# NVlabs/neuralrgbd

Hardware: AMD Instinct MI355X
Metric: depth frames/sec @256x192x64cand, 5-view window; warp-kernel HBM GB/s vs peak (higher is better)
Workload: dtype f32; 1 GPU; plane-sweep grid 256x192x64cand (image 1024x768); config_id=B, depth_candidates=64, views=5, streams_per_gpu=1, streams_total=1, parallelism=replicas x1 (independent video streams)

## Files before the change

### include/nrgbd.h

```cpp
#ifndef NRGBD_H
#define NRGBD_H

#ifdef __cplusplus
extern "C" {
#endif

#define NRGBD_OK             0
#define NRGBD_E_NULL        -1
#define NRGBD_E_SHAPE       -2
#define NRGBD_E_ALIGN       -3
#define NRGBD_E_ARG         -4

#define NRGBD_DIST_L2        0
#define NRGBD_DIST_L1        1

#define NRGBD_MAX_D        256
#define NRGBD_MAX_V         16

#define NRGBD_INTERFACE_VERSION "0.10"
const char* nrgbd_version(void);
const char* nrgbd_strerror(int code);

int nrgbd_homography_terms(const float* K, const float* R, long r_view_stride, long r_row_stride,
                           const float* t, long t_view_stride, long t_elem_stride, float* KR, float* Kt,
// ... 61 lines not shown
int nrgbd_dpv_resample(const float* dpv, const float* T, const float* rays,
                       const float* d_candi, float tan_hh, float tan_hv,
                       float z_half, float z_radius, float pad_value,
                       int do_clamp, float clamp_lo, float clamp_hi,
                       float* out, int D, int h, int w, void* stream);

int nrgbd_dpv_resample_to(const float* dpv, const float* T, const float* rays,
                          const float* d_candi_out, float tan_hh, float tan_hv,
                          float z_half, float z_radius, float pad_value,
                          int do_clamp, float clamp_lo, float clamp_hi,
                          float* out, int D_src, int D_out, int h, int w, void* stream);

int nrgbd_dpv_keyframe_maps(const float* dpv, const float* T, const float* rays,
                            const float* d_candi_out, const float* d_candi_src,
                            float tan_hh, float tan_hv, float z_half, float z_radius, float pad_value,
                            int do_clamp, float clamp_lo, float clamp_hi,
                            float* dmap_kf, float* conf_kf, float* dmap_ref, float* conf_ref,
                            int D_src, int D_out, int h, int w, void* stream);

int nrgbd_logsoftmax_d(const float* a, const float* b, float scale, float* out,
                       int D, long n, void* stream);

int nrgbd_depth_regress(const float* logp, const float* d_candi,
                        float* depth, float* conf, int D, long n, void* stream);

int nrgbd_export_depth_u16(const float* logp, const float* d_candi, float depth_scale, float conf_scale,
                           float* depth, float* conf, unsigned short* depth_u16, unsigned short* conf_u16,
                           int D, long n, void* stream);

int nrgbd_depth_regress_rows(const float* logp, const float* d_candi,
                             float* depth, float* conf, int D, long n, void* stream);
int nrgbd_export_depth_u16_rows(const float* logp, const float* d_candi, float depth_scale, float conf_scale,
                                float* depth, float* conf, unsigned short* depth_u16, unsigned short* conf_u16,
                                int D, long n, void* stream);

int nrgbd_warp_depth_fwd(const float* src, const float* dmap, const float* K, const float* R, const float* t,
                         const float* rays, float* out, int N, int C, int H, int W, void* stream);
int nrgbd_warp_depth_bwd_workgroups(int H, int W);
int nrgbd_warp_depth_bwd(const float* src, const float* dmap, const float* K, const float* R, const float* t,
                         const float* rays, const float* g_out, float* partial, float* g_R, float* g_t,
                         int N, int C, int H, int W, void* stream);

#define NRGBD_LBA_STATE      32
#define NRGBD_LBA_MAX_LEVELS  8
int nrgbd_lba_pyramid(const float* const* planes, int nplanes, int H, int W, const int* ks, int nlevels, float* out,
                      void* stream);
int nrgbd_lba_workgroups(int H, int W);
int nrgbd_lba_grad(const float* ref, const float* src, const float* dmap, const float* conf, const float* K, const float* rays,
                   const float* state, float* partial, int N, int H, int W, void* stream);
int nrgbd_lba_update(const float* partial, int nwg, const float* init, float* state, float* loss_log, int log_stride,
                     int log_slot, int N, int H, int W, int joint, int step, double lr, int opt_R, int opt_t, void* stream);

int nrgbd_conv3d_workgroups(int D, int H, int W);
int nrgbd_conv3d_pack_weights(const float* w, float* w_packed, int Cin, void* stream);
int nrgbd_conv3d_3x3x3_f32(const float* x, const float* x_ss, int x_relu,
                           const float* res, const float* res_ss, int res_relu,
                           float* materialized, const float* w_packed, float* y, float* stats,
                           int D, int H, int W, int Cin, int Cout, void* stream);
int nrgbd_conv3d_3x3x3_cout1_f32(const float* x, const float* x_ss, int x_relu,
                                 const float* res, const float* res_ss, int res_relu,
                                 const float* w_tap_major, float* y,
                                 int D, int H, int W, int Cin, void* stream);
int nrgbd_conv3d_cout1_bwd_workgroups(int D, int H, int W, int dgrad);
int nrgbd_conv3d_cout1_dgrad_f32(const float* gy, const float* w_tap_major, float* gx, int D, int H, int W, void* stream);
int nrgbd_conv3d_cout1_wgrad_workspace(int D, int H, int W, size_t* bytes);
int nrgbd_conv3d_cout1_wgrad_f32(const float* x, const float* gy, float* dw, void* workspace, size_t workspace_bytes, int D, int H, int W,
                                 void* stream);
int nrgbd_conv3d_wgrad_workgroups(void);
int nrgbd_conv3d_wgrad_ranges(void);
int nrgbd_conv3d_wgrad_f32(const float* x, const float* gy, float* partial, float* dw,
                           int D, int H, int W, int Cin, void* stream);
int nrgbd_bn3d_finalize(const float* stats, int num_workgroups, long count,
                        const float* gamma, const float* beta, float eps, float momentum,
                        float* running_mean, float* running_var, float* scale_shift, unsigned int* collapse_count, long long* batches_tracked, void* stream);

int nrgbd_bn2d_partial_floats(int C);
int nrgbd_bn2d_train_act(const float* x, const float* gamma, const float* beta, float eps, int act,
                         const float* residual, float* y, float* partial, float* mean_var,
                         int N, int C, long HW, void* stream);
int nrgbd_avgpool8(const float* x, float* y, int NC, int H, int W, void* stream);
int nrgbd_avgpool_cl(const float* x, float* y, int N, int H, int W, int C, int k, void* stream);
int nrgbd_conv2d_few_f32(const float* x, int ldx, const float* w_packed, const float* bias, int out_lrelu, float* y, int ldy,
                         int ycoff, int N, int H, int W, int Cin, int Cout, void* stream);
int nrgbd_scatter_channels(const float* src, long stride_c, long stride_y, long stride_x, int C, int H, int W, float* dst,
                           int ldy, int coff, int n_rep, long rep_stride, void* stream);
int nrgbd_bias_act_nchw(float* x, const float* bias, float slope, int N, int C, long HW, void* stream);

int nrgbd_conv_wino_tiles(int N, int H, int W, int dilation);
int nrgbd_conv_wino_rnet_f32(const float* x, const float* w_wino, const float* bias, int out_lrelu, float* y,
                             int N, int H, int W, int Cin, int Cout, void* stream);
int nrgbd_conv_wino_rnet_ex_f32(const float* x, const float* w_wino, const float* bias, int out_lrelu, float* y,
                                int N, int H, int W, int Cin, int Cout, int ldy, int ycoff, int cout_valid, void* stream);
int nrgbd_conv_wino_rnet_deconv_f32(const float* x, const float* w_masked, const float* bias, int out_lrelu, float* y,
                                    int N, int H, int W, int Cin, int Cout, int ldy, int ycoff, int cout_valid, void* stream);
int nrgbd_conv_wino_rnet_deconv_pack(const float* w_wino, float* w_masked, int Cin, void* stream);
int nrgbd_conv_wino_pack(const float* w, float* w_wino, int Cin, int Cout, int kd, int transposed, void* stream);
int nrgbd_bn_finalize_cm(const float* stats, int rows, int C, long count, const float* gamma, const float* beta, float eps,
                         float momentum, float* running_mean, float* running_var, float* scale_shift, unsigned int* collapse_count,
                         long long* batches_tracked, void* stream);
int nrgbd_conv_wino_f32(const float* x, const float* x_ss, int x_relu, const float* res, const float* res_ss,
                        int res_relu, float* materialized, const float* w_wino, float* y, float* stats,
                        int N, int H, int W, int Cin, int Cout, int kd, int dilation, void* stream);

int nrgbd_conv_wino_dw_pack(const float* w, float* w_wino, int Cin, int Cout, int transposed, void* stream);
int nrgbd_conv_wino_dw_f32(const float* x, const float* x_ss, int x_relu, const float* res, const float* res_ss,
                           int res_relu, float* materialized, const float* w_wino, float* y, float* stats,
                           int N, int H, int W, int Cin, int Cout, void* stream);
int nrgbd_conv_wino_dw_workgroups(int N, int H, int W, int Cout);
int nrgbd_conv_wino_dw4_pack(const float* w, float* w_wino, int Cin, int Cout, int transposed, void* stream);
int nrgbd_conv_wino_dw4_workspace(int N, int H, int W, int Cout, size_t* bytes);
int nrgbd_conv_wino_dw4_f32(const float* x, const float* x_ss, int x_relu, float x_unit, const float* w_wino, float* y, float* stats,
                            void* workspace, size_t workspace_bytes, int N, int H, int W, int Cin, int Cout, void* stream);
int nrgbd_conv_wino_dw_unit_f32(const float* x, const float* x_ss, float x_unit, const float* w_wino, float* y, float* stats,
                                int N, int H, int W, int Cin, int Cout, void* stream);

int nrgbd_conv2d_rnet_f32(const float* x, const float* w_packed, const float* bias, int out_lrelu, float* y,
                          int ldy, int ycoff, int cout_valid, int mode, int pa, int pb,
                          int N, int H, int W, int Cin, int Cout, void* stream);
int nrgbd_rnet_pack(const float* dpv_log, const float* feat, int feat_planar, float* out, int D, int Cf, long P,
                    void* stream);

int nrgbd_conv2d_taps_f32(const float* x, const float* x_ss, int x_relu, const float* w_packed, float* y, float* stats,
                          int N, int H, int W, int Cin, int Cout, int taps, int in_stride, void* stream);
int nrgbd_space_to_depth2(const float* x, int nchw, float* y, int N, int C, int H, int W, int Cp, void* stream);
int nrgbd_conv2d_wgrad_workgroups(int N, int H, int W, int Cin, int Cout);
int nrgbd_conv2d_wgrad_f32(const float* x, const float* gy, float* partial, float* dw, int N, int H, int W, int Cin, int Cout,
                           int dilation, void* stream);
int nrgbd_conv2d_workgroups(int N, int H, int W);
int nrgbd_conv_pack_weights(const float* w, float* w_packed, int Cin, int Cout, int taps, void* stream);
int nrgbd_conv2d_3x3_f32(const float* x, const float* x_ss, int x_relu,
                         const float* res, const float* res_ss, int res_relu,
                         float* materialized, const float* w_packed, const float* bias, int out_lrelu,
                         float* y, float* stats, int N, int H, int W, int Cin, int Cout, int dilation,
                         void* stream);
int nrgbd_bn_finalize(const float* stats, int num_workgroups, int C, long count,
                      const float* gamma, const float* beta, float eps, float momentum,
                      float* running_mean, float* running_var, float* scale_shift, unsigned int* collapse_count, long long* batches_tracked, void* stream);
int nrgbd_bn_small_stats(int nseg, const float* const* x, const long* rows, int C, const float* const* gamma, const float* const* beta,
                     const float* eps, const float* momentum, float* const* running_mean, float* const* running_var,
                     long long* const* batches_tracked, float* const* scale_shift, void* stream);
int nrgbd_spp_concat(const float* quarter, int Cq, const float* deep, int Cd,
                     const float* bz0, const float* bss0, int bh0, int bw0, const float* bz1, const float* bss1, int bh1, int bw1,
                     const float* bz2, const float* bss2, int bh2, int bw2, const float* bz3, const float* bss3, int bh3, int bw3,
                     int Cb, float* out, int N, int h, int w, void* stream);
int nrgbd_logsoftmax_rows(const float* x, float* y, long rows, int C, void* stream);
int nrgbd_logsoftmax_d_bwd(const float* logp, const float* g, float scale, float* gz, int D, long n, void* stream);
int nrgbd_logsoftmax_rows_bwd(const float* y, const float* g, float* gx, long rows, int C, void* stream);
int nrgbd_nll_workgroups(long n);
int nrgbd_nll_fwd(const float* logp, const long long* target, long ignore_index, int D, long n, int channels_last,
                  float* partial, float* out, void* stream);
int nrgbd_nll_bwd(const long long* target, long ignore_index, const float* g_out, const float* stat, float* g_logp, int D,
                  long n, int channels_last, void* stream);
int nrgbd_adam_step(float* const* params, const float* const* grads, float* const* exp_avg, float* const* exp_avg_sq,
                    float* const* steps, const long* numel, int ntensors, double lr, double beta1, double beta2, double eps,
                    double weight_decay, int maximize, void* stream);
long nrgbd_grad_norm_workspace(const long* numel, int ntensors);
int nrgbd_grad_norm(const float* const* grads, const long* numel, int ntensors, double max_norm, void* workspace,
                    size_t workspace_bytes, float* clip, float* nonfinite_steps, void* stream);
int nrgbd_scale_tensors(float* const* tensors, const long* numel, int ntensors, const float* clip, void* stream);
int nrgbd_adam_step_clipped(float* const* params, const float* const* grads, float* const* exp_avg, float* const* exp_avg_sq,
                            float* const* steps, const long* numel, int ntensors, double lr, double beta1, double beta2, double eps,
                            double weight_decay, int maximize, const float* clip, int skip_nonfinite, void* stream);
int nrgbd_bias_lrelu_cl_workgroups(long rows, int C);
int nrgbd_bias_lrelu_cl_fwd(const float* x, const float* bias, float slope, float* y, long rows, int C, void* stream);
int nrgbd_bias_lrelu_cl_bwd(const float* y, const float* gy, float slope, float* gx, float* g_bias, float* partial,
                            long rows, int C, void* stream);
int nrgbd_upsample_bilinear_ac(const float* x, float* y, int N, int bh, int bw, int H, int W, int C, int backward,
                               void* stream);
#define NRGBD_GATHER_MAX_V   6
typedef struct { int idx[NRGBD_GATHER_MAX_V + 1]; } nrgbd_window_slots;
int nrgbd_frame_ingest_u8(const unsigned char* src, int Hin, int Win, long pitch, int layout, float mean0, float mean1, float mean2,
                          float std0, float std1, float std2, float* dst, int Hout, int Wout, void* stream);
int nrgbd_window_gather(const float* ring, int R, long slot_stride, nrgbd_window_slots slots, int V, float* src, float* ref,
                        int H, int W, void* stream);
#define NRGBD_DEPTH_MAX_THRESHOLDS 512
int nrgbd_depth_ingest_u16(const unsigned short* depth, int Hin, int Win, long pitch, const int* rows_full, const int* cols_full,
                           const int* rows_q, const int* cols_q, const int* mask_rows_q, const int* mask_cols_q, float depth_scale,
                           const int* thr_q, int n_q, const int* thr_full, int n_full, long long* labels_q, long long* labels_full,
                           float* dmap_raw, float* dmap_imgsize, int H, int W, int h, int w, void* stream);
int nrgbd_nhwc_stats_workgroups(long P);
int nrgbd_nhwc_stats(const float* x, long P, int C, float* stats, void* stream);
int nrgbd_nhwc_act(const float* x, const float* x_ss, int x_relu, const float* res, const float* res_ss,
                   int res_relu, float* y, long P, int C, int ldy, void* stream);
int nrgbd_nhwc_act_lean(const float* x, const float* x_ss, int x_relu, const float* res, const float* res_ss,
                        int res_relu, float* y, long P, int C, int ldy, int wg_per_cu, void* stream);
#define NRGBD_DEPTH_EVAL_MAX_SETS 8
int nrgbd_depth_eval_workgroups(long n);
long nrgbd_depth_eval_workspace(long n, int J);
int nrgbd_depth_eval(const float* depth, const float* logconf, const float* gt, long n, float gt_min, float gt_max,
                     const float* log_thr, int J, void* workspace, long workspace_bytes, double* frame_sums,
                     long long* frame_counts, long long* frame_header, double* total_sums, long long* total_counts,
                     long long* total_header, float* err_map, void* stream);
#define NRGBD_DGF_TILE_Y 16
#define NRGBD_DGF_TILE_X 64
int nrgbd_dgf_refine_f32(const float* depth_lr, int n, int h, int w, const float* img, int H, int W,
                         const float* w1, const float* b1, const float* w2, const float* b2, float eps,
                         float* out, void* stream);
#define NRGBD_TSDF_EXTRACT_VOXELS 1024
#define NRGBD_TSDF_SCAN_PASS 1024
#define NRGBD_TSDF_RAYCAST_MAX_STEPS 65536
#define NRGBD_TSDF_RAYCAST_TILE 16
#define NRGBD_TSDF_RAYCAST_MAX_SIDE 16384
int nrgbd_tsdf_integrate_f32(float* tsdf, float* weight, int X, int Y, int Z, float ox, float oy, float oz, float voxel_size,
                             const float* depth, const float* gate, float gate_thr, const float* wmap, int H, int W,
                             const float* pose, float fx, float fy, float cx, float cy, float trunc, float d_near, float d_far,
                             float w_max, const int* box, void* stream);
long nrgbd_tsdf_extract_workspace(int X, int Y, int Z);
// ... 79 lines not shown
```

### neuralrgbd_amd/_lib.py

```python
import ctypes
import os

_HERE = os.path.dirname(os.path.abspath(__file__))
LIB_PATH = os.path.join(_HERE, "csrc", "libnrgbd_hip.so")

_c = ctypes
_P = _c.c_void_p
_F = _c.c_float
_I = _c.c_int
_L = _c.c_long
_D = _c.c_double
_Z = _c.c_size_t

GATHER_MAX_V = 6
DEPTH_MAX_THRESHOLDS = 512
DEPTH_EVAL_MAX_SETS = 8
DGF_TILE = (16, 64)
TSDF_EXTRACT_VOXELS = 1024
TSDF_SCAN_PASS = 1024
TSDF_RAYCAST_MAX_STEPS = 65536
TSDF_RAYCAST_TILE = 16
TSDF_RAYCAST_MAX_SIDE = 16384
ICP_MAX_WG = 256
ICP_RECORD_BYTES = 240
ICP_STATE_BYTES = 152
ICP_FEW, ICP_NONFINITE, ICP_DEGENERATE, ICP_LARGE = 1, 2, 3, 4
ICP_MAX_THETA2 = 0.25
CONSISTENCY_MAX_SRC = 16


class WindowSlots(ctypes.Structure):
    _fields_ = [("idx", _I * (GATHER_MAX_V + 1))]


SIGNATURES = {
    "nrgbd_version": (_c.c_char_p, []),
    "nrgbd_strerror": (_c.c_char_p, [_I]),
    "nrgbd_homography_terms": (_I, [_P, _P, _L, _L, _P, _L, _L, _P, _P, _I, _P]),
    "nrgbd_pose_inverse": (_I, [_P, _L, _P, _P, _I, _P]),
    "nrgbd_pack_nhwc": (_I, [_P, _P, _P, _I, _I, _I, _I, _I, _I, _I, _P, _P]),
    "nrgbd_costvol_fwd": (_I, [_P, _P, _P, _P, _P, _P, _F, _F, _F, _I, _I, _P, _P,
                               _I, _I, _I, _I, _I, _I, _P]),
    "nrgbd_costvol_fwd_gen": (_I, [_P, _P, _P, _P, _P, _P, _F, _F, _F, _I, _I, _P, _P,
                                   _I, _I, _I, _I, _I, _I, _I, _P]),
    "nrgbd_costvol_bwd_workspace": (_I, [_I, _I, _I, _I, _I, _P]),
    "nrgbd_costvol_bwd": (_I, [_P, _P, _P, _P, _P, _P, _F, _F, _F, _I, _I, _P, _P, _P,
                               _I, _I, _I, _I, _I, _I, _P, _Z, _P]),
    "nrgbd_costvol_bwd_det_workspace": (_I, [_I, _I, _I, _I, _I, _P]),
    "nrgbd_costvol_bwd_det": (_I, [_P, _P, _P, _P, _P, _P, _F, _F, _F, _I, _I, _P, _P, _P,
                                   _I, _I, _I, _I, _I, _I, _P, _Z, _P]),
    "nrgbd_bn_cl_workgroups": (_I, [_L, _I]),
    "nrgbd_bn_cl_fwd": (_I, [_P, _P, _P, _P, _F, _F, _P, _P, _I, _P, _P, _P, _L, _I, _P]),
    "nrgbd_bn_cl_bwd": (_I, [_P, _P, _P, _I, _P, _P, _P, _P, _P, _L, _I, _P]),
    "nrgbd_warp_volume": (_I, [_P, _L, _L, _L, _L, _P, _L, _L, _L, _P, _P, _P, _P, _F, _F, _I,
                               _P, _P, _P, _I, _I, _I, _I, _I, _I, _P]),
    "nrgbd_warp_volume_cl": (_I, [_P, _L, _L, _L, _L, _P, _L, _L, _L, _P, _P, _P, _P, _F, _F, _I,
                                  _P, _P, _P, _I, _I, _I, _I, _I, _I, _P]),
    "nrgbd_dpv_resample": (_I, [_P, _P, _P, _P, _F, _F, _F, _F, _F, _I, _F, _F, _P, _I, _I, _I, _P]),
    "nrgbd_dpv_resample_to": (_I, [_P, _P, _P, _P, _F, _F, _F, _F, _F, _I, _F, _F, _P, _I, _I, _I, _I, _P]),
    "nrgbd_dpv_keyframe_maps": (_I, [_P, _P, _P, _P, _P, _F, _F, _F, _F, _F, _I, _F, _F, _P, _P, _P, _P, _I, _I, _I, _I, _P]),
    "nrgbd_logsoftmax_d": (_I, [_P, _P, _F, _P, _I, _L, _P]),
    "nrgbd_depth_regress": (_I, [_P, _P, _P, _P, _I, _L, _P]),
    "nrgbd_export_depth_u16": (_I, [_P, _P, _F, _F, _P, _P, _P, _P, _I, _L, _P]),
    "nrgbd_depth_regress_rows": (_I, [_P, _P, _P, _P, _I, _L, _P]),
    "nrgbd_export_depth_u16_rows": (_I, [_P, _P, _F, _F, _P, _P, _P, _P, _I, _L, _P]),
    "nrgbd_warp_depth_fwd": (_I, [_P, _P, _P, _P, _P, _P, _P, _I, _I, _I, _I, _P]),
    "nrgbd_warp_depth_bwd_workgroups": (_I, [_I, _I]),
    "nrgbd_warp_depth_bwd": (_I, [_P, _P, _P, _P, _P, _P, _P, _P, _P, _P, _I, _I, _I, _I, _P]),
    "nrgbd_lba_pyramid": (_I, [_P, _I, _I, _I, _P, _I, _P, _P]),
    "nrgbd_lba_workgroups": (_I, [_I, _I]),
    "nrgbd_lba_grad": (_I, [_P, _P, _P, _P, _P, _P, _P, _P, _I, _I, _I, _P]),
    "nrgbd_lba_update": (_I, [_P, _I, _P, _P, _P, _I, _I, _I, _I, _I, _I, _I, _D, _I, _I, _P]),
    "nrgbd_conv3d_workgroups": (_I, [_I, _I, _I]),
    "nrgbd_conv3d_pack_weights": (_I, [_P, _P, _I, _P]),
    "nrgbd_conv3d_3x3x3_f32": (_I, [_P, _P, _I, _P, _P, _I, _P, _P, _P, _P, _I, _I, _I, _I, _I, _P]),
    "nrgbd_conv3d_3x3x3_cout1_f32": (_I, [_P, _P, _I, _P, _P, _I, _P, _P, _I, _I, _I, _I, _P]),
    "nrgbd_conv3d_cout1_bwd_workgroups": (_I, [_I, _I, _I, _I]),
    "nrgbd_conv3d_cout1_dgrad_f32": (_I, [_P, _P, _P, _I, _I, _I, _P]),
    "nrgbd_conv3d_cout1_wgrad_workspace": (_I, [_I, _I, _I, _P]),
    "nrgbd_conv3d_cout1_wgrad_f32": (_I, [_P, _P, _P, _P, _Z, _I, _I, _I, _P]),
    "nrgbd_conv_wino_tiles": (_I, [_I, _I, _I, _I]),
    "nrgbd_conv_wino_rnet_f32": (_I, [_P, _P, _P, _I, _P, _I, _I, _I, _I, _I, _P]),
    "nrgbd_conv_wino_rnet_ex_f32": (_I, [_P, _P, _P, _I, _P, _I, _I, _I, _I, _I, _I, _I, _I, _P]),
    "nrgbd_conv_wino_rnet_deconv_f32": (_I, [_P, _P, _P, _I, _P, _I, _I, _I, _I, _I, _I, _I, _I, _P]),
    "nrgbd_conv_wino_rnet_deconv_pack": (_I, [_P, _P, _I, _P]),
    "nrgbd_conv_wino_pack": (_I, [_P, _P, _I, _I, _I, _I, _P]),
    "nrgbd_bn_finalize_cm": (_I, [_P, _I, _I, _L, _P, _P, _F, _F, _P, _P, _P, _P, _P, _P]),
    "nrgbd_conv_wino_f32": (_I, [_P, _P, _I, _P, _P, _I, _P, _P, _P, _P, _I, _I, _I, _I, _I, _I, _I, _P]),
    "nrgbd_conv_wino_dw_pack": (_I, [_P, _P, _I, _I, _I, _P]),
    "nrgbd_conv_wino_dw_f32": (_I, [_P, _P, _I, _P, _P, _I, _P, _P, _P, _P, _I, _I, _I, _I, _I, _P]),
    "nrgbd_conv_wino_dw_workgroups": (_I, [_I, _I, _I, _I]),
    "nrgbd_conv_wino_dw_unit_f32": (_I, [_P, _P, _F, _P, _P, _P, _I, _I, _I, _I, _I, _P]),
    "nrgbd_conv_wino_dw4_pack": (_I, [_P, _P, _I, _I, _I, _P]),
    "nrgbd_conv_wino_dw4_workspace": (_I, [_I, _I, _I, _I, _P]),
    "nrgbd_conv_wino_dw4_f32": (_I, [_P, _P, _I, _F, _P, _P, _P, _P, _c.c_size_t, _I, _I, _I, _I, _I, _P]),
    "nrgbd_conv3d_wgrad_workgroups": (_I, []),
    "nrgbd_conv3d_wgrad_ranges": (_I, []),
    "nrgbd_conv3d_wgrad_f32": (_I, [_P, _P, _P, _P, _I, _I, _I, _I, _P]),
    "nrgbd_bn3d_finalize": (_I, [_P, _I, _L, _P, _P, _F, _F, _P, _P, _P, _P, _P, _P]),
    "nrgbd_bn2d_partial_floats": (_I, [_I]),
    "nrgbd_bn2d_train_act": (_I, [_P, _P, _P, _F, _I, _P, _P, _P, _P, _I, _I, _L, _P]),
    "nrgbd_avgpool8": (_I, [_P, _P, _I, _I, _I, _P]),
    "nrgbd_conv2d_few_f32": (_I, [_P, _I, _P, _P, _I, _P, _I, _I, _I, _I, _I, _I, _I, _P]),
    "nrgbd_avgpool_cl": (_I, [_P, _P, _I, _I, _I, _I, _I, _P]),
    "nrgbd_scatter_channels": (_I, [_P, _L, _L, _L, _I, _I, _I, _P, _I, _I, _I, _L, _P]),
    "nrgbd_bias_act_nchw": (_I, [_P, _P, _F, _I, _I, _L, _P]),
    "nrgbd_conv2d_workgroups": (_I, [_I, _I, _I]),
    "nrgbd_conv2d_wgrad_workgroups": (_I, [_I, _I, _I, _I, _I]),
    "nrgbd_conv2d_wgrad_f32": (_I, [_P, _P, _P, _P, _I, _I, _I, _I, _I, _I, _P]),
    "nrgbd_conv2d_taps_f32": (_I, [_P, _P, _I, _P, _P, _P, _I, _I, _I, _I, _I, _I, _I, _P]),
    "nrgbd_space_to_depth2": (_I, [_P, _I, _P, _I, _I, _I, _I, _I, _P]),
    "nrgbd_conv_pack_weights": (_I, [_P, _P, _I, _I, _I, _P]),
    "nrgbd_conv2d_3x3_f32": (_I, [_P, _P, _I, _P, _P, _I, _P, _P, _P, _I, _P, _P, _I, _I, _I, _I, _I, _I, _P]),
    "nrgbd_conv2d_rnet_f32": (_I, [_P, _P, _P, _I, _P, _I, _I, _I, _I, _I, _I, _I, _I, _I, _I, _I, _P]),
    "nrgbd_rnet_pack": (_I, [_P, _P, _I, _P, _I, _I, _L, _P]),
    "nrgbd_bn_finalize": (_I, [_P, _I, _I, _L, _P, _P, _F, _F, _P, _P, _P, _P, _P, _P]),
    "nrgbd_logsoftmax_rows": (_I, [_P, _P, _L, _I, _P]),
    "nrgbd_logsoftmax_d_bwd": (_I, [_P, _P, _F, _P, _I, _L, _P]),
    "nrgbd_logsoftmax_rows_bwd": (_I, [_P, _P, _P, _L, _I, _P]),
    "nrgbd_nll_workgroups": (_I, [_L]),
    "nrgbd_nll_fwd": (_I, [_P, _P, _L, _I, _L, _I, _P, _P, _P]),
    "nrgbd_nll_bwd": (_I, [_P, _L, _P, _P, _P, _I, _L, _I, _P]),
    "nrgbd_adam_step": (_I, [_P, _P, _P, _P, _P, _P, _I, _D, _D, _D, _D, _D, _I, _P]),
    "nrgbd_grad_norm_workspace": (_L, [_P, _I]),
    "nrgbd_grad_norm": (_I, [_P, _P, _I, _D, _P, _Z, _P, _P, _P]),
    "nrgbd_scale_tensors": (_I, [_P, _P, _I, _P, _P]),
    "nrgbd_adam_step_clipped": (_I, [_P, _P, _P, _P, _P, _P, _I, _D, _D, _D, _D, _D, _I, _P, _I, _P]),
    "nrgbd_bias_lrelu_cl_workgroups": (_I, [_L, _I]),
    "nrgbd_bias_lrelu_cl_fwd": (_I, [_P, _P, _F, _P, _L, _I, _P]),
    "nrgbd_bias_lrelu_cl_bwd": (_I, [_P, _P, _F, _P, _P, _P, _L, _I, _P]),
    "nrgbd_upsample_bilinear_ac": (_I, [_P, _P, _I, _I, _I, _I, _I, _I, _I, _P]),
    "nrgbd_bn_small_stats": (_I, [_I, _P, _P, _I, _P, _P, _P, _P, _P, _P, _P, _P, _P]),
    "nrgbd_spp_concat": (_I, [_P, _I, _P, _I, _P, _P, _I, _I, _P, _P, _I, _I, _P, _P, _I, _I, _P, _P, _I, _I, _I, _P, _I, _I, _I, _P]),
    "nrgbd_frame_ingest_u8": (_I, [_P, _I, _I, _L, _I, _F, _F, _F, _F, _F, _F, _P, _I, _I, _P]),
    "nrgbd_window_gather": (_I, [_P, _I, _L, WindowSlots, _I, _P, _P, _I, _I, _P]),
    "nrgbd_depth_ingest_u16": (_I, [_P, _I, _I, _L, _P, _P, _P, _P, _P, _P, _F, _P, _I, _P, _I, _P, _P, _P, _P, _I, _I, _I, _I, _P]),
    "nrgbd_depth_eval_workgroups": (_I, [_L]),
    "nrgbd_depth_eval_workspace": (_L, [_L, _I]),
    "nrgbd_depth_eval": (_I, [_P, _P, _P, _L, _F, _F, _P, _I, _P, _L, _P, _P, _P, _P, _P, _P, _P, _P]),
    "nrgbd_dgf_refine_f32": (_I, [_P, _I, _I, _I, _P, _I, _I, _P, _P, _P, _P, _F, _P, _P]),
    "nrgbd_tsdf_integrate_f32": (_I, [_P, _P, _I, _I, _I, _F, _F, _F, _F, _P, _P, _F, _P, _I, _I, _P, _F, _F, _F, _F, _F, _F, _F, _F, _P, _P]),
    "nrgbd_tsdf_extract_workspace": (_L, [_I, _I, _I]),
    "nrgbd_tsdf_extract_points": (_I, [_P, _P, _I, _I, _I, _F, _F, _F, _F, _F, _P, _L, _P, _L, _P, _P]),
    "nrgbd_tsdf_raycast_f32": (_I, [_P, _P, _I, _I, _I, _F, _F, _F, _F, _P, _P, _F, _F, _F, _F, _I, _I, _F, _F, _F, _F, _P, _P, _P]),
    "nrgbd_tsdf_mesh_workspace": (_L, [_I, _I, _I]),
    "nrgbd_tsdf_extract_mesh": (_I, [_P, _P, _I, _I, _I, _F, _F, _F, _F, _F, _P, _L, _P, _L, _P, _L, _P, _P]),
    "nrgbd_tsdf_integrate_color_f32": (_I, [_P, _P, _P, _I, _I, _I, _F, _F, _F, _F, _P, _P, _F, _P, _I, _I, _P, _F, _F, _F, _F, _F, _F, _F, _F,
                                            _P, _P, _I, _I, _F, _F, _F, _F, _P, _P]),
    "nrgbd_tsdf_extract_points_color": (_I, [_P, _P, _P, _I, _I, _I, _F, _F, _F, _F, _F, _P, _L, _P, _P, _L, _P, _P]),
    "nrgbd_tsdf_extract_mesh_color": (_I, [_P, _P, _P, _I, _I, _I, _F, _F, _F, _F, _F, _P, _L, _P, _P, _L, _P, _L, _P, _P]),
    "nrgbd_tsdf_raycast_color_f32": (_I, [_P, _P, _P, _I, _I, _I, _F, _F, _F, _F, _P, _P, _F, _F, _F, _F, _I, _I, _F, _F, _F, _F, _P, _P, _P, _P]),
    "nrgbd_tsdf_reintegrate_f32": (_I, [_P, _P, _I, _I, _I, _F, _F, _F, _F, _P, _P, _P, _P, _P, _I, _I, _F, _F, _F, _F, _F, _F, _F, _F, _F, _F,
                                        _P, _P]),
    "nrgbd_tsdf_reintegrate_color_f32": (_I, [_P, _P, _P, _I, _I, _I, _F, _F, _F, _F, _P, _P, _P, _P, _P, _I, _I, _F, _F, _F, _F, _F, _F, _F, _F,
                                              _F, _F, _P, _P, _I, _I, _F, _F, _F, _F, _P, _P]),
    "nrgbd_icp_workgroups": (_I, [_I, _I]),
    "nrgbd_icp_workspace": (_L, [_I, _I]),
    "nrgbd_icp_terms_f32": (_I, [_P, _P, _F, _I, _I, _F, _F, _F, _F, _F, _F, _I, _P, _P, _I, _I, _F, _F, _F, _F, _P, _F, _F, _P, _L, _P,
                                 _P]),
    "nrgbd_icp_terms_photo_f32": (_I, [_P, _P, _F, _I, _I, _F, _F, _F, _F, _F, _F, _I, _P, _P, _I, _I, _F, _F, _F, _F, _P, _F, _F, _P, _L,
                                       _P, _P, _P, _P, _P, _F, _F, _P, _P]),
    "nrgbd_icp_update": (_I, [_P, _P, _I, _P, _I, _c.c_longlong, _D, _P, _P]),
    "nrgbd_depth_consistency_f32": (_I, [_P, _P, _F, _I, _I, _F, _F, _F, _F, _F, _F, _P, _P, _L, _P, _P, _I, _F, _I, _P, _P, _P]),
    "nrgbd_tsdf_shift_f32": (_I, [_P, _P, _I, _I, _I, _I, _I, _I, _I, _I, _P]),
    "nrgbd_tsdf_blocks_gather_f32": (_I, [_P, _I, _I, _I, _I, _P, _I, _P, _P, _P]),
    "nrgbd_tsdf_blocks_scatter_f32": (_I, [_P, _I, _I, _I, _I, _P, _I, _P, _P]),
    "nrgbd_nhwc_stats_workgroups": (_I, [_L]),
    "nrgbd_nhwc_stats": (_I, [_P, _L, _I, _P, _P]),
    "nrgbd_nhwc_act": (_I, [_P, _P, _I, _P, _P, _I, _P, _L, _I, _I, _P]),
    "nrgbd_nhwc_act_lean": (_I, [_P, _P, _I, _P, _P, _I, _P, _L, _I, _I, _I, _P]),
}

_lib = None


class NrgbdError(RuntimeError):
    pass


def load():
    global _lib
    if _lib is not None:
        return _lib
    if not os.path.isfile(LIB_PATH):
        raise NrgbdError(
            "libnrgbd_hip.so not found at %s — build it with `python -m neuralrgbd_amd.build` "
            "(hipcc --offload-arch=gfx950). There is no CPU / eager fallback for this path." % LIB_PATH)
    lib = ctypes.CDLL(LIB_PATH)
    for name, (res, args) in SIGNATURES.items():
        try:
            fn = getattr(lib, name)
        except AttributeError:
            raise NrgbdError("libnrgbd_hip.so does not export %s (stale build?)" % name)
# ... 11 lines not shown
```

### neuralrgbd_amd/csrc/conv2d.hip

```cpp
#include <cstdint>
#include <cstdlib>

#include "conv_tile.hpp"

namespace nrgbd {

constexpr int kT2 = 16;

struct Conv2dArgs {
    const float* x;
    const float* x_ss;
    const float* res;
    const float* res_ss;
    float* mat;
    const float* wp;
    const float* bias;
    float* y;
    float* stats;
    int x_relu, res_relu, out_lrelu;
    int N, H, W, Cin;
    int xcd;
    int ldy;
    int ycoff;
    int cout_valid;
    int up;
    int pa, pb;
    float* planar;
    int xs;
};

template <int COUT, int DIL, bool RES, int NTAP = 9, int EPI = 0>
__global__ __launch_bounds__(256, COUT <= 32 ? 3 : 2) void conv2d_mfma_kernel(const Conv2dArgs a) {
    constexpr int HS = kT2 + 2 * DIL, HALO = HS * HS;
    constexpr int NPF = (HALO * (kCB / 4) + 255) / 256;
    constexpr int NF = COUT / 32;
    constexpr int G4 = kCB / 8;
    constexpr int NSTEP = NTAP * G4;
    static_assert(NTAP == 9 || ((NTAP == 4 || NTAP == 1) && DIL == 1), "2x2 taps: transposed-conv phases / stride-2 convs on a "
                                                                         "space-to-depth input; 1 tap: 1x1 convolutions");
    constexpr bool PF_SPREAD = 2 + (RES ? 2 : 1) * NPF <= NSTEP;
    static_assert(PF_SPREAD || NSTEP >= 2, "prefetch does not fit the step loop");
    extern __shared__ __attribute__((aligned(16))) float lds[];

    const int tid = threadIdx.x, lane = tid & 63, wv = tid >> 6;
    const int tiles_x = (a.W + kT2 - 1) / kT2, tiles_y = (a.H + kT2 - 1) / kT2;
    int t = xcd_tile(blockIdx.x, gridDim.x, a.xcd);
    const int tile_id = t;
    const int tx = t % tiles_x; t /= tiles_x;
    const int ty = t % tiles_y; const int n = t / tiles_y;
    const int x0 = tx * kT2, y0 = ty * kT2;
    const int Cin = a.Cin, ncblk = Cin / kCB;

    const int i = lane & 31, khalf = lane >> 5;
    int dy, px;
    row_to_yx(i, dy, px);
    const int wy = wv * 4;
    int pa = a.pa, pb = a.pb;
    const float* wpk = a.wp;
    if constexpr (NTAP == 4) {
        if (a.up == 2) { pa = blockIdx.y >> 1; pb = blockIdx.y & 1; wpk += (size_t)blockIdx.y * 4 * a.Cin * COUT; }
    }
    const int hv0 = (wy + dy) * HS + px + (NTAP == 4 ? pa * HS + pb : NTAP == 1 ? HS + 1 : 0);

    f32x16 acc[2][NF];
#pragma unroll
    for (int m = 0; m < 2; ++m)
#pragma unroll
        for (int f = 0; f < NF; ++f)
#pragma unroll
            for (int e = 0; e < 16; ++e) acc[m][f][e] = 0.f;

    const int c4 = tid & 3;
    unsigned pf_off[NPF];
    unsigned pf_ok = 0;
    unsigned pf_own = 0;
    f32x4 pre[NPF], prer[RES ? NPF : 1];
#pragma unroll
    for (int u = 0; u < NPF; ++u) {
        const int hv = (tid >> 2) + 64 * u;
        const int hy = hv / HS, hx = hv - hy * HS;
        const int gy = y0 + hy - DIL, gx = x0 + hx - DIL;
        const bool ok = hv < HALO && gy >= 0 && gy < a.H && gx >= 0 && gx < a.W;
        const int xs = (NTAP == 1 && a.xs > 1) ? a.xs : 1;
        pf_off[u] = ok ? (unsigned)((((size_t)n * (a.H * xs) + (size_t)gy * xs) * (a.W * xs) + (size_t)gx * xs) * Cin + c4 * 4) : (unsigned)(c4 * 4);
        if (ok) pf_ok |= 1u << u;
        if (ok && hy >= DIL && hy < DIL + kT2 && hx >= DIL && hx < DIL + kT2) pf_own |= 1u << u;
    }
#pragma unroll
    for (int u = 0; u < NPF; ++u) {
        pre[u] = *reinterpret_cast<const f32x4*>(a.x + pf_off[u]);
        if constexpr (RES) prer[u] = *reinterpret_cast<const f32x4*>(a.res + pf_off[u]);
    }

    const int wstep = ncblk * (G4 * NF * 64);
    for (int cblk = 0; cblk < ncblk; ++cblk) {
        {
            const int c = cblk * kCB + c4 * 4;
            float ss[8] = {1.f, 0.f, 1.f, 0.f, 1.f, 0.f, 1.f, 0.f}, rs[8] = {1.f, 0.f, 1.f, 0.f, 1.f, 0.f, 1.f, 0.f};
            if (a.x_ss) {
#pragma unroll
                for (int e = 0; e < 8; ++e) ss[e] = a.x_ss[2 * c + e];
            }
            if (RES && a.res_ss) {
#pragma unroll
                for (int e = 0; e < 8; ++e) rs[e] = a.res_ss[2 * c + e];
            }
#pragma unroll
            for (int u = 0; u < NPF; ++u) {
                const int hv = (tid >> 2) + 64 * u;
                if (hv >= HALO) continue;
                f32x4 v = {0.f, 0.f, 0.f, 0.f};
                if ((pf_ok >> u) & 1u) {
                    v = pre[u];
                    if (a.x_ss) {
                        v.x = __builtin_fmaf(v.x, ss[0], ss[1]); v.y = __builtin_fmaf(v.y, ss[2], ss[3]);
                        v.z = __builtin_fmaf(v.z, ss[4], ss[5]); v.w = __builtin_fmaf(v.w, ss[6], ss[7]);
                    }
                    if (a.x_relu) { v.x = fmaxf(v.x, 0.f); v.y = fmaxf(v.y, 0.f); v.z = fmaxf(v.z, 0.f); v.w = fmaxf(v.w, 0.f); }
                    if constexpr (RES) {
                        f32x4 r = prer[u];
                        if (a.res_ss) {
                            r.x = __builtin_fmaf(r.x, rs[0], rs[1]); r.y = __builtin_fmaf(r.y, rs[2], rs[3]);
                            r.z = __builtin_fmaf(r.z, rs[4], rs[5]); r.w = __builtin_fmaf(r.w, rs[6], rs[7]);
                        }
                        if (a.res_relu) { r.x = fmaxf(r.x, 0.f); r.y = fmaxf(r.y, 0.f); r.z = fmaxf(r.z, 0.f); r.w = fmaxf(r.w, 0.f); }
                        v = v + r;
                    }
                    if (a.mat && ((pf_own >> u) & 1u))
                        *reinterpret_cast<f32x4*>(a.mat + pf_off[u] + cblk * kCB) = v;
                }
                *reinterpret_cast<f32x4*>(lds + lds_slot(hv, c4)) = v;
            }
        }
        __syncthreads();

        const f32x4* wb = reinterpret_cast<const f32x4*>(wpk) + (size_t)cblk * (G4 * NF * 64) + lane;
        constexpr int BD = NTAP == 1 ? 1 : (COUT <= 64 ? 3 : 1), NB = BD + 1;
        f32x4 Bn[NB][NF], An[2][2];
#pragma unroll
        for (int b = 0; b < BD; ++b) {
            const f32x4* w0 = wb + (size_t)(b / G4) * wstep + (b % G4) * (NF * 64);
#pragma unroll
            for (int f = 0; f < NF; ++f) Bn[b][f] = w0[f * 64];
        }
        An[0][0] = *reinterpret_cast<const f32x4*>(lds + lds_slot(hv0, khalf * 2));
        An[0][1] = *reinterpret_cast<const f32x4*>(lds + lds_slot(hv0 + 2 * HS, khalf * 2));
        const unsigned nb = (cblk + 1) * kCB, live = cblk + 1 < ncblk ? ~0u : 0u;
#pragma unroll
        for (int s = 0; s < NSTEP; ++s) {
            const int cur = s & 1, nxt = cur ^ 1;
            if (s + 1 < NSTEP) {
                const int tap = (s + 1) / G4, g = (s + 1) % G4;
                const int voff = NTAP == 9 ? ((tap / 3) * HS + (tap % 3)) * DIL : NTAP == 4 ? (tap >> 1) * HS + (tap & 1) : 0;
                int h0 = hv0;
                asm volatile("" : "+v"(h0));
                An[nxt][0] = *reinterpret_cast<const f32x4*>(lds + lds_slot(h0 + voff, khalf * 2 + g));
                An[nxt][1] = *reinterpret_cast<const f32x4*>(lds + lds_slot(h0 + 2 * HS + voff, khalf * 2 + g));
            }
            if (s + BD < NSTEP) {
                const int tap = (s + BD) / G4, g = (s + BD) % G4;
                const f32x4* wn = wb + (size_t)tap * wstep + g * (NF * 64);
#pragma unroll
                for (int f = 0; f < NF; ++f) Bn[(s + BD) % NB][f] = wn[f * 64];
            }
            if constexpr (PF_SPREAD) {
                if constexpr (!RES) {
                    if (s >= 2 && s < 2 + NPF && live) pre[s - 2] = *reinterpret_cast<const f32x4*>(a.x + pf_off[s - 2] + nb);
                } else {
                    if (s >= 2 && s < 2 + NPF) pre[s - 2] = *reinterpret_cast<const f32x4*>(a.x + ((pf_off[s - 2] + nb) & live));
                }
                if constexpr (RES) {
                    if (s >= 2 + NPF && s < 2 + 2 * NPF)
                        prer[s - 2 - NPF] = *reinterpret_cast<const f32x4*>(a.res + ((pf_off[s - 2 - NPF] + nb) & live));
                }
            } else {
                if (s == 0) {
#pragma unroll
                    for (int u = 0; u < NPF; ++u) pre[u] = *reinterpret_cast<const f32x4*>(a.x + ((pf_off[u] + nb) & live));
                }
                if constexpr (RES) {
                    if (s == 1) {
#pragma unroll
                        for (int u = 0; u < NPF; ++u) prer[u] = *reinterpret_cast<const f32x4*>(a.res + ((pf_off[u] + nb) & live));
                    }
                }
            }
#pragma unroll
            for (int e = 0; e < 4; ++e)
#pragma unroll
                for (int m = 0; m < 2; ++m)
#pragma unroll
                    for (int f = 0; f < NF; ++f)
                        acc[m][f] = __builtin_amdgcn_mfma_f32_32x32x2f32(An[cur][m][e], Bn[s % NB][f][e], acc[m][f], 0, 0, 0);
        }
        __syncthreads();
    }

    float s1[NF], s2[NF], bs[NF];
#pragma unroll
    for (int f = 0; f < NF; ++f) { s1[f] = 0.f; s2[f] = 0.f; bs[f] = a.bias ? a.bias[f * 32 + i] : 0.f; }
    if constexpr (EPI == 1) {
        const size_t plane = (size_t)a.H * a.W;
#pragma unroll
        for (int m = 0; m < 2; ++m) {
#pragma unroll
            for (int q = 0; q < 4; ++q) {
                float z[4][NF];
#pragma unroll
                for (int e = 0; e < 4; ++e) {
                    float mx = -INFINITY;
#pragma unroll
                    for (int f = 0; f < NF; ++f) { z[e][f] = acc[m][f][4 * q + e] + bs[f]; mx = fmaxf(mx, z[e][f]); }
#pragma unroll
                    for (int o = 1; o < 32; o <<= 1) mx = fmaxf(mx, __shfl_xor(mx, o, 64));
                    float sm = 0.f;
#pragma unroll
                    for (int f = 0; f < NF; ++f) { z[e][f] = z[e][f] - mx; sm += expf(z[e][f]); }
#pragma unroll
                    for (int o = 1; o < 32; o <<= 1) sm += __shfl_xor(sm, o, 64);
                    const float ls = logf(sm);
#pragma unroll
                    for (int f = 0; f < NF; ++f) z[e][f] = z[e][f] - ls;
                }
                const int row = 8 * q + 4 * khalf;
                int ry, rx;
                row_to_yx(row, ry, rx);
                const int gy = y0 + wy + 2 * m + ry, gx = x0 + rx;
                if (gy < a.H) {
#pragma unroll
                    for (int f = 0; f < NF; ++f) {
                        float* o = a.planar + ((size_t)n * COUT + f * 32 + i) * plane + (size_t)gy * a.W + gx;
                        if (gx + 3 < a.W && (a.W & 3) == 0) {
                            *reinterpret_cast<f32x4*>(o) = f32x4{z[0][f], z[1][f], z[2][f], z[3][f]};
                        } else {
#pragma unroll
                            for (int e = 0; e < 4; ++e)
                                if (gx + e < a.W) o[e] = z[e][f];
                        }
                    }
                }
            }
        }
        return;
    }
#pragma unroll
    for (int m = 0; m < 2; ++m) {
#pragma unroll
        for (int r = 0; r < 16; ++r) {
            const int row = (r & 3) + 8 * (r >> 2) + 4 * khalf;
            int ry, rx;
            row_to_yx(row, ry, rx);
            const int gy = y0 + wy + 2 * m + ry, gx = x0 + rx;
            if (gy < a.H && gx < a.W) {
                const size_t pix = a.up ? ((size_t)n * (2 * a.H) + 2 * gy + pa) * (2 * a.W) + 2 * gx + pb
                                        : ((size_t)n * a.H + gy) * a.W + gx;
#pragma unroll
                for (int f = 0; f < NF; ++f) {
                    float z = acc[m][f][r] + bs[f];
                    if (a.out_lrelu) z = z > 0.f ? z : 0.01f * z;
                    if (f * 32 + i < a.cout_valid) a.y[pix * a.ldy + a.ycoff + f * 32 + i] = z;
                    s1[f] += z;
                    s2[f] = __builtin_fmaf(z, z, s2[f]);
                }
            }
        }
    }
    if (a.stats) {
        float* red = lds;
#pragma unroll
        for (int f = 0; f < NF; ++f) {
            s1[f] += __shfl_xor(s1[f], 32, 64);
            s2[f] += __shfl_xor(s2[f], 32, 64);
        }
        if (khalf == 0) {
#pragma unroll
            for (int f = 0; f < NF; ++f) {
                red[wv * (2 * COUT) + f * 32 + i] = s1[f];
                red[wv * (2 * COUT) + COUT + f * 32 + i] = s2[f];
            }
        }
// ... 98 lines not shown
void nhwc_act_lean_kernel(const float* __restrict__ x, const float* __restrict__ x_ss, int x_relu, const float* __restrict__ res,
                          const float* __restrict__ res_ss, int res_relu, float* __restrict__ y, int P, int C, int ldy) {
    extern __shared__ __attribute__((aligned(16))) float lean_tab[];
    const int tid = threadIdx.x, cq = C >> 2, ppw = 256 / cq;
    const bool xa = x_ss != nullptr, ra = RES && res_ss != nullptr;
    for (int j = tid; j < 2 * C; j += 256) {
        if (xa) lean_tab[(j & 1) * C + (j >> 1)] = x_ss[j];
        if (ra) lean_tab[2 * C + (j & 1) * C + (j >> 1)] = res_ss[j];
    }
    __syncthreads();
    const int lp = tid / cq, c = (tid - lp * cq) * 4;
    const unsigned lx = (unsigned)tid * 16u;
    const unsigned ly = ((unsigned)lp * (unsigned)ldy + (unsigned)c) * 4u;
    const float* tx = lean_tab + c;
    const int pstep = (int)gridDim.x * ppw;
    int pb = (int)blockIdx.x * ppw;
    u32x4 v[kLeanWords], r[RES ? kLeanWords : 1];
    auto request = [&](int u, int q) {
        v[u] = __builtin_amdgcn_raw_buffer_load_b128(lean_window(x, q, P, C, C, ppw), lx, 0, kLeanNt);
        if constexpr (RES) r[u] = __builtin_amdgcn_raw_buffer_load_b128(lean_window(res, q, P, C, C, ppw), lx, 0, kLeanNt);
    };
    auto finish = [&](int u, int q) {
        f32x4 a = __builtin_bit_cast(f32x4, v[u]);
        lean_apply(a, tx, C, xa, x_relu);
        if constexpr (RES) {
            f32x4 b = __builtin_bit_cast(f32x4, r[u]);
            lean_apply(b, tx + 2 * C, C, ra, res_relu);
            a = a + b;
        }
        __builtin_amdgcn_raw_buffer_store_b128(__builtin_bit_cast(u32x4, a), lean_window(y, q, P, ldy, C, ppw), ly, 0, kLeanNt);
    };
    static_assert(kLeanWords == 2, "the loop below names its two slots");
    request(0, pb);
    for (; pb < P; pb += 2 * pstep) {
        request(1, pb + pstep);
        finish(0, pb);
        request(0, pb + 2 * pstep);
        finish(1, pb + pstep);
    }
}

__global__ __launch_bounds__(256) void bn_finalize_kernel(const float* __restrict__ stats, int nwg, int C, double count,
                                                          const float* __restrict__ gamma, const float* __restrict__ beta,
                                                          float eps, float momentum, float* __restrict__ running_mean,
                                                          float* __restrict__ running_var, float* __restrict__ ss, unsigned int* __restrict__ collapse_count, long long* __restrict__ batches_tracked) {
    __shared__ double sh[2][256];
    const int c = blockIdx.x, tid = threadIdx.x;
    double s1 = 0.0, s2 = 0.0;
    for (int g = tid; g < nwg; g += 256) {
        s1 += (double)stats[(size_t)g * 2 * C + c];
        s2 += (double)stats[(size_t)g * 2 * C + C + c];
    }
    sh[0][tid] = s1; sh[1][tid] = s2;
    __syncthreads();
    for (int o = 128; o > 0; o >>= 1) {
        if (tid < o) { sh[0][tid] += sh[0][tid + o]; sh[1][tid] += sh[1][tid + o]; }
        __syncthreads();
    }
    if (tid == 0) bn_finalize_channel(sh[0][0], sh[1][0], count, gamma[c], beta[c], eps, momentum, running_mean, running_var, ss, c, collapse_count);
    if (tid == 0 && c == 0 && batches_tracked) *batches_tracked += 1;
}

template <int COUT, int DIL>
static void launch_conv2d(const Conv2dArgs& a, int nwg, hipStream_t st) {
    constexpr int HS = kT2 + 2 * DIL;
    const size_t lds = (size_t)HS * HS * kSV * sizeof(float);
    if (a.res) hipLaunchKernelGGL((conv2d_mfma_kernel<COUT, DIL, true>), dim3(nwg), dim3(256), lds, st, a);
    else       hipLaunchKernelGGL((conv2d_mfma_kernel<COUT, DIL, false>), dim3(nwg), dim3(256), lds, st, a);
}

template <int COUT, int NTAP, int EPI>
static void launch_conv2d_ex(const Conv2dArgs& a, int nwg, hipStream_t st, int ny = 1) {
    constexpr int HS = kT2 + 2;
    const size_t lds = (size_t)HS * HS * kSV * sizeof(float);
    hipLaunchKernelGGL((conv2d_mfma_kernel<COUT, 1, false, NTAP, EPI>), dim3(nwg, ny), dim3(256), lds, st, a);
}

template <int COUT, int NTAP>
static void launch_conv2d_taps(const Conv2dArgs& a, int nwg, hipStream_t st) {
    constexpr int HS = kT2 + 2;
    const size_t lds = (size_t)HS * HS * kSV * sizeof(float);
    hipLaunchKernelGGL((conv2d_mfma_kernel<COUT, 1, false, NTAP, 0>), dim3(nwg), dim3(256), lds, st, a);
}

__global__ __launch_bounds__(256) void space_to_depth2_kernel(const float* __restrict__ x, int nchw, float* __restrict__ y,
                                                              int N, int C, int H, int W, int Cp) {
    const int Ho = H >> 1, Wo = W >> 1;
    const long total = (long)N * Ho * Wo * Cp;
    const long idx = (long)blockIdx.x * 256 + threadIdx.x;
    if (idx >= total) return;
    const int cp = (int)(idx % Cp);
    long t = idx / Cp;
    const int xo = (int)(t % Wo); t /= Wo;
    const int yo = (int)(t % Ho);
    const int n = (int)(t / Ho);
    float v = 0.f;
    if (cp < 4 * C) {
        const int ph = cp / C, c = cp - ph * C;
        const int yi = 2 * yo + (ph >> 1), xi = 2 * xo + (ph & 1);
        v = nchw ? x[(((size_t)n * C + c) * H + yi) * W + xi] : x[(((size_t)n * H + yi) * W + xi) * C + c];
    }
    y[idx] = v;
}

__global__ __launch_bounds__(256) void space_to_depth2_cl4_kernel(const float* __restrict__ x, float* __restrict__ y, int N, int C, int H,
                                                                  int W, int Cp) {
    const int Ho = H >> 1, Wo = W >> 1, q4 = Cp >> 2;
    const long total = (long)N * Ho * Wo * q4;
    const long idx = (long)blockIdx.x * 256 + threadIdx.x;
    if (idx >= total) return;
    const int cp = (int)(idx % q4) * 4;
    long t = idx / q4;
    const int xo = (int)(t % Wo); t /= Wo;
    const int yo = (int)(t % Ho);
    const int n = (int)(t / Ho);
    float4 v = make_float4(0.f, 0.f, 0.f, 0.f);
    if (cp < 4 * C) {
        const int ph = cp / C, c = cp - ph * C;
        v = *reinterpret_cast<const float4*>(x + (((size_t)n * H + 2 * yo + (ph >> 1)) * W + 2 * xo + (ph & 1)) * C + c);
    }
    *reinterpret_cast<float4*>(y + idx * 4) = v;
}

__global__ __launch_bounds__(256) void space_to_depth2_rgb_kernel(const float* __restrict__ x, float* __restrict__ y, int N, int H, int W) {
    const int Ho = H >> 1, Wo = W >> 1;
    const long total = (long)N * Ho * Wo;
    const long idx = (long)blockIdx.x * 256 + threadIdx.x;
    if (idx >= total) return;
    const int xo = (int)(idx % Wo);
    long t = idx / Wo;
    const int yo = (int)(t % Ho);
    const int n = (int)(t / Ho);
    float2 v[3][2];
#pragma unroll
    for (int c = 0; c < 3; ++c)
#pragma unroll
        for (int py = 0; py < 2; ++py)
            v[c][py] = *reinterpret_cast<const float2*>(x + (((size_t)n * 3 + c) * H + 2 * yo + py) * W + 2 * xo);
    float o[16];
#pragma unroll
    for (int py = 0; py < 2; ++py)
#pragma unroll
        for (int c = 0; c < 3; ++c) { o[(py * 2 + 0) * 3 + c] = v[c][py].x; o[(py * 2 + 1) * 3 + c] = v[c][py].y; }
    o[12] = o[13] = o[14] = o[15] = 0.f;
    float4* dst = reinterpret_cast<float4*>(y + idx * 16);
#pragma unroll
    for (int q = 0; q < 4; ++q) dst[q] = make_float4(o[4 * q], o[4 * q + 1], o[4 * q + 2], o[4 * q + 3]);
}

}

extern "C" int nrgbd_space_to_depth2(const float* x, int nchw, float* y, int N, int C, int H, int W, int Cp, void* stream) {
    using namespace nrgbd;
    if (!x || !y) return NRGBD_E_NULL;
    if (N <= 0 || C <= 0 || H <= 0 || W <= 0 || (H & 1) || (W & 1) || Cp < 4 * C) return NRGBD_E_SHAPE;
    const long total = (long)N * (H / 2) * (W / 2) * Cp;
    const bool aligned = (((uintptr_t)x | (uintptr_t)y) & 15) == 0;
    if (!nchw && (C & 3) == 0 && (Cp & 3) == 0 && aligned)
        hipLaunchKernelGGL(space_to_depth2_cl4_kernel, dim3((unsigned)((total / 4 + 255) / 256)), dim3(256), 0, (hipStream_t)stream, x, y, N, C,
                           H, W, Cp);
    else if (nchw && C == 3 && Cp == 16 && aligned)
        hipLaunchKernelGGL(space_to_depth2_rgb_kernel, dim3((unsigned)((total / 16 + 255) / 256)), dim3(256), 0, (hipStream_t)stream, x, y, N,
                           H, W);
    else
        hipLaunchKernelGGL(space_to_depth2_kernel, dim3((unsigned)((total + 255) / 256)), dim3(256), 0, (hipStream_t)stream, x, nchw,
                           y, N, C, H, W, Cp);
    NRGBD_CHECK_LAUNCH();
    return NRGBD_OK;
}

extern "C" int nrgbd_conv2d_taps_f32(const float* x, const float* x_ss, int x_relu, const float* w_packed, float* y,
                                     float* stats, int N, int H, int W, int Cin, int Cout, int taps, int in_stride, void* stream) {
    using namespace nrgbd;
    if (!x || !w_packed || !y) return NRGBD_E_NULL;
    if (N <= 0 || H <= 0 || W <= 0 || Cin <= 0 || Cin % kCB) return NRGBD_E_SHAPE;
    if (taps != 1 && taps != 4) return NRGBD_E_ARG;
    if (in_stride < 1 || in_stride > 8 || (in_stride != 1 && taps != 1)) return NRGBD_E_ARG;
    if ((long)N * H * W * Cin * in_stride * in_stride >= (1L << 32)) return NRGBD_E_SHAPE;
    Conv2dArgs a{x, x_ss, nullptr, nullptr, nullptr, w_packed, nullptr, y, stats, x_relu, 0, 0, N, H, W, Cin,
                 0, Cout, 0, Cout, 0, 0, 0, nullptr, in_stride};
    const int nwg = ceil_div(W, kT2) * ceil_div(H, kT2) * N;
    hipStream_t st = (hipStream_t)stream;
    if (taps == 1) {
        if (Cout == 32) launch_conv2d_taps<32, 1>(a, nwg, st);
        else if (Cout == 64) launch_conv2d_taps<64, 1>(a, nwg, st);
        else if (Cout == 128) launch_conv2d_taps<128, 1>(a, nwg, st);
        else return NRGBD_E_SHAPE;
    } else {
        if (Cout == 32) launch_conv2d_taps<32, 4>(a, nwg, st);
        else if (Cout == 64) launch_conv2d_taps<64, 4>(a, nwg, st);
        else return NRGBD_E_SHAPE;
    }
    NRGBD_CHECK_LAUNCH();
    return NRGBD_OK;
}

extern "C" int nrgbd_conv2d_workgroups(int N, int H, int W) {
    using namespace nrgbd;
    if (N <= 0 || H <= 0 || W <= 0) return NRGBD_E_SHAPE;
    return ceil_div(W, kT2) * ceil_div(H, kT2) * N;
}

extern "C" int nrgbd_conv_pack_weights(const float* w, float* wp, int Cin, int Cout, int taps, void* stream) {
    using namespace nrgbd;
    if (!w || !wp) return NRGBD_E_NULL;
    if (Cin <= 0 || Cin % kCB || Cout <= 0 || Cout % 32 || (taps != 9 && taps != 27 && taps != 4 && taps != 1)) return NRGBD_E_SHAPE;
    const long total = (long)taps * Cin * Cout;
    hipLaunchKernelGGL(conv_pack_weights_kernel, dim3((unsigned)((total + 255) / 256)), dim3(256), 0, (hipStream_t)stream,
                       w, wp, Cin, Cout, taps);
    NRGBD_CHECK_LAUNCH();
    return NRGBD_OK;
}

extern "C" int nrgbd_conv2d_3x3_f32(const float* x, const float* x_ss, int x_relu, const float* res, const float* res_ss,
                                    int res_relu, float* materialized, const float* w_packed, const float* bias,
                                    int out_lrelu, float* y, float* stats, int N, int H, int W, int Cin, int Cout,
                                    int dilation, void* stream) {
    using namespace nrgbd;
    if (!x || !w_packed || !y) return NRGBD_E_NULL;
    if (N <= 0 || H <= 0 || W <= 0 || Cin <= 0 || Cin % kCB) return NRGBD_E_SHAPE;
    if ((long)N * H * W * Cin >= (1L << 32)) return NRGBD_E_SHAPE;
    Conv2dArgs a{x, x_ss, res, res_ss, materialized, w_packed, bias, y, stats, x_relu, res_relu, out_lrelu, N, H, W, Cin,
                 dev_env_int("NRGBD_XCD"), Cout, 0, Cout, 0, 0, 0, nullptr};
    const int nwg = ceil_div(W, kT2) * ceil_div(H, kT2) * N;
    hipStream_t st = (hipStream_t)stream;
    if (dilation == 1 && Cout == 32) launch_conv2d<32, 1>(a, nwg, st);
    else if (dilation == 1 && Cout == 64) launch_conv2d<64, 1>(a, nwg, st);
    else if (dilation == 1 && Cout == 96) launch_conv2d<96, 1>(a, nwg, st);
    else if (dilation == 1 && Cout == 128) launch_conv2d<128, 1>(a, nwg, st);
    else if (dilation == 2 && Cout == 128) launch_conv2d<128, 2>(a, nwg, st);
    else return NRGBD_E_SHAPE;
    NRGBD_CHECK_LAUNCH();
    return NRGBD_OK;
}

extern "C" int nrgbd_conv2d_rnet_f32(const float* x, const float* w_packed, const float* bias, int out_lrelu, float* y,
                                     int ldy, int ycoff, int cout_valid, int mode, int pa, int pb, int N, int H, int W,
                                     int Cin, int Cout, void* stream) {
    using namespace nrgbd;
    if (!x || !w_packed || !y) return NRGBD_E_NULL;
    if (N <= 0 || H <= 0 || W <= 0 || Cin <= 0 || Cin % kCB) return NRGBD_E_SHAPE;
    if ((long)N * H * W * Cin >= (1L << 32)) return NRGBD_E_SHAPE;
    if (mode < 0 || mode > 3 || (pa & ~1) || (pb & ~1)) return NRGBD_E_ARG;
    if (mode != 2 && (cout_valid <= 0 || cout_valid > Cout || ycoff < 0 || ldy < ycoff + cout_valid)) return NRGBD_E_SHAPE;
    Conv2dArgs a{x, nullptr, nullptr, nullptr, nullptr, w_packed, bias, y, nullptr, 0, 0, out_lrelu, N, H, W, Cin,
                 0, ldy, ycoff, cout_valid, mode == 1 ? 1 : (mode == 3 ? 2 : 0), pa, pb, mode == 2 ? y : nullptr};
    const int nwg = ceil_div(W, kT2) * ceil_div(H, kT2) * N;
    hipStream_t st = (hipStream_t)stream;
    if (mode == 0) {
        if (Cout == 64) launch_conv2d_ex<64, 9, 0>(a, nwg, st);
        else if (Cout == 96) launch_conv2d_ex<96, 9, 0>(a, nwg, st);
        else if (Cout == 128) launch_conv2d_ex<128, 9, 0>(a, nwg, st);
        else return NRGBD_E_SHAPE;
    } else if (mode == 1) {
        if (Cout == 64) launch_conv2d_ex<64, 4, 0>(a, nwg, st);
        else return NRGBD_E_SHAPE;
    } else if (mode == 3) {
        if (Cout == 64) launch_conv2d_ex<64, 4, 0>(a, nwg, st, 4);
        else return NRGBD_E_SHAPE;
    } else {
        if (Cout == 64) launch_conv2d_ex<64, 9, 1>(a, nwg, st);
        else if (Cout == 128) launch_conv2d_ex<128, 9, 1>(a, nwg, st);
        else return NRGBD_E_SHAPE;
    }
    NRGBD_CHECK_LAUNCH();
    return NRGBD_OK;
}

namespace nrgbd {
__global__ __launch_bounds__(256) void rnet_pack_kernel(const float* __restrict__ dpv_log, const float* __restrict__ feat,
                                                        int feat_planar, float* __restrict__ out, int D, int Cf, long P) {
    __shared__ float tile[64][65];
    const long p0 = (long)blockIdx.x * 64;
    const int tid = threadIdx.x, lane = tid & 63, wv = tid >> 6;
    const int C = D + Cf;
// ... 97 lines not shown
```

### neuralrgbd_amd/csrc/conv_few.hip

```cpp
#include "common.hpp"

namespace nrgbd {

typedef float f32x4 __attribute__((ext_vector_type(4)));

constexpr int kFewT = 16, kFewHS = kFewT + 2, kFewHalo = kFewHS * kFewHS;
constexpr int kFewPitch = 20;
constexpr int kFewNPF = (kFewHalo * 4 + 255) / 256;

struct ConvFewArgs {
    const float* x;
    const float* wp;
    const float* bias;
    float* y;
    int N, H, W, Cin, ldx, ldy, ycoff, lrelu;
};

template <int CO>
__global__ __launch_bounds__(256, 6) void conv_few_kernel(const ConvFewArgs a) {
    __shared__ __attribute__((aligned(16))) float tile[1][kFewHalo * kFewPitch];
    const int tid = threadIdx.x, px = tid & 15, py = tid >> 4;
    const int tiles_x = (a.W + kFewT - 1) / kFewT, tiles_y = (a.H + kFewT - 1) / kFewT;
    int t = blockIdx.x;
    const int tx = t % tiles_x; t /= tiles_x;
    const int ty = t % tiles_y; const int n = t / tiles_y;
    const int x0 = tx * kFewT, y0 = ty * kFewT;
    const int nblk = a.Cin >> 4;

    const int c4 = tid & 3;
    unsigned off[kFewNPF];
    unsigned ok = 0;
#pragma unroll
    for (int u = 0; u < kFewNPF; ++u) {
        const int hv = (tid >> 2) + 64 * u;
        const int hy = hv / kFewHS, hx = hv - hy * kFewHS;
        const int gy = y0 + hy - 1, gx = x0 + hx - 1;
        const bool in = hv < kFewHalo && gy >= 0 && gy < a.H && gx >= 0 && gx < a.W;
        off[u] = in ? (unsigned)((((size_t)n * a.H + gy) * a.W + gx) * a.ldx + c4 * 4) : (unsigned)(c4 * 4);
        if (in) ok |= 1u << u;
    }
    f32x4 pre[kFewNPF];
#pragma unroll
    for (int u = 0; u < kFewNPF; ++u) pre[u] = *reinterpret_cast<const f32x4*>(a.x + off[u]);
    auto publish = [&](int buf) {
#pragma unroll
        for (int u = 0; u < kFewNPF; ++u) {
            const int hv = (tid >> 2) + 64 * u;
            if (hv < kFewHalo)
                *reinterpret_cast<f32x4*>(&tile[buf][hv * kFewPitch + c4 * 4]) = ((ok >> u) & 1u) ? pre[u] : f32x4{0.f, 0.f, 0.f, 0.f};
        }
    };
    publish(0);
    __syncthreads();

    float acc[CO];
#pragma unroll
    for (int co = 0; co < CO; ++co) acc[co] = a.bias ? a.bias[co] : 0.f;

    for (int c = 0; c < nblk; ++c) {
        constexpr int buf = 0;
        if (c + 1 < nblk) {
#pragma unroll
            for (int u = 0; u < kFewNPF; ++u) pre[u] = *reinterpret_cast<const f32x4*>(a.x + off[u] + (c + 1) * 16);
        }
        const float* w = a.wp + (size_t)c * (9 * CO * 16);
#pragma unroll 1
        for (int ky = 0; ky < 3; ++ky) {
            const float* trow = &tile[buf][((py + ky) * kFewHS + px) * kFewPitch];
#pragma unroll
            for (int kx = 0; kx < 3; ++kx) {
                const float* tp = trow + kx * kFewPitch;
                f32x4 v[4];
#pragma unroll
                for (int q = 0; q < 4; ++q) v[q] = *reinterpret_cast<const f32x4*>(tp + 4 * q);
#pragma unroll
                for (int co = 0; co < CO; ++co) {
                    const float* wr = w + ((ky * 3 + kx) * CO + co) * 16;
#pragma unroll
                    for (int q = 0; q < 4; ++q) {
                        acc[co] = __builtin_fmaf(v[q].x, wr[4 * q + 0], acc[co]);
                        acc[co] = __builtin_fmaf(v[q].y, wr[4 * q + 1], acc[co]);
                        acc[co] = __builtin_fmaf(v[q].z, wr[4 * q + 2], acc[co]);
                        acc[co] = __builtin_fmaf(v[q].w, wr[4 * q + 3], acc[co]);
                    }
                }
            }
        }
        __syncthreads();
        if (c + 1 < nblk) publish(0);
        __syncthreads();
    }
    const int gy = y0 + py, gx = x0 + px;
    if (gy < a.H && gx < a.W) {
        float* o = a.y + (((size_t)n * a.H + gy) * a.W + gx) * a.ldy + a.ycoff;
#pragma unroll
        for (int co = 0; co < CO; ++co) {
            float z = acc[co];
            if (a.lrelu) z = z > 0.f ? z : 0.01f * z;
            o[co] = z;
        }
    }
}

}

extern "C" int nrgbd_conv2d_few_f32(const float* x, int ldx, const float* w_packed, const float* bias, int out_lrelu, float* y, int ldy,
                                    int ycoff, int N, int H, int W, int Cin, int Cout, void* stream) {
    using namespace nrgbd;
    if (!x || !w_packed || !y) return NRGBD_E_NULL;
    if (N <= 0 || H <= 0 || W <= 0 || Cin <= 0 || (Cin & 15) || ldx < Cin || (ldx & 3) || Cout < 1 || Cout > 4 || ycoff < 0 ||
        ldy < ycoff + Cout)
        return NRGBD_E_SHAPE;
    if (reinterpret_cast<uintptr_t>(x) & 15) return NRGBD_E_ALIGN;
    if ((long)N * H * W * ldx >= (1L << 32)) return NRGBD_E_SHAPE;
    ConvFewArgs a{x, w_packed, bias, y, N, H, W, Cin, ldx, ldy, ycoff, out_lrelu};
    const int nwg = ceil_div(W, kFewT) * ceil_div(H, kFewT) * N;
    hipStream_t st = (hipStream_t)stream;
    switch (Cout) {
        case 1: hipLaunchKernelGGL(conv_few_kernel<1>, dim3(nwg), dim3(256), 0, st, a); break;
        case 2: hipLaunchKernelGGL(conv_few_kernel<2>, dim3(nwg), dim3(256), 0, st, a); break;
        case 3: hipLaunchKernelGGL(conv_few_kernel<3>, dim3(nwg), dim3(256), 0, st, a); break;
        default: hipLaunchKernelGGL(conv_few_kernel<4>, dim3(nwg), dim3(256), 0, st, a); break;
    }
    NRGBD_CHECK_LAUNCH();
    return NRGBD_OK;
}
```

### neuralrgbd_amd/csrc/wino_pc.hip

```cpp
#include "wino_pc.hpp"

namespace nrgbd {

namespace {

struct PcLane {
    int kq, jj;
    int msel, cwv;
    int a0, a1;
    unsigned ldy, lane_yoff;
};
template <bool HALF> using PcAcc = f32x4[16][HALF ? 1 : 2];

template <int DIL, int EPI, bool HALF>
__device__ __forceinline__ PcLane pc_lane(const WinoPcArgs& a, int lane, int wv) {
    PcLane c;
    c.kq = lane >> 4; c.jj = lane & 15;
    c.msel = HALF ? (wv >> 1) : 0;
    c.cwv = HALF ? (wv & 1) : wv;
    c.a0 = pc_slot(0, 16 * c.msel + c.jj, c.kq); c.a1 = pc_slot(0, 16 + c.jj, c.kq);
    c.ldy = (EPI == 1 && a.ldy) ? (unsigned)a.ldy : (unsigned)a.Cout;
    c.lane_yoff = (unsigned)c.jj + (unsigned)((DIL * 2 * (c.kq >> 1)) * a.W + 8 * (c.kq & 1) * DIL) * c.ldy;
    return c;
}

template <bool HALF>
__device__ __forceinline__ void pc_prime_weights(f32x4 (&Bn)[kPcNB], const f32x4* wt) {
    constexpr int BD = HALF ? 6 : kPcBD;
#pragma unroll
    for (int b = 0; b < BD; ++b) Bn[b] = wt[b * 256];
}
template <bool HALF>
__device__ __forceinline__ void pc_prime_a(f32x4 (&An)[4][2], const float* Vb, const PcLane& c) {
#pragma unroll
    for (int i = 0; i < 2; ++i) {
        An[i][0] = *reinterpret_cast<const f32x4*>(Vb + c.a0 + (HALF ? 2 * i : i) * kPcTiles * kCB);
        An[i][1] = *reinterpret_cast<const f32x4*>(Vb + (HALF ? c.a0 + (2 * i + 1) * kPcTiles * kCB : c.a1 + i * kPcTiles * kCB));
    }
}

template <bool HALF, bool FIRST>
__device__ __forceinline__ void pc_mfma_stage(PcAcc<HALF>& acc, f32x4 (&An)[4][2], f32x4 (&Bn)[kPcNB], const float* Vc, const float* Vn,
                                              const f32x4* wcur, const f32x4* wnx, const PcLane& c) {
    const int a0 = c.a0, a1 = c.a1;
    const f32x4 zero4 = {0.f, 0.f, 0.f, 0.f};
    if constexpr (HALF) {
#pragma unroll
        for (int xp = 0; xp < 8; ++xp) {
            const int cur = xp & 3, nxt = (xp + 2) & 3;
            const float* Vs = xp + 2 < 8 ? Vc : Vn;
            const int pn = (xp + 2) & 7;
            An[nxt][0] = *reinterpret_cast<const f32x4*>(Vs + a0 + (2 * pn) * (kPcTiles * kCB));
            An[nxt][1] = *reinterpret_cast<const f32x4*>(Vs + a0 + (2 * pn + 1) * (kPcTiles * kCB));
#pragma unroll
            for (int e = 0; e < 4; ++e) {
                acc[2 * xp][0] = __builtin_amdgcn_mfma_f32_16x16x4f32(An[cur][0][e], Bn[(2 * xp) % kPcNB][e],
                                                                      FIRST && e == 0 ? zero4 : acc[2 * xp][0], 0, 0, 0);
                acc[2 * xp + 1][0] = __builtin_amdgcn_mfma_f32_16x16x4f32(An[cur][1][e], Bn[(2 * xp + 1) % kPcNB][e],
                                                                          FIRST && e == 0 ? zero4 : acc[2 * xp + 1][0], 0, 0, 0);
                if (e == 1) Bn[(2 * xp + 6) % kPcNB] = 2 * xp + 6 < 16 ? wcur[(2 * xp + 6) * 256] : wnx[(2 * xp + 6 - 16) * 256];
                if (e == 3) Bn[(2 * xp + 7) % kPcNB] = 2 * xp + 7 < 16 ? wcur[(2 * xp + 7) * 256] : wnx[(2 * xp + 7 - 16) * 256];
                __builtin_amdgcn_sched_barrier(0);
            }
        }
    } else {
#pragma unroll
        for (int xi = 0; xi < 16; ++xi) {
            const int cur = xi & 3, nxt = (xi + 2) & 3;
            if (xi + 2 < 16) {
                An[nxt][0] = *reinterpret_cast<const f32x4*>(Vc + a0 + (xi + 2) * (kPcTiles * kCB));
                An[nxt][1] = *reinterpret_cast<const f32x4*>(Vc + a1 + (xi + 2) * (kPcTiles * kCB));
            } else {
                An[nxt][0] = *reinterpret_cast<const f32x4*>(Vn + a0 + (xi + 2 - 16) * (kPcTiles * kCB));
                An[nxt][1] = *reinterpret_cast<const f32x4*>(Vn + a1 + (xi + 2 - 16) * (kPcTiles * kCB));
            }
#pragma unroll
            for (int e = 0; e < 4; ++e) {
                acc[xi][0] = __builtin_amdgcn_mfma_f32_16x16x4f32(An[cur][0][e], Bn[xi % kPcNB][e], FIRST && e == 0 ? zero4 : acc[xi][0], 0, 0, 0);
                acc[xi][1] = __builtin_amdgcn_mfma_f32_16x16x4f32(An[cur][1][e], Bn[xi % kPcNB][e], FIRST && e == 0 ? zero4 : acc[xi][1], 0, 0, 0);
                if (e == kPcWPos) Bn[(xi + kPcBD) % kPcNB] = xi + kPcBD < 16 ? wcur[(xi + kPcBD) * 256] : wnx[(xi + kPcBD - 16) * 256];
                __builtin_amdgcn_sched_barrier(0);
            }
        }
    }
}

template <int DIL, int EPI, bool HALF>
__device__ __forceinline__ void pc_epilogue_interior(const PcAcc<HALF>& acc, const WinoPcArgs& a, const PcLane& c, float* ybase, bool cok,
                                                     float bval, float& s1, float& s2) {
    const unsigned ldy = c.ldy, lane_yoff = c.lane_yoff;
    float neg1 = -1.f;
    asm volatile("" : "+v"(neg1));
    const f32x2 n1 = {neg1, neg1};
    const f32x2 bias2 = {bval, bval};
    f32x2 S1 = {0.f, 0.f}, S2 = {0.f, 0.f};
#pragma unroll
    for (int mi = 0; mi < (HALF ? 1 : 2); ++mi) {
        const int m = HALF ? c.msel : mi;
#pragma unroll
        for (int rp = 0; rp < 2; ++rp) {
            f32x2 tr[2][4];
#pragma unroll
            for (int xx = 0; xx < 4; ++xx) {
                const f32x2 m0 = rp ? acc[0 + xx][mi].hi : acc[0 + xx][mi].lo, m1 = rp ? acc[4 + xx][mi].hi : acc[4 + xx][mi].lo;
                const f32x2 m2 = rp ? acc[8 + xx][mi].hi : acc[8 + xx][mi].lo, m3 = rp ? acc[12 + xx][mi].hi : acc[12 + xx][mi].lo;
                tr[0][xx] = (m0 + m1) + m2;
                tr[1][xx] = __builtin_elementwise_fma(m3, n1, __builtin_elementwise_fma(m2, n1, m1));
            }
#pragma unroll
            for (int aa = 0; aa < 2; ++aa) {
                f32x2 o0 = (tr[aa][0] + tr[aa][1]) + tr[aa][2];
                f32x2 o1 = __builtin_elementwise_fma(tr[aa][3], n1, __builtin_elementwise_fma(tr[aa][2], n1, tr[aa][1]));
                if constexpr (EPI == 1) {
                    o0 = o0 + bias2; o1 = o1 + bias2;
                    if (a.out_lrelu) {
                        const f32x2 sl = {0.01f, 0.01f};
                        o0 = __builtin_elementwise_max(o0, o0 * sl); o1 = __builtin_elementwise_max(o1, o1 * sl);
                    }
                }
                float* oa = ybase + ((size_t)(DIL * (4 * m + aa)) * a.W + (size_t)(2 * (2 * rp) * DIL)) * ldy;
                float* ob = ybase + ((size_t)(DIL * (4 * m + aa)) * a.W + (size_t)(2 * (2 * rp + 1) * DIL)) * ldy;
                if (cok) {
                    oa[lane_yoff] = o0.x; oa[lane_yoff + DIL * ldy] = o1.x;
                    ob[lane_yoff] = o0.y; ob[lane_yoff + DIL * ldy] = o1.y;
                }
                S1 = (S1 + o0) + o1;
                S2 = __builtin_elementwise_fma(o1, o1, __builtin_elementwise_fma(o0, o0, S2));
            }
        }
    }
    s1 = S1.x + S1.y; s2 = S2.x + S2.y;
}

template <int DIL, int EPI, bool HALF>
__device__ __forceinline__ void pc_epilogue_edge(const PcAcc<HALF>& acc, const WinoPcArgs& a, const PcTile& tl, const PcLane& c, float* ybase,
                                                 bool cok, float bval, float& s1, float& s2) {
    const unsigned ldy = c.ldy, lane_yoff = c.lane_yoff;
#pragma unroll
    for (int mi = 0; mi < (HALF ? 1 : 2); ++mi) {
        const int m = HALF ? c.msel : mi;
#pragma unroll
        for (int r = 0; r < 4; ++r) {
            float tr[2][4];
#pragma unroll
            for (int xx = 0; xx < 4; ++xx) {
                const float m0 = acc[0 + xx][mi][r], m1 = acc[4 + xx][mi][r], m2 = acc[8 + xx][mi][r], m3 = acc[12 + xx][mi][r];
                tr[0][xx] = (m0 + m1) + m2;
                tr[1][xx] = (m1 - m2) - m3;
            }
#pragma unroll
            for (int aa = 0; aa < 2; ++aa) {
                float o0 = (tr[aa][0] + tr[aa][1]) + tr[aa][2];
                float o1 = (tr[aa][1] - tr[aa][2]) - tr[aa][3];
                if constexpr (EPI == 1) {
                    o0 += bval; o1 += bval;
                    if (a.out_lrelu) { o0 = fmaxf(o0, 0.01f * o0); o1 = fmaxf(o1, 0.01f * o1); }
                }
                float* o = ybase + ((size_t)(DIL * (4 * m + aa)) * a.W + (size_t)(2 * r * DIL)) * ldy;
                const int tile = 16 * m + 4 * c.kq + r;
                const int gy = tl.y0 + tl.py + DIL * (2 * (tile >> 3) + aa), gx = tl.x0 + tl.px + DIL * (2 * (tile & 7));
                if (gy < a.H && cok) {
                    if (gx < a.W) { o[lane_yoff] = o0; s1 += o0; s2 = __builtin_fmaf(o0, o0, s2); }
// ... 364 lines not shown
        const f32x4 R0 = *reinterpret_cast<const f32x4*>(rawT + p.rdR0 + co);
        const f32x4 R1 = *reinterpret_cast<const f32x4*>(rawT + p.rdR1 + co);
        const f32x4 R2 = *reinterpret_cast<const f32x4*>(rawT + p.rdR2 + co);
        ya[cc] = pk_fma_s(R1, m1, R0);
        yb[cc] = pk_fma_s(R2, p.sg, R1);
    }
    float* V = Vq + p.vslot;
    constexpr int kXi = kPcTiles * kCB;
    *reinterpret_cast<f32x4*>(V + 0 * kXi) = pk_fma_s(ya[2], m1, ya[0]);
    *reinterpret_cast<f32x4*>(V + 1 * kXi) = pk_add(ya[1], ya[2]);
    *reinterpret_cast<f32x4*>(V + 2 * kXi) = pk_fma_s(ya[1], m1, ya[2]);
    *reinterpret_cast<f32x4*>(V + 3 * kXi) = pk_fma_s(ya[3], m1, ya[1]);
    *reinterpret_cast<f32x4*>(V + 4 * kXi) = pk_fma_s(yb[2], m1, yb[0]);
    *reinterpret_cast<f32x4*>(V + 5 * kXi) = pk_add(yb[1], yb[2]);
    *reinterpret_cast<f32x4*>(V + 6 * kXi) = pk_fma_s(yb[1], m1, yb[2]);
    *reinterpret_cast<f32x4*>(V + 7 * kXi) = pk_fma_s(yb[3], m1, yb[1]);
}

template <int KD, bool RES, int EPI, bool MAT>
__device__ __forceinline__ void pc_stage(const WinoPcArgs& a, const PcProd& P, int NS, int s, PcRegs<RES>& r) {
    const int cb = s / KD, kd = s - cb * KD;
    const int z = KD == 3 ? P.tl.n + kd - 1 : P.tl.n;
    const bool zin = KD != 3 || (z >= 0 && z < a.N);
    float* raw = P.rawb + (P.gi & 1) * kPcShStrip;
    const float* rawT = P.rawb + ((P.gi & 1) ^ 1) * kPcShStrip;
    if (!zin) {
#pragma unroll
        for (int u = 0; u < kPcNPF; ++u) *reinterpret_cast<f32x4*>(raw + P.p.wr_off[u]) = f32x4{0.f, 0.f, 0.f, 0.f};
    } else {
        asm volatile("" : "+v"(r.ss[0]), "+v"(r.ss[1]));
        if constexpr (RES) asm volatile("" : "+v"(r.rs[0]), "+v"(r.rs[1]));
        if (P.interior) pc_activate_publish<KD, RES, EPI, MAT, true>(a, P, r, raw, cb, kd, z);
        else pc_activate_publish<KD, RES, EPI, MAT, false>(a, P, r, raw, cb, kd, z);
    }
    const bool nx = s + 2 >= NS;
    pc_issue<KD, RES, EPI>(a, P, nx && P.has_next, nx ? s + 2 - NS : s + 2, r);
    if (P.gi > 0) pc_transform(P.p, rawT, P.Vb + P.qbuf * kPcV);
}
__device__ __forceinline__ void pc_stage_end(PcProd& P) {
    if (P.gi > 0) P.qbuf = P.qbuf == kPcNBuf - 1 ? 0 : P.qbuf + 1;
    ++P.gi;
}

}

template <int KD, int DIL, bool RES, bool ODD = false, int EPI = 0, bool MAT = false, bool HALF = false>
__global__ __launch_bounds__(512) void conv_wino_pc_kernel(const WinoPcArgs a) {
    extern __shared__ __attribute__((aligned(16))) float lds[];
    float* Vb = lds;
    float* rawb = lds + kPcNBuf * kPcV;
    float* ssl = rawb + kPcStrips;

    const int tid = threadIdx.x, lane = tid & 63;
    const int wave = __builtin_amdgcn_readfirstlane(tid >> 6);
    const int wv = wave & 3;
    const int NS = (a.Cin / kCB) * KD;

    int first, step, end;
    pc_tile_share(a.ntiles, first, step, end);
    if (first >= end) return;
    const int count = (end - first + step - 1) / step;
    if constexpr (EPI == 0) {
        pc_load_ss_table<true>(ssl, a.Cin, a.x_ss, RES ? a.res_ss : nullptr, 1.f);
        __syncthreads();
    }

    if constexpr (EPI == 2) {
        if (wave >= 4) { pc_dc_consumer(a, Vb, NS, first, step, count, lane, wv); return; }
    }
    if (wave >= 4) {
        const PcLane c = pc_lane<DIL, EPI, HALF>(a, lane, wv);
        PcAcc<HALF> acc;
        const f32x4* wbase = reinterpret_cast<const f32x4*>(a.wp) + c.cwv * 64 + lane;
        const size_t wgroup = (size_t)NS * 16 * 256;
        PcTile tl = pc_decode<KD, DIL>(first, a);
        const f32x4* wt = wbase + (size_t)tl.cg * wgroup;
        f32x4 Bn[kPcNB], An[4][2];
        pc_prime_weights<HALF>(Bn, wt);
        __syncthreads();
        __syncthreads();
        __syncthreads();
        pc_prime_a<HALF>(An, Vb, c);
        int buf = 0;
        for (int it = 0; it < count; ++it) {
            const int tnext = first + (it + 1 < count ? it + 1 : it) * step;
            const PcTile tn = pc_decode<KD, DIL>(tnext, a);
            const f32x4* wt_next = wbase + (size_t)tn.cg * wgroup;
            for (int s = 0; s < NS; ++s) {
                const float* Vc = Vb + buf * kPcV;
                const int nbuf = buf == kPcNBuf - 1 ? 0 : buf + 1;
                const float* Vn = Vb + nbuf * kPcV;
                const f32x4* wcur = wt + (size_t)s * (16 * 256);
                const f32x4* wnx = s + 1 < NS ? wcur + 16 * 256 : wt_next;
                if (s == 0) pc_mfma_stage<HALF, true>(acc, An, Bn, Vc, Vn, wcur, wnx, c);
                else pc_mfma_stage<HALF, false>(acc, An, Bn, Vc, Vn, wcur, wnx, c);
                __syncthreads();
                buf = nbuf;
            }
            pc_epilogue<DIL, EPI, HALF>(acc, a, tl, c);
            tl = tn;
            wt = wt_next;
        }
    } else {
        PcProd P;
        P.p = pc_items(wv, lane);
        P.Vb = Vb; P.rawb = rawb; P.ssl = ssl;
        P.plane = (unsigned)((size_t)a.H * a.W * a.Cin);
        P.tl = pc_decode<KD, DIL>(first, a); P.tn = P.tl;
        pc_book<KD, DIL>(a, P.p, P.tl, P.cur);
        PcRegs<RES> set0, set1;
        pc_issue<KD, RES, EPI>(a, P, false, 0, set0);
        pc_issue<KD, RES, EPI>(a, P, false, 1, set1);
        P.qbuf = 0; P.gi = 0;
        for (int it = 0; it < count; ++it) {
            P.has_next = it + 1 < count;
            P.interior = P.tl.y0 + P.tl.py - DIL >= 0 && P.tl.y0 + P.tl.py + DIL * kPcTH < a.H && P.tl.x0 + P.tl.px - DIL >= 0 && P.tl.x0 + P.tl.px + DIL * kPcTW < a.W;
            if constexpr (!ODD) {
                for (int s = 0; s < NS; s += 2) {
                    if (s + 2 == NS && P.has_next) { P.tn = pc_decode<KD, DIL>(first + (it + 1) * step, a); pc_book<KD, DIL>(a, P.p, P.tn, P.nxt); }
                    pc_stage<KD, RES, EPI, MAT>(a, P, NS, s, set0);
                    __syncthreads();
                    pc_stage_end(P);
                    pc_stage<KD, RES, EPI, MAT>(a, P, NS, s + 1, set1);
                    __syncthreads();
                    pc_stage_end(P);
                }
            } else {
                for (int s = 0; s < NS; ++s) {
                    if (s + 2 == NS && P.has_next) { P.tn = pc_decode<KD, DIL>(first + (it + 1) * step, a); pc_book<KD, DIL>(a, P.p, P.tn, P.nxt); }
                    if (((unsigned)it * (unsigned)NS + (unsigned)s) & 1u) { pc_stage<KD, RES, EPI, MAT>(a, P, NS, s, set1); __syncthreads(); }
                    else { pc_stage<KD, RES, EPI, MAT>(a, P, NS, s, set0); __syncthreads(); }
                    pc_stage_end(P);
                }
            }
            P.tl = P.tn;
            P.cur = P.nxt;
        }
        pc_transform(P.p, rawb + ((P.gi & 1) ^ 1) * kPcShStrip, Vb + P.qbuf * kPcV);
        __syncthreads();
        __syncthreads();
        __syncthreads();
    }
}

__global__ __launch_bounds__(1024) void bn_finalize_cm_kernel(const float* __restrict__ stats, int rows, int C, double count,
                                                              const float* __restrict__ gamma, const float* __restrict__ beta,
                                                              float eps, float momentum, float* __restrict__ running_mean,
                                                              float* __restrict__ running_var, float* __restrict__ ss, unsigned int* __restrict__ collapse_count, long long* __restrict__ batches_tracked) {
    __shared__ double sh[2][1024];
    const int c = blockIdx.x, tid = threadIdx.x;
    const float* p1 = stats + (size_t)c * rows;
    const float* p2 = stats + (size_t)(C + c) * rows;
    double s1 = 0.0, s2 = 0.0;
    int g = tid;
    for (; g + 7 * 1024 < rows; g += 8 * 1024) {
        float u[8], v[8];
#pragma unroll
        for (int k = 0; k < 8; ++k) { u[k] = p1[g + k * 1024]; v[k] = p2[g + k * 1024]; }
#pragma unroll
        for (int k = 0; k < 8; ++k) { s1 += (double)u[k]; s2 += (double)v[k]; }
    }
    for (; g < rows; g += 1024) { s1 += (double)p1[g]; s2 += (double)p2[g]; }
    sh[0][tid] = s1; sh[1][tid] = s2;
    __syncthreads();
    for (int o = 512; o > 0; o >>= 1) {
        if (tid < o) { sh[0][tid] += sh[0][tid + o]; sh[1][tid] += sh[1][tid + o]; }
        __syncthreads();
    }
    if (tid == 0) bn_finalize_channel(sh[0][0], sh[1][0], count, gamma[c], beta[c], eps, momentum, running_mean, running_var, ss, c, collapse_count);
    if (tid == 0 && c == 0 && batches_tracked) *batches_tracked += 1;
}

__global__ __launch_bounds__(256) void conv_wino_pack_kernel(const float* __restrict__ w, float* __restrict__ wp, int Cin, int Cout, int KD,
                                                             int transposed) {
    const long total = (long)Cout * Cin * KD * 16;
    if (transposed == 2) {
        transposed = blockIdx.y;
        if (transposed) { const int c = Cin; Cin = Cout; Cout = c; wp += total; }
// ... 52 lines not shown
    const hipError_t e = set_max_dynamic_lds(reinterpret_cast<const void*>(&conv_wino_pc_kernel<KD, DIL, RES, ODD, EPI, MAT, HALF>), L.lds_attr);
    if (e != hipSuccess) return e;
    hipLaunchKernelGGL((conv_wino_pc_kernel<KD, DIL, RES, ODD, EPI, MAT, HALF>), dim3(L.nwg), dim3(512), L.lds, L.stream, a);
    return hipSuccess;
}

template <int KD, int DIL, bool HALF>
static hipError_t pc_launch_forms(const void* res, const void* mat, const PcLaunch& L, const WinoPcArgs& a) {
    if (res && mat) return pc_launch<KD, DIL, true, false, 0, true, HALF>(L, a);
    if (res) return pc_launch<KD, DIL, true, false, 0, false, HALF>(L, a);
    if (mat) return pc_launch<KD, DIL, false, false, 0, true, HALF>(L, a);
    return pc_launch<KD, DIL, false, false, 0, false, HALF>(L, a);
}

}

extern "C" int nrgbd_conv_wino_pack(const float* w, float* w_wino, int Cin, int Cout, int kd, int transposed, void* stream) {
    using namespace nrgbd;
    if (!w || !w_wino) return NRGBD_E_NULL;
    if (Cin <= 0 || Cin % kCB || Cout <= 0 || Cout % 64 || (kd != 1 && kd != 3)) return NRGBD_E_SHAPE;
    if (transposed < 0 || transposed > 2) return NRGBD_E_ARG;
    if (transposed == 2 && Cin % 64) return NRGBD_E_SHAPE;
    const long total = (long)Cout * Cin * kd * 16;
    hipLaunchKernelGGL(conv_wino_pack_kernel, dim3((unsigned)((total + 255) / 256), transposed == 2 ? 2 : 1), dim3(256), 0, (hipStream_t)stream,
                       w, w_wino, Cin, Cout, kd, transposed);
    NRGBD_CHECK_LAUNCH();
    return NRGBD_OK;
}

extern "C" int nrgbd_bn_finalize_cm(const float* stats, int rows, int C, long count, const float* gamma, const float* beta,
                                    float eps, float momentum, float* running_mean, float* running_var, float* scale_shift, unsigned int* collapse_count, long long* batches_tracked,
                                    void* stream) {
    using namespace nrgbd;
    if (!stats || !gamma || !beta || !scale_shift) return NRGBD_E_NULL;
    if (rows <= 0 || count <= 0 || C <= 0) return NRGBD_E_SHAPE;
    if ((running_mean == nullptr) != (running_var == nullptr)) return NRGBD_E_NULL;
    hipLaunchKernelGGL(bn_finalize_cm_kernel, dim3(C), dim3(1024), 0, (hipStream_t)stream, stats, rows, C, (double)count, gamma,
                       beta, eps, momentum, running_mean, running_var, scale_shift, collapse_count, batches_tracked);
    NRGBD_CHECK_LAUNCH();
    return NRGBD_OK;
}

extern "C" int nrgbd_conv_wino_tiles(int N, int H, int W, int dilation) {
    using namespace nrgbd;
    if (N <= 0 || H <= 0 || W <= 0 || (dilation != 1 && dilation != 2)) return NRGBD_E_SHAPE;
    return N * ceil_div(H, kPcTH * dilation) * ceil_div(W, kPcTW * dilation) * dilation * dilation;
}

extern "C" int nrgbd_conv_wino_f32(const float* x, const float* x_ss, int x_relu, const float* res, const float* res_ss,
                                   int res_relu, float* materialized, const float* w_wino, float* y, float* stats, int N,
                                   int H, int W, int Cin, int Cout, int kd, int dilation, void* stream) {
    using namespace nrgbd;
    if (!x || !w_wino || !y) return NRGBD_E_NULL;
    const bool half = Cout == 32;
    if (N <= 0 || H <= 0 || W <= 0 || Cin <= 0 || Cin % kCB || Cin > 2048 || Cout <= 0 || (Cout % 64 && !half)) return NRGBD_E_SHAPE;
    if ((kd != 1 && kd != 3) || (dilation != 1 && dilation != 2) || (kd == 3 && dilation != 1)) return NRGBD_E_ARG;
    if (half && (kd != 1 || dilation != 1)) return NRGBD_E_SHAPE;
    if ((Cin / kCB) * kd < 2) return NRGBD_E_SHAPE;
    if ((long)(kd == 3 ? 1 : N) * H * W * Cin >= (1L << 30)) return NRGBD_E_SHAPE;
    const int rows = nrgbd_conv_wino_tiles(N, H, W, dilation);
    const long nt = (long)rows * (half ? 1 : Cout / 64);
    if (nt >= (1L << 30)) return NRGBD_E_SHAPE;
    WinoPcArgs a{x, x_ss, res, res_ss, materialized, w_wino, y, stats, x_relu, res_relu, N, H, W, Cin, Cout, (int)nt, half ? 2 * rows : rows,
                 nullptr, 0, 0, 0, 0};
    int nwg = 0;
    const int rc = pc_workgroups(nt, &nwg);
    if (rc != NRGBD_OK) return rc;
    const size_t lds = (size_t)(kPcNBuf * kPcV + kPcStrips + 4 * Cin) * sizeof(float);
    const int lds_attr = (int)((size_t)(kPcNBuf * kPcV + kPcStrips + 4 * 2048) * sizeof(float));
    const bool odd = (((Cin / kCB) * kd) & 1) != 0;
    if (odd && (kd != 3 || res || materialized)) return NRGBD_E_SHAPE;
    const PcLaunch L{nwg, lds, lds_attr, (hipStream_t)stream};
    hipError_t e;
    if (half) e = pc_launch_forms<1, 1, true>(res, materialized, L, a);
    else if (kd == 3 && odd) e = pc_launch<3, 1, false, true>(L, a);
    else if (kd == 3) e = pc_launch_forms<3, 1, false>(res, materialized, L, a);
    else if (dilation == 1) e = pc_launch_forms<1, 1, false>(res, materialized, L, a);
    else e = pc_launch_forms<1, 2, false>(res, materialized, L, a);
    if (e != hipSuccess) return (int)e;
    NRGBD_CHECK_LAUNCH();
    return NRGBD_OK;
}

extern "C" int nrgbd_conv_wino_rnet_ex_f32(const float* x, const float* w_wino, const float* bias, int out_lrelu, float* y, int N,
                                           int H, int W, int Cin, int Cout, int ldy, int ycoff, int cout_valid, void* stream) {
    using namespace nrgbd;
    if (!x || !w_wino || !y) return NRGBD_E_NULL;
    const bool half = Cout == 32;
    if (N <= 0 || H <= 0 || W <= 0 || Cin < 32 || Cin % kCB || Cout <= 0 || (Cout % 64 && !half)) return NRGBD_E_SHAPE;
    if ((long)N * H * W * Cin >= (1L << 30)) return NRGBD_E_SHAPE;
    if (cout_valid < 0 || cout_valid > Cout || ycoff < 0 || (ldy != 0 && ldy < ycoff + (cout_valid ? cout_valid : Cout))) return NRGBD_E_ARG;
    if ((long)N * H * W * (ldy ? ldy : Cout) >= (1L << 32)) return NRGBD_E_SHAPE;
    const int rows = nrgbd_conv_wino_tiles(N, H, W, 1);
    const long nt = (long)rows * (half ? 1 : Cout / 64);
    if (nt >= (1L << 30)) return NRGBD_E_SHAPE;
    WinoPcArgs a{x, nullptr, nullptr, nullptr, nullptr, w_wino, y, nullptr, 0, 0, N, H, W, Cin, Cout, (int)nt, half ? 2 * rows : rows,
                 bias, out_lrelu, ldy, ycoff, cout_valid};
    int nwg = 0;
    const int rc = pc_workgroups(nt, &nwg);
    if (rc != NRGBD_OK) return rc;
    const size_t lds = (size_t)(kPcNBuf * kPcV + kPcStrips) * sizeof(float);
    const PcLaunch L{nwg, lds, (int)lds, (hipStream_t)stream};
    const bool odd = ((Cin / kCB) & 1) != 0;
    hipError_t e;
    if (odd && half) e = pc_launch<1, 1, false, true, 1, false, true>(L, a);
    else if (odd) e = pc_launch<1, 1, false, true, 1, false, false>(L, a);
    else if (half) e = pc_launch<1, 1, false, false, 1, false, true>(L, a);
    else e = pc_launch<1, 1, false, false, 1, false, false>(L, a);
    if (e != hipSuccess) return (int)e;
    NRGBD_CHECK_LAUNCH();
    return NRGBD_OK;
}

extern "C" int nrgbd_conv_wino_rnet_deconv_pack(const float* w_wino, float* w_masked, int Cin, void* stream) {
    using namespace nrgbd;
    if (!w_wino || !w_masked) return NRGBD_E_NULL;
    if (Cin <= 0 || Cin % kCB) return NRGBD_E_SHAPE;
    if ((reinterpret_cast<uintptr_t>(w_wino) | reinterpret_cast<uintptr_t>(w_masked)) & 15) return NRGBD_E_ALIGN;
    const int NS = Cin / kCB;
    const long total = 4L * NS * kPcDcPts * 256;
    hipLaunchKernelGGL(conv_wino_deconv_pack_kernel, dim3((unsigned)((total + 255) / 256)), dim3(256), 0, (hipStream_t)stream,
                       reinterpret_cast<const f32x4*>(w_wino), reinterpret_cast<f32x4*>(w_masked), NS);
    NRGBD_CHECK_LAUNCH();
    return NRGBD_OK;
}

extern "C" int nrgbd_conv_wino_rnet_deconv_f32(const float* x, const float* w_masked, const float* bias, int out_lrelu, float* y, int N,
                                               int H, int W, int Cin, int Cout, int ldy, int ycoff, int cout_valid, void* stream) {
    using namespace nrgbd;
    if (!x || !w_masked || !y) return NRGBD_E_NULL;
    if (N <= 0 || H <= 0 || W <= 0 || Cin < 32 || Cin % kCB || ((Cin / kCB) & 1) || Cout != 64) return NRGBD_E_SHAPE;
    if ((long)N * H * W * Cin >= (1L << 30)) return NRGBD_E_SHAPE;
    if (ldy == 0) ldy = Cout;
    if (cout_valid == 0) cout_valid = Cout;
    if (cout_valid < 0 || cout_valid > Cout || ycoff < 0 || ldy < ycoff + cout_valid) return NRGBD_E_ARG;
    if (4L * N * H * W * ldy >= (1L << 31)) return NRGBD_E_SHAPE;
    if ((reinterpret_cast<uintptr_t>(x) | reinterpret_cast<uintptr_t>(w_masked)) & 15) return NRGBD_E_ALIGN;
    if ((reinterpret_cast<uintptr_t>(y) | reinterpret_cast<uintptr_t>(bias)) & 3) return NRGBD_E_ALIGN;
    const int rows = nrgbd_conv_wino_tiles(N, H, W, 1);
    const long nt = (long)rows * 4;
    if (nt >= (1L << 30)) return NRGBD_E_SHAPE;
    WinoPcArgs a{x, nullptr, nullptr, nullptr, nullptr, w_masked, y, nullptr, 0, 0, N, H, W, Cin, 4 * Cout, (int)nt, rows,
                 bias, out_lrelu, ldy, ycoff, cout_valid};
    int nwg = 0;
    const int rc = pc_workgroups(nt, &nwg);
    if (rc != NRGBD_OK) return rc;
    const size_t lds = (size_t)(kPcNBuf * kPcV + kPcStrips) * sizeof(float);
    const PcLaunch L{nwg, lds, (int)lds, (hipStream_t)stream};
    const hipError_t e = pc_launch<1, 1, false, false, 2, false, false>(L, a);
    if (e != hipSuccess) return (int)e;
    NRGBD_CHECK_LAUNCH();
    return NRGBD_OK;
}

extern "C" int nrgbd_conv_wino_rnet_f32(const float* x, const float* w_wino, const float* bias, int out_lrelu, float* y, int N,
                                        int H, int W, int Cin, int Cout, void* stream) {
    return nrgbd_conv_wino_rnet_ex_f32(x, w_wino, bias, out_lrelu, y, N, H, W, Cin, Cout, 0, 0, 0, stream);
}
```

### neuralrgbd_amd/csrc/wino_pc.hpp

```cpp
#pragma once
#include <type_traits>

#include "conv_tile.hpp"

namespace nrgbd {

constexpr int kPcTH = 8, kPcTW = 16;
constexpr int kPcTiles = 32;
constexpr int kPcRawW = 20;
constexpr int kPcV = 16 * kPcTiles * kCB;
constexpr int kPcNBuf = 3;
constexpr int kPcWPos = 1;
constexpr int kPcBD = 7, kPcNB = 8;
constexpr int kPcShRows = kPcTH + 2;
constexpr int kPcShStrip = kPcShRows * kPcRawW * kCB;
constexpr int kPcShItems = kPcShRows * 18 * 4;
constexpr int kPcNPF = 3;
constexpr int kPcStrips = 2 * kPcShStrip;

struct WinoPcArgs {
    const float* x;
    const float* x_ss;
    const float* res;
    const float* res_ss;
    float* mat;
    const float* wp;
    float* y;
    float* stats;
    int x_relu, res_relu;
    int N, H, W, Cin, Cout;
    int ntiles;
    int rows;
    const float* bias;
    int out_lrelu;
    int ldy, ycoff, cout_valid;
    float x_unit;
};

struct PcTile { int n, y0, x0, py, px, cg, row; };

template <int KD, int DIL>
__device__ __forceinline__ PcTile pc_decode(int t, const WinoPcArgs& a) {
    PcTile r;
    const int ncg = (a.Cout + 63) >> 6;
    const int tiles_x = (a.W + kPcTW * DIL - 1) / (kPcTW * DIL), tiles_y = (a.H + kPcTH * DIL - 1) / (kPcTH * DIL);
    r.row = t / ncg;
    r.cg = t - r.row * ncg;
    t = r.row;
    r.n = 0;
    if (KD == 3) { r.n = t % a.N; t /= a.N; }
    int par = 0;
    if (DIL > 1) { par = t % (DIL * DIL); t /= DIL * DIL; }
    const int tx = t % tiles_x; t /= tiles_x;
    int ty = t;
    if (KD != 3) { ty = t % tiles_y; r.n = t / tiles_y; }
    r.py = par / DIL; r.px = par - r.py * DIL;
    r.y0 = ty * kPcTH * DIL; r.x0 = tx * kPcTW * DIL;
    return r;
}

__device__ __forceinline__ void pc_tile_share(int ntiles, int& first, int& step, int& end) {
    const int G = (int)gridDim.x, b = (int)blockIdx.x;
    if ((G & 7) == 0) {
        const int xc = b & 7;
        first = (int)(((long)ntiles * xc) >> 3) + (b >> 3);
        end = (int)(((long)ntiles * (xc + 1)) >> 3);
        step = G >> 3;
    } else { first = b; end = ntiles; step = G; }
}

__device__ __forceinline__ int pc_slot(int xi, int tile, int slot) {
    return ((xi * kPcTiles + tile) << 4) + (((slot + 2 * ((tile >> 3) & 1)) & 3) << 2);
}

typedef float f32x2 __attribute__((ext_vector_type(2)));

typedef int i32x4_t __attribute__((ext_vector_type(4)));
__device__ __forceinline__ __amdgpu_buffer_rsrc_t pc_rsrc(const void* base) {
    return __builtin_amdgcn_make_buffer_rsrc(const_cast<void*>(base), 0, -1, 0x00020000);
}
__device__ __forceinline__ f32x4 pc_bload(__amdgpu_buffer_rsrc_t r, unsigned byte_off) {
    return __builtin_bit_cast(f32x4, __builtin_amdgcn_raw_buffer_load_b128(r, (int)byte_off, 0, 0));
}

__device__ __forceinline__ int pc_ss_slot(int i) {
    const int c = i >> 1, t = i & 1;
    return ((c >> 2) << 3) + (((c >> 1) & 1) << 2) + (t << 1) + (c & 1);
}

template <bool RES_TABLE>
__device__ __forceinline__ void pc_load_ss_table(float* ssl, int Cin, const float* x_ss, const float* res_ss, float unit) {
    for (int i = threadIdx.x; i < 2 * Cin; i += 512) {
        const int j = pc_ss_slot(i);
        ssl[j] = (x_ss ? x_ss[i] : ((i & 1) ? 0.f : 1.f)) * unit;
        if constexpr (RES_TABLE) ssl[2 * Cin + j] = res_ss ? res_ss[i] : ((i & 1) ? 0.f : 1.f);
    }
}

__device__ __forceinline__ f32x4 pk_fma_s(f32x4 a, float s, f32x4 c) {
    const f32x2 m = {s, s};
    const f32x2 lo = __builtin_elementwise_fma(a.lo, m, c.lo), hi = __builtin_elementwise_fma(a.hi, m, c.hi);
    return __builtin_shufflevector(lo, hi, 0, 1, 2, 3);
}
__device__ __forceinline__ float relu1(float x) {
    float r;
    asm("v_max_f32 %0, 0, %1" : "=v"(r) : "v"(x));
    return r;
}
__device__ __forceinline__ f32x2 pk_fma_clamp01(f32x2 a, f32x2 b, f32x2 c) {
    f32x2 d;
    asm("v_pk_fma_f32 %0, %1, %2, %3 clamp" : "=v"(d) : "v"(a), "v"(b), "v"(c));
    return d;
}
__device__ __forceinline__ f32x4 pk_add(f32x4 a, f32x4 b) {
    const f32x2 lo = a.lo + b.lo, hi = a.hi + b.hi;
    return __builtin_shufflevector(lo, hi, 0, 1, 2, 3);
}

}
// ... 1 lines not shown
```

### neuralrgbd_amd/nets.py

```python
import math

import numpy as np
import torch
import torch.nn as nn
import torch.nn.functional as F


def _conv_bn2d(cin, cout, k, stride, pad, dilation, track=False):
    p = dilation if dilation > 1 else pad
    return nn.Sequential(
        nn.Conv2d(cin, cout, k, stride=stride, padding=p, dilation=dilation, bias=False),
        nn.BatchNorm2d(cout, track_running_stats=track),
    )


def _conv_bn3d(cin, cout):
    return nn.Sequential(nn.Conv3d(cin, cout, 3, stride=1, padding=1, bias=False), nn.BatchNorm3d(cout))


def _conv_lrelu(cin, cout):
    return nn.Sequential(nn.Conv2d(cin, cout, 3, stride=1, padding=1, bias=True), nn.LeakyReLU())


def _deconv_lrelu(cin, cout):
    return nn.Sequential(nn.ConvTranspose2d(cin, cout, 4, stride=2, padding=1, bias=True), nn.LeakyReLU())


def _he_init(module):
    for m in module.modules():
        if isinstance(m, (nn.Conv2d, nn.Conv3d)):
            fan = int(np.prod(m.kernel_size)) * m.out_channels
            m.weight.data.normal_(0, math.sqrt(2.0 / fan))
        elif isinstance(m, (nn.BatchNorm2d, nn.BatchNorm3d)):
            m.weight.data.fill_(1)
            m.bias.data.zero_()



def _no_kernel(what):
    from ._lib import NrgbdError
    return NrgbdError("no hand-written kernel for " + what)


class _Act(object):
    __slots__ = ("z", "ss", "relu", "r", "r_ss", "r_relu")

    def __init__(self, z, ss=None, relu=False, r=None, r_ss=None, r_relu=False):
        self.z, self.ss, self.relu, self.r, self.r_ss, self.r_relu = z, ss, relu, r, r_ss, r_relu


_PACKERS = {
    "taps": lambda ops, w: ops.conv_pack_weights(w),
    "s2": lambda ops, w: ops.conv_s2_pack(w),
    "pc": lambda ops, w: ops.conv_wino_pack32(w) if w.shape[0] == 32 and w.dim() == 4 else ops.conv_wino_pack(w),
    "dw": lambda ops, w: ops.conv_wino_dw_pack(w),
    "dw4": lambda ops, w: ops.conv_wino_dw4_pack(w),
    "direct": lambda ops, w: ops.conv3d_pack_weights(w),
    "cout1": lambda ops, w: w[0].reshape(w.shape[1], 27).t().contiguous(),
}


def padded_channels(c):
    return -(-int(c) // 16) * 16


def pad_input_channels(w, cin):
    if cin == w.shape[1]:
        return w
    return torch.cat((w, w.new_zeros((w.shape[0], cin - w.shape[1]) + tuple(w.shape[2:]))), dim=1)


def _packed(owner, conv, kind, mult=1.0, cin=None):
    from . import ops
    cache = owner.__dict__.setdefault("_wp_cache", {})
    w = conv.weight
    cin = int(w.shape[1] if cin is None else cin)
    key = (w.data_ptr(), w._version, str(w.device), float(mult), cin)
    hit = cache.get((kind, id(conv)))
    if hit is None or hit[0] != key:
        wc = pad_input_channels(w.detach(), cin).contiguous()
        hit = (key, _PACKERS[kind](ops, wc if mult == 1.0 else wc * float(mult)))
        cache[(kind, id(conv))] = hit
    return hit[1]


def _relu_unit(owner, bn, count):
    from . import ops
    if not (bn.training or not bn.track_running_stats) or not bn.affine:
        return 0.0
    cache = owner.__dict__.setdefault("_wp_cache", {})
    key = (bn.weight.data_ptr(), bn.weight._version, bn.bias.data_ptr(), bn.bias._version, int(count))
    hit = cache.get(("unit", id(bn)))
    if hit is None or hit[0] != key:
        hit = (key, ops.relu_unit(bn.weight, bn.bias, count))
        cache[("unit", id(bn))] = hit
    return hit[1]


def invalidate_packed_weights(module):
    for m in module.modules():
        m.__dict__.pop("_wp_cache", None)
        m.__dict__.pop("_pk_cache", None)


class _PackedWeightsMixin(object):

    def load_state_dict(self, *a, **k):
        out = super().load_state_dict(*a, **k)
        invalidate_packed_weights(self)
        return out

    def _apply(self, fn, *a, **k):
        out = super()._apply(fn, *a, **k)
        invalidate_packed_weights(self)
        return out


_status_words = {}


def status_word(device):
    key = str(device)
    w = _status_words.get(key)
    if w is None:
        w = torch.zeros(1, dtype=torch.int32, device=device)
        _status_words[key] = w
    return w


def check_status(device):
    w = _status_words.get(str(device))
    if w is None:
        return
    n = int(w.clone().item())
    if n:
        w.zero_()
# ... 84 lines not shown


class PSMFeatures(_PackedWeightsMixin, nn.Module):

    SPP_WINDOWS = (64, 32, 16, 8)

    def __init__(self, feature_dim=32, bn_running_avg=False, multi_scale=False):
        super().__init__()
        self.multi_scale = multi_scale
        t = bn_running_avg
        self.firstconv = nn.Sequential(
            _conv_bn2d(3, 32, 3, 2, 1, 1, t), nn.ReLU(inplace=True),
            _conv_bn2d(32, 32, 3, 1, 1, 1, t), nn.ReLU(inplace=True),
            _conv_bn2d(32, 32, 3, 1, 1, 1, t), nn.ReLU(inplace=True),
        )
        self._width = 32
        self.layer1 = self._stage(32, 3, 1, 1, 1)
        self.layer2 = self._stage(64, 16, 2, 1, 1)
        self.layer3 = self._stage(128, 3, 1, 1, 1)
        self.layer4 = self._stage(128, 3, 1, 1, 2)
        for i, win in enumerate(self.SPP_WINDOWS, start=1):
            setattr(self, "branch%d" % i, nn.Sequential(
                nn.AvgPool2d((win, win), stride=(win, win)),
                _conv_bn2d(128, 32, 1, 1, 0, 1, t), nn.ReLU(inplace=True)))
        self.lastconv = nn.Sequential(
            _conv_bn2d(320, 128, 3, 1, 1, 1, t), nn.ReLU(inplace=True),
            nn.Conv2d(128, feature_dim, 1, padding=0, stride=1, bias=False))

    def _stage(self, width, n_blocks, stride, pad, dilation):
        shortcut = None
        if stride != 1 or self._width != width:
            shortcut = nn.Sequential(nn.Conv2d(self._width, width, 1, stride=stride, bias=False),
                                     nn.BatchNorm2d(width))
        blocks = [ResBlock2d(self._width, width, stride, shortcut, pad, dilation)]
        self._width = width
        blocks += [ResBlock2d(width, width, 1, None, pad, dilation) for _ in range(n_blocks - 1)]
        return nn.Sequential(*blocks)

    def _spp_pools(self, deep):
        if _fused_ok(deep) and deep.shape[2] % 8 == 0 and deep.shape[3] % 8 == 0:
            from . import ops
            p8 = ops.avgpool8(deep)
            return {8: p8, 16: F.avg_pool2d(p8, 2), 32: F.avg_pool2d(p8, 4), 64: F.avg_pool2d(p8, 8)}
        if deep.is_cuda and torch.is_grad_enabled():
            N, C, H, W = deep.shape
            out = {}
            for k in self.SPP_WINDOWS:
                ph, pw = H // k, W // k
                out[k] = deep[:, :, :ph * k, :pw * k].reshape(N, C, ph, k, pw, k).mean((3, 5))
            return out
        return {w: F.avg_pool2d(deep, (w, w), stride=(w, w)) for w in self.SPP_WINDOWS}


    def _upsample(self, y, size):
        if y.is_cuda and torch.is_grad_enabled() and y.dtype == torch.float32 and y.shape[1] % 4 == 0 and y.shape[1] <= 256:
            from .autograd import UpsampleBilinearCL
            return UpsampleBilinearCL.apply(y, int(size[0]), int(size[1]))
        return F.interpolate(y, size=size, mode="bilinear", align_corners=True)

    _MFMA_SHAPES = {(32, 1), (64, 1), (128, 1), (128, 2)}

    def _conv_bn_cl(self, seq, a, relu, materialize=False):
        from . import ops
        conv, bn = seq[0], seq[1]
        d = conv.dilation[0]
        mfma = (conv.kernel_size == (3, 3) and conv.stride == (1, 1) and conv.padding == (d, d)
                and conv.in_channels % 16 == 0 and (conv.out_channels, d) in self._MFMA_SHAPES)
        wino = (mfma and conv.in_channels % 32 == 0 and ((d in (1, 2) and conv.out_channels % 64 == 0) or (d == 1 and conv.out_channels == 32))
                and ops.conv_wino_supported(a.z.shape[0], a.z.shape[1], a.z.shape[2], conv.in_channels, conv.out_channels, 1))
        if wino:
            z, st, mat = ops.conv_wino(a.z, _packed(self, conv, "pc"), conv.out_channels, 1, d, x_ss=a.ss, x_relu=a.relu,
                                       res=a.r, res_ss=a.r_ss, res_relu=a.r_relu, materialize=materialize,
                                       want_stats=_needs_stats(bn))
        elif mfma:
            z, st, mat = ops.conv2d(a.z, _packed(self, conv, "taps"), conv.out_channels, d, x_ss=a.ss, x_relu=a.relu,
                                    res=a.r, res_ss=a.r_ss, res_relu=a.r_relu, materialize=materialize,
                                    want_stats=_needs_stats(bn))
        else:
            mat = a.z if (a.ss is None and a.r is None and not a.relu) else \
                ops.nhwc_act(a.z, a.ss, a.relu, a.r, a.r_ss, a.r_relu)
            s2 = (conv.kernel_size == (3, 3) and conv.stride == (2, 2) and conv.padding == (1, 1) and d == 1
                  and mat.shape[1] % 2 == 0 and mat.shape[2] % 2 == 0 and conv.out_channels in (32, 64))
            if s2:
                z, st = ops.conv2d_taps(ops.space_to_depth2(mat), _packed(self, conv, "s2"), conv.out_channels, 4,
                                        want_stats=_needs_stats(bn))
            else:
                raise _no_kernel("feature CNN layer %d -> %d, kernel %s, stride %s, dilation %d on a %d x %d map" % (
                    conv.in_channels, conv.out_channels, tuple(conv.kernel_size), tuple(conv.stride), d, mat.shape[1], mat.shape[2]))
        count = z.shape[0] * z.shape[1] * z.shape[2]
        return _Act(z, _bn_scale_shift(bn, st, count, "cm" if wino else "rows"), relu), mat

    def _pointwise_cl(self, conv, m, stride=1, want_stats=False):
        from . import ops
        N, H, W, C = m.shape
        if C % 16 != 0 or conv.out_channels not in (32, 64, 128) or H % stride or W % stride:
            raise _no_kernel("1x1 layer %d -> %d, stride %d on a %d x %d map" % (C, conv.out_channels, stride, H, W))
        return ops.conv2d_taps(m.contiguous(), _packed(self, conv, "taps"), conv.out_channels, 1, want_stats=want_stats, stride=stride)

    def _pointwise_bn_cl(self, seq, m, stride=1):
        conv, bn = seq[0], seq[1]
        z, st = self._pointwise_cl(conv, m, stride, want_stats=_needs_stats(bn))
        return _Act(z, _bn_scale_shift(bn, st, z.shape[0] * z.shape[1] * z.shape[2]), False)

    def _block_cl(self, blk, a):
        y1, m = self._conv_bn_cl(blk.conv1[0], a, relu=True, materialize=True)
        y2, _ = self._conv_bn_cl(blk.conv2, y1, relu=False)
        if blk.downsample is None:
            return _Act(y2.z, y2.ss, False, r=m)
        sk = self._pointwise_bn_cl(blk.downsample, m, blk.downsample[0].stride[0])
        return _Act(y2.z, y2.ss, False, r=sk.z, r_ss=sk.ss)

    def fused_ok(self, x):
        return x.is_cuda and not torch.is_grad_enabled() and x.dtype == torch.float32

    def forward_channels_last(self, x):
        from . import ops
        conv, bn = self.firstconv[0]
        if x.shape[2] % 4 or x.shape[3] % 4:
            raise _no_kernel("image %d x %d: the plane-sweep grid is the image / 4 (models/basic.py:254-263), both sides must be multiples of 4"
                             % (x.shape[2], x.shape[3]))
        z, st = ops.conv2d_taps(ops.space_to_depth2(x.contiguous(), nchw=True), _packed(self, conv, "s2"), conv.out_channels, 4,
                                want_stats=_needs_stats(bn))
        a = _Act(z, _bn_scale_shift(bn, st, z.numel() // z.shape[-1]), True)
        for i in (2, 4):
            a, _ = self._conv_bn_cl(self.firstconv[i], a, relu=True)
        for blk in self.layer1:
            a = self._block_cl(blk, a)
        half = ops.nhwc_act(a.z, a.ss, a.relu, a.r, a.r_ss, a.r_relu)
        a = _Act(half)
        for blk in self.layer2:
            a = self._block_cl(blk, a)
        quarter = None
        for k, blk in enumerate(self.layer3):
            y1, m = self._conv_bn_cl(blk.conv1[0], a, relu=True, materialize=True)
            if k == 0:
                quarter = m
            y2, _ = self._conv_bn_cl(blk.conv2, y1, relu=False)
            if blk.downsample is None:
                a = _Act(y2.z, y2.ss, False, r=m)
            else:
                sk = self._pointwise_bn_cl(blk.downsample, m, blk.downsample[0].stride[0])
                a = _Act(y2.z, y2.ss, False, r=sk.z, r_ss=sk.ss)
        for blk in self.layer4:
            a = self._block_cl(blk, a)
        deep = ops.nhwc_act(a.z, a.ss, a.relu, a.r, a.r_ss, a.r_relu)
        N, h, w, _ = deep.shape
        if h < 64 or w < 64:
            raise _no_kernel("an SPP window of 64 on a %d x %d map (psm_submodule.py:100: images below 256 x 256)" % (h, w))
        if h % 8 == 0 and w % 8 == 0:
            p8 = ops.avgpool_cl(deep, 8)
            p16 = ops.avgpool_cl(p8, 2)
            p32 = ops.avgpool_cl(p16, 2)
            pools = {8: p8, 16: p16, 32: p32, 64: ops.avgpool_cl(p32, 2)}
        else:
            pools = {k: ops.avgpool_cl(deep, k) for k in self.SPP_WINDOWS}
        zs, norms = [], []
        for i in (4, 3, 2, 1):
            branch = getattr(self, "branch%d" % i)
            z, _ = self._pointwise_cl(branch[1][0], pools[self.SPP_WINDOWS[i - 1]])
            zs.append(z)
            norms.append(branch[1][1])
        sss = _bn_scale_shift_small(norms, zs)
        cat = ops.spp_concat(quarter, deep, list(zip(zs, sss)))
        y, _ = self._conv_bn_cl(self.lastconv[0], _Act(cat), relu=True)
        head = self.lastconv[2]
        if head.out_channels not in (32, 64, 128):
            raise _no_kernel("feature_dim %d (1x1 head): 32, 64 or 128" % head.out_channels)
        feat, _ = ops.conv2d_taps(y.z, _packed(self, head, "taps"), head.out_channels, 1, x_ss=y.ss, x_relu=True, want_stats=False)
        return half, feat

    def forward(self, x):
        if x.is_cuda:
            x = x.contiguous(memory_format=torch.channels_last)
        stem = x
        for i in (0, 2, 4):
            stem = _conv_bn_act(stem, self.firstconv[i], relu=True)
        half = self.layer1(stem)
        quarter = self.layer2(half)
        deep = self.layer4(self.layer3(quarter))
        size = deep.shape[2:]
        pools = self._spp_pools(deep)
        pyramid = []
        for i in (4, 3, 2, 1):
            branch = getattr(self, "branch%d" % i)
            y = _conv_bn_act(pools[self.SPP_WINDOWS[i - 1]], branch[1], relu=True)
            pyramid.append(self._upsample(y, size))
        y = _conv_bn_act(torch.cat([quarter, deep] + pyramid, dim=1), self.lastconv[0], relu=True)
        if y.is_cuda:
            from .autograd import conv2d_module
            feat = conv2d_module(self.lastconv[2], y)
        else:
            feat = self.lastconv[2](y)
        return (half, feat) if self.multi_scale else feat


class FeatureExtractor(nn.Module):

    def __init__(self, feature_dim=32, bn_running_avg=False, multi_scale=False):
        super().__init__()
        self.feature_extraction = PSMFeatures(feature_dim, bn_running_avg, multi_scale)
        self.multi_scale = multi_scale
        _he_init(self)

    def forward(self, img):
        return self.feature_extraction(img)
# ... 108 lines not shown
        L = self._layers()

        def cbr(x_cl, i, relu, res=None):
            conv, bn = L[i]
            return batch_norm_act_cl(Conv3dCL.apply(x_cl, conv.weight, id(conv.weight), grad_channel if i == 0 else None), bn, relu, res)

        x = cbr(vol, 0, True)
        x = cbr(x, 1, True)
        for i in (2, 4, 6, 8):
            x = cbr(cbr(x, i, True), i + 1, False, x)
        y = cbr(x, 10, True)
        w1 = L[11][0].weight
        if w1.shape[1] == 64 and y.is_cuda:
            return Conv3dCout1CL.apply(y, w1, id(w1))
        w_pad = torch.cat((w1, w1.new_zeros(63, *w1.shape[1:])), dim=0)
        return Conv3dCL.apply(y, w_pad, id(w1))[..., 0]

    def forward(self, volume):
        if volume.shape[1] != self.in_channels:
            raise AssertionError("Input volume should have correct # of channels !")
        x = self.dres0(volume.contiguous())
        for i in (1, 2, 3, 4):
            x = getattr(self, "dres%d" % i)(x) + x
        out = self.classify(x)
        if self.if_normalize:
            out = F.log_softmax(out, dim=2)
        if self.up_sample_ratio is not None:
            d, h, w = volume.shape[2:]
            out = F.interpolate(out, (self.up_sample_ratio * d, h, w), mode="trilinear", align_corners=True)
        return out


class DPVUpsampleNet(_PackedWeightsMixin, nn.Module):

    def __init__(self, C0, C1, C2, D=64, upsample_D=False):
        super().__init__()
        cin = D + C0
        D0 = 2 * D if upsample_D else D
        D1 = 2 * D0 if upsample_D else D
        self.conv0 = _conv_lrelu(cin, cin)
        self.conv0_1 = _conv_lrelu(cin, cin)
        self.trans_conv0 = _deconv_lrelu(cin, D0)
        self.conv1 = _conv_lrelu(D0 + C1, D0 + C1)
        self.conv1_1 = _conv_lrelu(D0 + C1, D0 + C1)
        self.trans_conv1 = _deconv_lrelu(D0 + C1, D1)
        self.conv2 = _conv_lrelu(D1 + C2, D1 + C2)
        self.conv2_1 = _conv_lrelu(D1 + C2, D1)
        self.conv2_2 = nn.Conv2d(D1, D1, kernel_size=3, stride=1, padding=1, bias=True)
        self._init()

    def _init(self):
        for m in self.modules():
            if isinstance(m, nn.Conv2d):
                fan = m.kernel_size[0] * m.kernel_size[1] * m.out_channels
                m.weight.data.normal_(0, math.sqrt(2.0 / fan))
            elif isinstance(m, nn.ConvTranspose2d):
                n = m.kernel_size[1]
                factor = (n + 1) // 2
                center = factor - 1 if n % 2 == 1 else factor - 0.5
                og = np.ogrid[:n, :n]
                bil = (1 - abs(og[0] - center) / factor) * (1 - abs(og[1] - center) / factor)
                m.weight.data.copy_(torch.from_numpy(bil))

    def _widths(self):
        D = self.conv2_2.out_channels
        C0 = self.conv0[0].in_channels - D
        C1 = self.conv1[0].in_channels - D
        C2 = self.conv2[0].in_channels - D
        ok = 1 <= D <= 128 and (C0, C1, C2) == (64, 32, 3) and self.trans_conv0[0].out_channels == D \
            and self.trans_conv1[0].out_channels == D and self.conv2_1[0].out_channels == D
        return (D, 64 if D <= 64 else 128, C0, C1, C2) if ok else None

    def _levels(self):
        wd = self._widths()
        if wd is not None:
            return ((wd[0], wd[1]),) * 3
        D = self.conv0[0].in_channels - 64
        D0, D1 = self.trans_conv0[0].out_channels, self.conv2_2.out_channels
        ok = D in (32, 64) and (D0, D1) == (2 * D, 4 * D) and self.conv1[0].in_channels == D0 + 32 \
            and self.trans_conv1[0].out_channels == D1 and self.conv2[0].in_channels == D1 + 3 and self.conv2_1[0].out_channels == D1
        return ((D, 64), (D0, D0), (D1, D1)) if ok else None

    deconv_kernels = ("wino", "direct")
    _FEATS = (64, 32, 3)

    def mfma_ok(self, dpv):
        return dpv.is_cuda and not torch.is_grad_enabled() and dpv.dtype == torch.float32

    def _embedded(self):
        lv = self._levels()
        C0, C1, C2 = self._FEATS
        mods = {"conv0": self.conv0[0], "conv0_1": self.conv0_1[0], "trans_conv0": self.trans_conv0[0], "conv1": self.conv1[0],
                "conv1_1": self.conv1_1[0], "trans_conv1": self.trans_conv1[0], "conv2": self.conv2[0], "conv2_1": self.conv2_1[0],
                "conv2_2": self.conv2_2}
        if all(d == dp for d, dp in lv):
            return {k: (m.weight.detach(), m.bias.detach()) for k, m in mods.items()}
        dev = self.conv2_2.weight.device
        cat = lambda l, C: (torch.cat((torch.arange(lv[l][0], device=dev), lv[l][1] + torch.arange(C, device=dev))), lv[l][1] + C)
        plain = lambda l: (torch.arange(lv[l][0], device=dev), lv[l][1])
        io = {"conv0": cat(0, C0) + cat(0, C0), "conv0_1": cat(0, C0) + cat(0, C0), "trans_conv0": cat(0, C0) + plain(1),
              "conv1": cat(1, C1) + cat(1, C1), "conv1_1": cat(1, C1) + cat(1, C1), "trans_conv1": cat(1, C1) + plain(2),
              "conv2": cat(2, C2) + cat(2, C2), "conv2_1": cat(2, C2) + plain(2), "conv2_2": plain(2) + plain(2)}
        out = {}
        for k, m in mods.items():
            in_idx, cin_p, out_idx, cout_p = io[k]
            w, b = m.weight.detach(), m.bias.detach()
            tr = isinstance(m, nn.ConvTranspose2d)
            if tr:
                w = w.transpose(0, 1)
            t = w.new_zeros((w.shape[0], cin_p) + tuple(w.shape[2:]))
            t[:, in_idx] = w
            wp = w.new_zeros((cout_p, cin_p) + tuple(w.shape[2:]))
            wp[out_idx] = t
            bp = b.new_full((cout_p,), -1e30 if k == "conv2_2" else 0.0)
            bp[out_idx] = b
            out[k] = ((wp.transpose(0, 1) if tr else wp).contiguous(), bp)
        return out

    def _rnet_packed(self):
        from . import ops
        cache = self.__dict__.setdefault("_pk_cache", {})
        key = tuple((p.data_ptr(), p._version) for p in self.parameters())
        if cache.get("key") == key:
            return cache["val"]
        pad16 = lambda c: (c + 15) // 16 * 16
        pad32 = pad16
        emb = self._embedded()

        def deconv(name):
            w, b = emb[name]
            res = {}
            for pa in (0, 1):
                for pb in (0, 1):
                    ky = [3, 1] if pa == 0 else [2, 0]
                    kx = [3, 1] if pb == 0 else [2, 0]
                    wph = w[:, :, ky][:, :, :, kx].permute(1, 0, 2, 3)
                    res[(pa, pb)] = [(ops.conv_pack_weights(wph[c0:c0 + 64].contiguous()), b[c0:c0 + 64].contiguous(), 64, c0, 64)
                                     for c0 in range(0, w.shape[1], 64)]
            res["all"] = [(torch.cat([res[(pa, pb)][i][0] for pa in (0, 1) for pb in (0, 1)]),) + res[(0, 0)][i][1:]
                          for i in range(len(res[(0, 0)]))]
            cin_p = pad16(w.shape[0])
            res["wino"] = None
            if cin_p % 32 == 0 and w.shape[1] % 64 == 0:
                wi = w.new_zeros((cin_p,) + tuple(w.shape[1:]))
                wi[:w.shape[0]] = w
                res["wino"] = [(ops.conv_wino_rnet_deconv_pack(ops.conv_wino_pack(ops.deconv_phase_weights(wi[:, c0:c0 + 64])), cin_p),
                                b[c0:c0 + 64].contiguous(), 64, c0, 64) for c0 in range(0, w.shape[1], 64)]
            return res

        def wino(name):
            w, b = emb[name]
            cin_p, cout_p = pad32(w.shape[1]), (w.shape[0] + 63) // 64 * 64
            wp = w.new_zeros(cout_p, cin_p, 3, 3)
            wp[:w.shape[0], :w.shape[1]] = w
            bp = b.new_zeros(cout_p)
            bp[:w.shape[0]] = b
            extra = w.shape[0] % 64
            if 0 < extra <= 4 and w.shape[0] > 64:
                full = w.shape[0] - extra
                few = wp[full:full + extra].reshape(extra, cin_p // 16, 16, 9).permute(1, 3, 0, 2).contiguous()
                return (ops.conv_wino_pack(wp[:full].contiguous()), bp[:full].contiguous(), full, full,
                        ("few", few, bp[full:full + extra].contiguous(), extra, full))
            if 0 < extra <= 32 and w.shape[0] > 64:
                full = w.shape[0] - extra
                tail = wp.new_zeros(64, cin_p, 3, 3)
                tail[:extra] = wp[full:full + extra]
                return (ops.conv_wino_pack(wp[:full].contiguous()), bp[:full].contiguous(), full, full,
                        (ops.conv_wino_pack(tail), bp[full:full + 32].contiguous(), 32, extra, full))
            return (ops.conv_wino_pack(wp.contiguous()), bp.contiguous(), cout_p, w.shape[0])

        val = {"t0": deconv("trans_conv0"), "t1": deconv("trans_conv1")}
        for name in ("conv0", "conv0_1", "conv1", "conv1_1", "conv2", "conv2_1", "conv2_2"):
            val[name + "_w"] = wino(name)
        cache["key"], cache["val"] = key, val
        return val

    def _rnet_buffers(self, n, h, w, dev):
        cache = self.__dict__.setdefault("_buf_cache", {})
        key = (n, h, w, str(dev))
        if key not in cache:
            for k in [k for k in cache if k[1:] != key[1:]]:
                del cache[k]
            (D, Dp), (_, Dp1), (_, Dp2) = self._levels()
            C0, C1, C2 = self._FEATS
            z = lambda *shape: torch.zeros(shape, dtype=torch.float32, device=dev)
            p32 = lambda c: (c + 15) // 16 * 16
            w0, w1, w2 = p32(Dp + C0), p32(Dp1 + C1), p32(Dp2 + C2)
            cache[key] = {"x0": z(n, h, w, w0), "a0": z(n, h, w, w0), "b0": z(n, h, w, w0),
                          "c1": z(n, 2 * h, 2 * w, w1), "a1": z(n, 2 * h, 2 * w, w1), "b1": z(n, 2 * h, 2 * w, w1),
                          "c2": z(n, 4 * h, 4 * w, w2), "g2": z(n, 4 * h, 4 * w, w2), "h2": z(n, 4 * h, 4 * w, Dp2)}
            if D != Dp:
                cache[key]["dpv"] = torch.full((n, Dp, h, w), float("-inf"), dtype=torch.float32, device=dev)
        return cache[key]

    def forward_log(self, dpv_log, img_features):
        first = dpv_log[0] if isinstance(dpv_log, (list, tuple)) else dpv_log
        if not self.mfma_ok(first):
            if isinstance(dpv_log, (list, tuple)):
                dpv_log = torch.cat(list(dpv_log), dim=0)
            return self.forward(torch.exp(dpv_log), img_features)
        from . import ops
        lv = self._levels()
        if lv is None:
            raise _no_kernel("this R-Net (image-feature widths other than 64 / 32 / 3, more than 128 candidates, or candidate "
                             "up-sampling from other than 32 or 64 candidates)")
        (D, Dp), (_, Dp1), (Dl, Dpl) = lv
        quarter, half, full = img_features
        if isinstance(dpv_log, (list, tuple)):
            vols = [v[i:i + 1] for v in dpv_log for i in range(v.shape[0])]
        else:
            vols = [dpv_log[i:i + 1] for i in range(dpv_log.shape[0])]
        n = len(vols)
        _, _, h, w = vols[0].shape
        if n > 2:
            return torch.cat([self.forward_log(vols[i:i + 2], img_features).clone() for i in range(0, n, 2)], dim=0)
        if tuple(quarter.shape) != (1, 64, h, w) or tuple(half.shape) != (1, 32, 2 * h, 2 * w) or tuple(full.shape) != (1, 3, 4 * h, 4 * w):
            raise ValueError("forward_log: features of ONE image at 1/4, 1/2 and full resolution ([1,64,h,w], [1,32,2h,2w], [1,3,4h,4w]) expected")
        dev = first.device
        pk, buf = self._rnet_packed(), self._rnet_buffers(n, h, w, dev)

        def deconv(x, layer, out):
            wino = self.deconv_kernels[0] == "wino" and layer["wino"] is not None \
                and ops.conv_wino_rnet_deconv_supported(x.shape[0], x.shape[1], x.shape[2], x.shape[3], out.shape[-1])
            for wp, bias, wdt, c0, valid in layer["wino" if wino else "all"]:
                if wino:
                    ops.conv_wino_rnet_deconv(x, wp, out, bias=bias, ycoff=c0, cout_valid=valid)
                else:
                    ops.conv2d_rnet(x, wp, wdt, bias=bias, out=out, ldy=out.shape[-1], ycoff=c0, cout_valid=valid, mode=3)
            return out

        def conv_w(x, name, out=None, lrelu=True):
            wt = pk[name + "_w"]
            out = ops.conv_wino_rnet(x, wt[0], wt[2], bias=wt[1], lrelu=lrelu, out=out, cout_valid=wt[3])
            if len(wt) > 4:
                t = wt[4]
                if t[0] == "few":
                    ops.conv2d_few(x, t[1], bias=t[2], lrelu=lrelu, out=out, ycoff=t[4])
                else:
                    ops.conv_wino_rnet(x, t[0], t[2], bias=t[1], lrelu=lrelu, out=out, ycoff=t[4], cout_valid=t[3])
            return out

        if D != Dp:
            for b in range(n):
                buf["dpv"][b, :D].copy_(vols[b][0])
            vols = [buf["dpv"][b:b + 1] for b in range(n)]
        q_cl = quarter.permute(0, 2, 3, 1)
        x = buf["x0"]
        for b in range(n):
            if q_cl.is_contiguous():
                ops.rnet_pack(vols[b][0].contiguous(), q_cl[0], feat_planar=False, out=x[b:b + 1])
            else:
                ops.rnet_pack(vols[b][0].contiguous(), quarter[0].contiguous(), feat_planar=True, out=x[b:b + 1])
        x = conv_w(conv_w(x, "conv0", buf["a0"]), "conv0_1", buf["b0"])
        c1 = buf["c1"]
        deconv(x, pk["t0"], c1)
        ops.scatter_channels(half[0], c1, Dp1)
        x = conv_w(conv_w(c1, "conv1", buf["a1"]), "conv1_1", buf["b1"])
        c2 = buf["c2"]
        deconv(x, pk["t1"], c2)
        ops.scatter_channels(full[0], c2, Dpl)
        x = conv_w(conv_w(c2, "conv2", buf["g2"]), "conv2_1", buf["h2"])
        y = ops.logsoftmax_rows(conv_w(x, "conv2_2", None, lrelu=False)).permute(0, 3, 1, 2)
        return y if Dl == Dpl else y[:, :Dl]

    def forward(self, dpv_raw, img_features):
        quarter, half, full = img_features
        from .autograd import LogSoftmaxCL, cat_cl, conv2d_module, conv_transpose2d_module, padded_in_width

        def cl(m, x):
            return conv2d_module(m[0], x, act_slope=0.01)

        def tl(m, x):
            return conv_transpose2d_module(m[0], x, act_slope=0.01)
        x = cl(self.conv0_1, cl(self.conv0, cat_cl([dpv_raw, quarter], padded_in_width(self.conv0[0]))))
        x = tl(self.trans_conv0, x)
        x = cl(self.conv1_1, cl(self.conv1, cat_cl([x, half], padded_in_width(self.conv1[0]))))
        x = tl(self.trans_conv1, x)
        x = conv2d_module(self.conv2[0], cat_cl([x, full], padded_in_width(self.conv2[0])), keep_width=True, act_slope=0.01)
        x = conv2d_module(self.conv2_2, cl(self.conv2_1, x))
        if LogSoftmaxCL.supported(x) and x.permute(0, 2, 3, 1).is_contiguous():
            return LogSoftmaxCL.apply(x)
        return torch.log_softmax(x, dim=1)


def dgf_host(dmap, img_guide, w1, b1, w2, b2, eps=1e-8):
    n, _, h, w = dmap.shape
    H, W = img_guide.shape[2:]
    dt, dev = dmap.dtype, dmap.device

    def table(lo, hi):
        num = torch.arange(hi, dtype=torch.int64, device=dev) * (lo - 1)
        i0 = num // (hi - 1)
        lam = (num % (hi - 1)).to(dt) / float(hi - 1)
        return i0, torch.clamp(i0 + 1, max=lo - 1), lam
    r0, r1, lr = table(h, H)
    c0, c1, lc = table(w, W)
    lr, lc = lr.view(1, 1, H, 1), lc.view(1, 1, 1, W)
    top, bot = dmap[:, :, r0], dmap[:, :, r1]
    y = (1 - lr) * ((1 - lc) * top[..., c0] + lc * top[..., c1]) + lr * ((1 - lc) * bot[..., c0] + lc * bot[..., c1])
    x = F.conv2d(torch.relu(F.conv2d(img_guide.to(dt), w1.reshape(64, 3, 1, 1).to(dt), b1.reshape(64).to(dt))),
                 w2.reshape(1, 64, 1, 1).to(dt), b2.reshape(1).to(dt))

    def window(t):
        p = F.pad(t, (1, 1, 1, 1))
        return torch.stack([p[..., dy:dy + H, dx:dx + W] for dy in range(3) for dx in range(3)])
    inside = window(torch.ones((1, 1, H, W), dtype=dt, device=dev))
    N = inside.sum(0)
    wx, wy = window(x), window(y)
    mx, my = wx.sum(0) / N, wy.sum(0) / N
    cx, cy = (wx - mx) * inside, (wy - my) * inside
    A = ((cx * cy).sum(0) / N) / ((cx * cx).sum(0) / N + eps)
    b = my - A * mx
    return (window(A).sum(0) / N) * x + window(b).sum(0) / N


class DGFRefineNet(nn.Module):

    def __init__(self, in_channels):
        super().__init__()
        if in_channels != 3:
# ... 32 lines not shown
```

### neuralrgbd_amd/ops.py

```python
import ctypes
import typing

import numpy as np
import torch

from . import _lib

DIST = {"L2": 0, "L1": 1}
GENERATION = {None: 0, "auto": 0, "gather": 1, "lds": 2, "quad": 3}


def _need(t, name, shape=None, strided=False):
    if not isinstance(t, torch.Tensor):
        raise TypeError("%s must be a torch.Tensor" % name)
    if not t.is_cuda:
        raise _lib.NrgbdError("%s is on %s: the plane-sweep path runs on the GPU only "
                              "(no CPU fallback)" % (name, t.device))
    if t.dtype != torch.float32:
        raise TypeError("%s must be float32, got %s" % (name, t.dtype))
    if shape is not None and tuple(t.shape) != tuple(shape):
        raise ValueError("%s has shape %s, expected %s" % (name, tuple(t.shape), tuple(shape)))
    return t if (strided or t.is_contiguous()) else t.contiguous()


# ... 652 lines not shown
        rc = _lib.load().nrgbd_conv3d_cout1_dgrad_f32(_p(gy), _p(w_tap_major), _p(gx), D, H, W, _stream(gy))
    _lib.check(rc, "nrgbd_conv3d_cout1_dgrad_f32")
    return gx


def conv3d_cout1_wgrad(x, gy):
    x = _need(x, "x")
    D, H, W, Cin = x.shape
    if Cin != 64:
        raise ValueError("conv3d_cout1_wgrad: 64 input channels, got %d" % Cin)
    gy = _need(gy, "gy", (D, H, W))
    lib = _lib.load()
    dw = torch.empty((1, 64, 3, 3, 3), dtype=torch.float32, device=x.device)
    with torch.cuda.device(x.device):
        nbytes = ctypes.c_size_t(0)
        _lib.check(lib.nrgbd_conv3d_cout1_wgrad_workspace(D, H, W, ctypes.byref(nbytes)), "nrgbd_conv3d_cout1_wgrad_workspace")
        ws = torch.empty(nbytes.value, dtype=torch.uint8, device=x.device)
        rc = lib.nrgbd_conv3d_cout1_wgrad_f32(_p(x), _p(gy), _p(dw), _p(ws), ctypes.c_size_t(ws.numel()), D, H, W, _stream(x))
    _lib.check(rc, "nrgbd_conv3d_cout1_wgrad_f32")
    return dw


def _status_ptr(status, like):
    if status is None:
        return ctypes.c_void_p(0)
    if not (isinstance(status, torch.Tensor) and status.is_cuda and status.dtype == torch.int32 and status.numel() >= 1 and status.device == like.device):
        raise TypeError("status must be an int32 tensor on the device of the statistics")
    return ctypes.c_void_p(status.data_ptr())


def _nbt_ptr(nbt, like):
    if nbt is None:
        return ctypes.c_void_p(0)
    if not (isinstance(nbt, torch.Tensor) and nbt.is_cuda and nbt.dtype == torch.int64 and nbt.numel() == 1 and nbt.device == like.device):
        raise TypeError("batches_tracked must be an int64 scalar tensor on the device of the statistics")
    return ctypes.c_void_p(nbt.data_ptr())


def bn3d_finalize(stats, count, gamma, beta, eps, momentum, running_mean=None, running_var=None, status=None, batches_tracked=None):
    stats = _need(stats, "stats")
    ss = torch.empty((64, 2), dtype=torch.float32, device=stats.device)
    with torch.cuda.device(stats.device):
        rc = _lib.load().nrgbd_bn3d_finalize(_p(stats), stats.shape[0], int(count), _p(gamma), _p(beta), float(eps),
                                             float(momentum), _p(running_mean), _p(running_var), _p(ss), _status_ptr(status, stats), _nbt_ptr(batches_tracked, stats),
                                             _stream(stats))
    _lib.check(rc, "nrgbd_bn3d_finalize")
    return ss


def conv2d_workgroups(N, H, W):
    return int(_lib.load().nrgbd_conv2d_workgroups(N, H, W))


def conv_pack_weights(w):
    w = _need(w, "w")
    cout, cin = w.shape[:2]
    taps = 1
    for k in w.shape[2:]:
        taps *= int(k)
    wp = torch.empty(taps * cin * cout, dtype=torch.float32, device=w.device)
    with torch.cuda.device(w.device):
        rc = _lib.load().nrgbd_conv_pack_weights(_p(w), _p(wp), cin, cout, taps, _stream(w))
    _lib.check(rc, "nrgbd_conv_pack_weights")
    return wp


def conv2d(x, w_packed, cout, dilation=1, x_ss=None, x_relu=False, res=None, res_ss=None, res_relu=False,
           materialize=False, bias=None, out_lrelu=False, want_stats=True):
    x = _need(x, "x")
    N, H, W, Cin = x.shape
    y = torch.empty((N, H, W, cout), dtype=torch.float32, device=x.device)
    stats = torch.empty((conv2d_workgroups(N, H, W), 2 * cout), dtype=torch.float32, device=x.device) if want_stats else None
    mat = torch.empty_like(x) if materialize else None
    if res is not None:
        res = _need(res, "res", x.shape)
    with torch.cuda.device(x.device):
        rc = _lib.load().nrgbd_conv2d_3x3_f32(_p(x), _p(x_ss), int(x_relu), _p(res), _p(res_ss), int(res_relu), _p(mat),
                                               _p(w_packed), _p(bias), int(out_lrelu), _p(y), _p(stats), N, H, W, Cin,
                                               int(cout), int(dilation), _stream(x))
    _lib.check(rc, "nrgbd_conv2d_3x3_f32")
    return y, stats, mat


def conv_s2_pack(w, cp=None):
    w = _need(w, "w")
    return conv_pack_weights(conv_s2_weights(w, cp))


def conv_s2_weights(w, cp=None):
    cout, c = w.shape[:2]
    cp = cp or -(-4 * c // 16) * 16
    w2 = torch.zeros((cout, cp, 2, 2), dtype=w.dtype, device=w.device)
    kmap = {(0, 1): 0, (1, 0): 1, (1, 1): 2}
    for (ty, py), ky in kmap.items():
        for (tx, px), kx in kmap.items():
            ph = py * 2 + px
            w2[:, ph * c:(ph + 1) * c, ty, tx] = w[:, :, ky, kx]
    return w2


def space_to_depth2(x, nchw=False, cp=None):
    x = _need(x, "x")
    if nchw:
        N, C, H, W = x.shape
    else:
        N, H, W, C = x.shape
    cp = cp or -(-4 * C // 16) * 16
    y = torch.empty((N, H // 2, W // 2, cp), dtype=torch.float32, device=x.device)
    with torch.cuda.device(x.device):
        rc = _lib.load().nrgbd_space_to_depth2(_p(x), int(nchw), _p(y), N, C, H, W, cp, _stream(x))
    _lib.check(rc, "nrgbd_space_to_depth2")
    return y


def conv2d_taps(x, w_packed, cout, taps, x_ss=None, x_relu=False, want_stats=True, stride=1):
    x = _need(x, "x")
    N, H, W, Cin = x.shape
    if stride != 1:
        if taps != 1 or H % stride or W % stride:
            raise ValueError("conv2d_taps: a stride needs taps = 1 and sides that are multiples of it")
        H, W = H // stride, W // stride
    y = torch.empty((N, H, W, cout), dtype=torch.float32, device=x.device)
    stats = torch.empty((conv2d_workgroups(N, H, W), 2 * cout), dtype=torch.float32, device=x.device) if want_stats else None
    with torch.cuda.device(x.device):
        rc = _lib.load().nrgbd_conv2d_taps_f32(_p(x), _p(x_ss), int(x_relu), _p(w_packed), _p(y), _p(stats), N, H, W, Cin,
                                                int(cout), int(taps), int(stride), _stream(x))
    _lib.check(rc, "nrgbd_conv2d_taps_f32")
    return y, stats


def conv2d_wgrad(x, gy, dilation=1):
    x = _need(x, "x")
    N, H, W, Cin = x.shape
    gy = _need(gy, "gy")
    Cout = gy.shape[-1]
    if tuple(gy.shape[:3]) != (N, H, W):
        raise ValueError("conv2d_wgrad: gy %s does not match x %s" % (tuple(gy.shape), tuple(x.shape)))
    lib = _lib.load()
    nwg = int(lib.nrgbd_conv2d_wgrad_workgroups(N, H, W, Cin, Cout))
    _lib.check(min(nwg, 0), "nrgbd_conv2d_wgrad_workgroups")
    blocks = -(-Cout // 64) * -(-Cin // 64)
    partial = torch.empty(blocks * nwg * 9 * 64 * 64, dtype=torch.float32, device=x.device)
    dw = torch.empty((Cout, Cin, 3, 3), dtype=torch.float32, device=x.device)
    with torch.cuda.device(x.device):
        rc = lib.nrgbd_conv2d_wgrad_f32(_p(x), _p(gy), _p(partial), _p(dw), N, H, W, Cin, Cout, int(dilation), _stream(x))
    _lib.check(rc, "nrgbd_conv2d_wgrad_f32")
    return dw


def conv2d_rnet(x, w_packed, cout, bias=None, lrelu=True, out=None, ldy=None, ycoff=0, cout_valid=None, mode=0, pa=0, pb=0):
    x = _need(x, "x")
    N, H, W, Cin = x.shape
    cv = cout if cout_valid is None else cout_valid
    if mode == 2:
        out = torch.empty((N, cout, H, W), dtype=torch.float32, device=x.device)
        ldy = cout
    elif out is None:
        if mode in (1, 3):
            raise ValueError("conv2d_rnet: a transposed conv writes into a caller-provided [N,2H,2W,ldy] buffer")
        out = torch.empty((N, H, W, cv), dtype=torch.float32, device=x.device)
        ldy = cv
    elif ldy is None:
        ldy = out.shape[-1]
    with torch.cuda.device(x.device):
        rc = _lib.load().nrgbd_conv2d_rnet_f32(_p(x), _p(w_packed), _p(bias), int(bool(lrelu)), _p(out), int(ldy), int(ycoff),
                                                int(cv), int(mode), int(pa), int(pb), N, H, W, Cin, int(cout), _stream(x))
    _lib.check(rc, "nrgbd_conv2d_rnet_f32")
    return out


def rnet_pack(dpv_log, feat, feat_planar, out=None):
    dpv_log = _need(dpv_log, "dpv_log")
    feat = _need(feat, "feat")
    D, h, w = dpv_log.shape
    Cf = feat.shape[0] if feat_planar else feat.shape[-1]
    if out is None:
        out = torch.empty((1, h, w, D + Cf), dtype=torch.float32, device=dpv_log.device)
    elif tuple(out.shape) != (1, h, w, D + Cf) or not out.is_contiguous():
        raise ValueError("rnet_pack: out must be a contiguous [1,h,w,D+Cf] tensor")
    with torch.cuda.device(dpv_log.device):
        rc = _lib.load().nrgbd_rnet_pack(_p(dpv_log), _p(feat), int(bool(feat_planar)), _p(out), D, Cf, h * w, _stream(dpv_log))
    _lib.check(rc, "nrgbd_rnet_pack")
    return out


def bn_finalize(stats, count, gamma, beta, eps, momentum, running_mean=None, running_var=None, status=None, batches_tracked=None):
    stats = _need(stats, "stats")
    C = stats.shape[1] // 2
    ss = torch.empty((C, 2), dtype=torch.float32, device=stats.device)
    with torch.cuda.device(stats.device):
        rc = _lib.load().nrgbd_bn_finalize(_p(stats), stats.shape[0], C, int(count), _p(gamma), _p(beta), float(eps),
                                           float(momentum), _p(running_mean), _p(running_var), _p(ss), _status_ptr(status, stats), _nbt_ptr(batches_tracked, stats),
                                           _stream(stats))
    _lib.check(rc, "nrgbd_bn_finalize")
    return ss


def bn_small_stats(xs, gammas, betas, eps, momentum, running_means=None, running_vars=None, batches_tracked=None):
    n = len(xs)
    if not 1 <= n <= 4 or len(gammas) != n or len(betas) != n:
        raise ValueError("bn_small_stats: 1 to 4 maps with one gamma and beta each, got %d / %d / %d" % (n, len(gammas), len(betas)))
    xs = [_need(x, "x") for x in xs]
    C = xs[0].shape[-1]
    if any(x.shape[-1] != C for x in xs):
        raise ValueError("bn_small_stats: the maps must share one channel count, got %s" % [tuple(x.shape) for x in xs])
    per = lambda v: [float(u) for u in v] if isinstance(v, (list, tuple)) else [float(v)] * n
    eps, momentum = per(eps), per(momentum)
    rms = list(running_means) if running_means is not None else [None] * n
    rvs = list(running_vars) if running_vars is not None else [None] * n
    nbts = list(batches_tracked) if batches_tracked is not None else [None] * n
    if len(eps) != n or len(momentum) != n or len(rms) != n or len(rvs) != n or len(nbts) != n:
        raise ValueError("bn_small_stats: one eps / momentum / running statistic per map")
    dev = xs[0].device
    ss = [torch.empty((C, 2), dtype=torch.float32, device=dev) for _ in range(n)]
    ptrs = lambda ts: (ctypes.c_void_p * n)(*[0 if t is None else t.data_ptr() for t in ts])
    gammas = [_need(g, "gamma", (C,)) for g in gammas]
    betas = [_need(b, "beta", (C,)) for b in betas]
    for i in range(n):
        if (rms[i] is None) != (rvs[i] is None):
            raise ValueError("bn_small_stats: running_mean and running_var come together")
        for t, name in ((rms[i], "running_mean"), (rvs[i], "running_var")):
            if t is not None and _need(t, name, (C,)) is not t:
                raise ValueError("bn_small_stats: %s must be contiguous (it is updated in place)" % name)
        _nbt_ptr(nbts[i], xs[i])
    keep = (ptrs(xs), (ctypes.c_long * n)(*[x.numel() // C for x in xs]), ptrs(gammas), ptrs(betas), (ctypes.c_float * n)(*eps),
            (ctypes.c_float * n)(*momentum), ptrs(rms), ptrs(rvs), ptrs(nbts), ptrs(ss))
    with torch.cuda.device(dev):
        rc = _lib.load().nrgbd_bn_small_stats(n, *[ctypes.cast(a, ctypes.c_void_p) for a in keep[:2]], int(C),
                                          *[ctypes.cast(a, ctypes.c_void_p) for a in keep[2:]], _stream(xs[0]))
    _lib.check(rc, "nrgbd_bn_small_stats")
    return ss


def conv_wino_rnet(x, w_wino, cout, bias=None, lrelu=True, out=None, ycoff=0, cout_valid=None):
    x = _need(x, "x")
    N, H, W, Cin = x.shape
    valid = int(cout if cout_valid is None else cout_valid)
    if out is None:
        out = torch.empty((N, H, W, valid), dtype=torch.float32, device=x.device)
    elif tuple(out.shape[:3]) != (N, H, W) or not out.is_contiguous() or out.shape[3] < ycoff + valid:
        raise ValueError("conv_wino_rnet: out must be a contiguous [N,H,W,>= ycoff + cout_valid] tensor")
    with torch.cuda.device(x.device):
        rc = _lib.load().nrgbd_conv_wino_rnet_ex_f32(_p(x), _p(w_wino), _p(bias), int(bool(lrelu)), _p(out), N, H, W, Cin, int(cout),
                                                      int(out.shape[3]), int(ycoff), valid, _stream(x))
    _lib.check(rc, "nrgbd_conv_wino_rnet_ex_f32")
    return out


def deconv_phase_weights(w):
    from .autograd import _tap_select
    cin, cout = w.shape[:2]
    idx, msk = _tap_select("t2", w.device)
    w4 = w.detach().permute(1, 0, 2, 3).reshape(cout, cin, 16).index_select(2, idx) * msk
    return w4.reshape(cout, cin, 4, 9).permute(2, 0, 1, 3).reshape(4 * cout, cin, 3, 3).contiguous()


def deconv_live_points(phase):
    a, b = phase >> 1, phase & 1
    return [4 * (r + a) + c + b for r in range(3) for c in range(3)]


def conv_wino_rnet_deconv_pack(w_wino, Cin):
    w_wino = _need(w_wino, "w_wino")
    if w_wino.numel() != 256 * Cin * 16:
        raise ValueError("conv_wino_rnet_deconv_pack: a 256-column stream of %d input channels expected" % Cin)
    wm = torch.empty(4 * (Cin // 16) * 9 * 1024, dtype=torch.float32, device=w_wino.device)
    with torch.cuda.device(w_wino.device):
        rc = _lib.load().nrgbd_conv_wino_rnet_deconv_pack(_p(w_wino), _p(wm), int(Cin), _stream(w_wino))
    _lib.check(rc, "nrgbd_conv_wino_rnet_deconv_pack")
    return wm


def conv_wino_rnet_deconv_supported(N, H, W, Cin, ldy):
    return Cin >= 32 and Cin % 32 == 0 and N * H * W * Cin < (1 << 30) and 4 * N * H * W * ldy < (1 << 31)


def conv_wino_rnet_deconv(x, w_masked, out, bias=None, lrelu=True, ycoff=0, cout_valid=64):
    x = _need(x, "x")
    N, H, W, Cin = x.shape
    if tuple(out.shape[:3]) != (N, 2 * H, 2 * W) or not out.is_contiguous() or out.shape[3] < ycoff + cout_valid:
        raise ValueError("conv_wino_rnet_deconv: out must be a contiguous [N,2H,2W,>= ycoff + cout_valid] tensor")
    if w_masked.numel() != 4 * (Cin // 16) * 9 * 1024:
        raise ValueError("conv_wino_rnet_deconv: the masked stream does not belong to %d input channels" % Cin)
    with torch.cuda.device(x.device):
        rc = _lib.load().nrgbd_conv_wino_rnet_deconv_f32(_p(x), _p(w_masked), _p(bias), int(bool(lrelu)), _p(out), N, H, W, Cin, 64,
                                                          int(out.shape[3]), int(ycoff), int(cout_valid), _stream(x))
    _lib.check(rc, "nrgbd_conv_wino_rnet_deconv_f32")
    return out


def conv2d_few(x, w_few, bias=None, lrelu=True, out=None, ycoff=0):
    x = _need(x, "x")
    w_few = _need(w_few, "w_few")
    N, H, W, ldx = x.shape
    nblk, taps, cout, lanes = w_few.shape
    if taps != 9 or lanes != 16 or not 1 <= cout <= 4 or nblk * 16 > ldx:
        raise ValueError("conv2d_few: w_few %s for an input of %d channels" % (tuple(w_few.shape), ldx))
    if out is None:
        out = torch.empty((N, H, W, cout), dtype=torch.float32, device=x.device)
    elif tuple(out.shape[:3]) != (N, H, W) or not out.is_contiguous() or out.shape[3] < ycoff + cout:
        raise ValueError("conv2d_few: out must be a contiguous [N,H,W,>= ycoff + Cout] tensor")
    with torch.cuda.device(x.device):
        rc = _lib.load().nrgbd_conv2d_few_f32(_p(x), int(ldx), _p(w_few), _p(bias), int(bool(lrelu)), _p(out), int(out.shape[3]), int(ycoff),
                                               N, H, W, nblk * 16, cout, _stream(x))
    _lib.check(rc, "nrgbd_conv2d_few_f32")
    return out


def bn_cl_supported(rows, C):
    return rows > 0 and 4 <= C <= 1024 and C % 4 == 0 and 256 % (C // 4) == 0


def bn_cl_fwd(x, gamma, beta, eps, relu, residual=None, momentum=0.0, running_mean=None, running_var=None):
    x = _need(x, "x")
    rows, C = x.shape
    if residual is not None:
        residual = _need(residual, "residual", (rows, C))
    y = torch.empty_like(x)
    coef = torch.empty((4, C), dtype=torch.float32, device=x.device)
    with torch.cuda.device(x.device):
        lib = _lib.load()
        G = lib.nrgbd_bn_cl_workgroups(rows, C)
        _lib.check(min(G, 0), "nrgbd_bn_cl_workgroups")
        partial = torch.empty((G, 2 * C), dtype=torch.float32, device=x.device)
        rc = lib.nrgbd_bn_cl_fwd(_p(x), _p(residual), _p(_need(gamma, "gamma", (C,))), _p(_need(beta, "beta", (C,))), float(eps),
                                 float(momentum), _p(running_mean), _p(running_var), int(bool(relu)), _p(y), _p(coef), _p(partial),
                                 rows, C, _stream(x))
    _lib.check(rc, "nrgbd_bn_cl_fwd")
    return y, coef


def bn_cl_bwd(x, gy, coef, relu):
    x = _need(x, "x")
    rows, C = x.shape
    gy = _need(gy, "gy", (rows, C))
    coef = _need(coef, "coef", (4, C))
    gx = torch.empty_like(x)
    gg = torch.empty((2, C), dtype=torch.float32, device=x.device)
    coef2 = torch.empty((2, C), dtype=torch.float32, device=x.device)
    with torch.cuda.device(x.device):
        lib = _lib.load()
        G = lib.nrgbd_bn_cl_workgroups(rows, C)
        _lib.check(min(G, 0), "nrgbd_bn_cl_workgroups")
        partial = torch.empty((G, 2 * C), dtype=torch.float32, device=x.device)
        rc = lib.nrgbd_bn_cl_bwd(_p(x), _p(gy), _p(coef), int(bool(relu)), _p(gx), _p(gg[0]), _p(gg[1]), _p(coef2), _p(partial),
                                 rows, C, _stream(x))
    _lib.check(rc, "nrgbd_bn_cl_bwd")
    return gx, gg[0], gg[1]


def bn_finalize_cm(stats, count, gamma, beta, eps, momentum, running_mean=None, running_var=None, status=None, batches_tracked=None):
    stats = _need(stats, "stats")
    C = stats.shape[0] // 2
    ss = torch.empty((C, 2), dtype=torch.float32, device=stats.device)
    with torch.cuda.device(stats.device):
        rc = _lib.load().nrgbd_bn_finalize_cm(_p(stats), stats.shape[1], C, int(count), _p(gamma), _p(beta), float(eps),
                                              float(momentum), _p(running_mean), _p(running_var), _p(ss), _status_ptr(status, stats), _nbt_ptr(batches_tracked, stats),
                                              _stream(stats))
    _lib.check(rc, "nrgbd_bn_finalize_cm")
    return ss


def logsoftmax_rows(x, inplace=True):
    x = _need(x, "x")
    C = x.shape[-1]
    y = x if inplace else torch.empty_like(x)
    with torch.cuda.device(x.device):
        rc = _lib.load().nrgbd_logsoftmax_rows(_p(x), _p(y), x.numel() // C, int(C), _stream(x))
    _lib.check(rc, "nrgbd_logsoftmax_rows")
    return y


def logsoftmax_d_bwd(logp, g, scale=1.0):
    logp = _need(logp, "logp")
    g = _need(g, "g", logp.shape)
    D = logp.shape[0]
    gz = torch.empty_like(logp)
    with torch.cuda.device(logp.device):
        rc = _lib.load().nrgbd_logsoftmax_d_bwd(_p(logp), _p(g), float(scale), _p(gz), D, logp.numel() // D, _stream(logp))
    _lib.check(rc, "nrgbd_logsoftmax_d_bwd")
    return gz


def logsoftmax_rows_bwd(y, g):
    y = _need(y, "y")
    g = _need(g, "g", y.shape)
    C = y.shape[-1]
    gx = torch.empty_like(y)
# ... 985 lines not shown
```

Before: 32.31 frames/s.

## Skip structurally-zero weight steps in stride-2 trunk, rnet last K block, and few-conv

Adds 'live' variants of three convolutions. They skip MFMA steps, channel words and weight lines that are structurally zero: from space-to-depth padding in the stride-2 trunk layers, and from channel padding in the refinement net's last K block and in its few-output convolution. Compile-time masks drive an unrolled walk over only the live steps, and the weight streams are repacked to drop the dead lines. This cuts wasted MFMA, LDS and global traffic. The cost is more template instantiations, validation of the masks, and a restructured prefetch schedule.

```diff
diff --git a/include/nrgbd.h b/include/nrgbd.h
--- a/include/nrgbd.h
+++ b/include/nrgbd.h
@@ -167,6 +167,8 @@
 int nrgbd_avgpool_cl(const float* x, float* y, int N, int H, int W, int C, int k, void* stream);
 int nrgbd_conv2d_few_f32(const float* x, int ldx, const float* w_packed, const float* bias, int out_lrelu, float* y, int ldy,
                          int ycoff, int N, int H, int W, int Cin, int Cout, void* stream);
+int nrgbd_conv2d_few_live_f32(const float* x, int ldx, const float* w_packed, const float* bias, int out_lrelu, float* y, int ldy,
+                              int ycoff, int N, int H, int W, int Cin, int Cout, int last_words, void* stream);
 int nrgbd_scatter_channels(const float* src, long stride_c, long stride_y, long stride_x, int C, int H, int W, float* dst,
                            int ldy, int coff, int n_rep, long rep_stride, void* stream);
 int nrgbd_bias_act_nchw(float* x, const float* bias, float slope, int N, int C, long HW, void* stream);
@@ -176,6 +178,9 @@
                              int N, int H, int W, int Cin, int Cout, void* stream);
 int nrgbd_conv_wino_rnet_ex_f32(const float* x, const float* w_wino, const float* bias, int out_lrelu, float* y,
                                 int N, int H, int W, int Cin, int Cout, int ldy, int ycoff, int cout_valid, void* stream);
+int nrgbd_conv_wino_rnet_live_f32(const float* x, const float* w_wino, const float* bias, int out_lrelu, float* y,
+                                  int N, int H, int W, int Cin, int Cout, int ldy, int ycoff, int cout_valid, int k_live_last, void* stream);
+int nrgbd_conv_wino_last_k_steps(int width);
 int nrgbd_conv_wino_rnet_deconv_f32(const float* x, const float* w_masked, const float* bias, int out_lrelu, float* y,
                                     int N, int H, int W, int Cin, int Cout, int ldy, int ycoff, int cout_valid, void* stream);
 int nrgbd_conv_wino_rnet_deconv_pack(const float* w_wino, float* w_masked, int Cin, void* stream);
@@ -208,6 +213,8 @@
 int nrgbd_conv2d_taps_f32(const float* x, const float* x_ss, int x_relu, const float* w_packed, float* y, float* stats,
                           int N, int H, int W, int Cin, int Cout, int taps, int in_stride, void* stream);
 int nrgbd_space_to_depth2(const float* x, int nchw, float* y, int N, int C, int H, int W, int Cp, void* stream);
+int nrgbd_conv2d_taps_live_f32(const float* x, const float* x_ss, int x_relu, const float* w_packed, float* y, float* stats,
+                               int N, int H, int W, int Cin, int Cout, const unsigned* live, void* stream);
 int nrgbd_conv2d_wgrad_workgroups(int N, int H, int W, int Cin, int Cout);
 int nrgbd_conv2d_wgrad_f32(const float* x, const float* gy, float* partial, float* dw, int N, int H, int W, int Cin, int Cout,
                            int dilation, void* stream);
diff --git a/neuralrgbd_amd/_lib.py b/neuralrgbd_amd/_lib.py
--- a/neuralrgbd_amd/_lib.py
+++ b/neuralrgbd_amd/_lib.py
@@ -82,6 +82,8 @@
     "nrgbd_conv_wino_tiles": (_I, [_I, _I, _I, _I]),
     "nrgbd_conv_wino_rnet_f32": (_I, [_P, _P, _P, _I, _P, _I, _I, _I, _I, _I, _P]),
     "nrgbd_conv_wino_rnet_ex_f32": (_I, [_P, _P, _P, _I, _P, _I, _I, _I, _I, _I, _I, _I, _I, _P]),
+    "nrgbd_conv_wino_rnet_live_f32": (_I, [_P, _P, _P, _I, _P, _I, _I, _I, _I, _I, _I, _I, _I, _I, _P]),
+    "nrgbd_conv_wino_last_k_steps": (_I, [_I]),
     "nrgbd_conv_wino_rnet_deconv_f32": (_I, [_P, _P, _P, _I, _P, _I, _I, _I, _I, _I, _I, _I, _I, _P]),
     "nrgbd_conv_wino_rnet_deconv_pack": (_I, [_P, _P, _I, _P]),
     "nrgbd_conv_wino_pack": (_I, [_P, _P, _I, _I, _I, _I, _P]),
@@ -102,6 +104,7 @@
     "nrgbd_bn2d_train_act": (_I, [_P, _P, _P, _F, _I, _P, _P, _P, _P, _I, _I, _L, _P]),
     "nrgbd_avgpool8": (_I, [_P, _P, _I, _I, _I, _P]),
     "nrgbd_conv2d_few_f32": (_I, [_P, _I, _P, _P, _I, _P, _I, _I, _I, _I, _I, _I, _I, _P]),
+    "nrgbd_conv2d_few_live_f32": (_I, [_P, _I, _P, _P, _I, _P, _I, _I, _I, _I, _I, _I, _I, _I, _P]),
     "nrgbd_avgpool_cl": (_I, [_P, _P, _I, _I, _I, _I, _I, _P]),
     "nrgbd_scatter_channels": (_I, [_P, _L, _L, _L, _I, _I, _I, _P, _I, _I, _I, _L, _P]),
     "nrgbd_bias_act_nchw": (_I, [_P, _P, _F, _I, _I, _L, _P]),
@@ -109,6 +112,7 @@
     "nrgbd_conv2d_wgrad_workgroups": (_I, [_I, _I, _I, _I, _I]),
     "nrgbd_conv2d_wgrad_f32": (_I, [_P, _P, _P, _P, _I, _I, _I, _I, _I, _I, _P]),
     "nrgbd_conv2d_taps_f32": (_I, [_P, _P, _I, _P, _P, _P, _I, _I, _I, _I, _I, _I, _I, _P]),
+    "nrgbd_conv2d_taps_live_f32": (_I, [_P, _P, _I, _P, _P, _P, _I, _I, _I, _I, _I, _P, _P]),
     "nrgbd_space_to_depth2": (_I, [_P, _I, _P, _I, _I, _I, _I, _I, _P]),
     "nrgbd_conv_pack_weights": (_I, [_P, _P, _I, _I, _I, _P]),
     "nrgbd_conv2d_3x3_f32": (_I, [_P, _P, _I, _P, _P, _I, _P, _P, _P, _I, _P, _P, _I, _I, _I, _I, _I, _I, _P]),
diff --git a/neuralrgbd_amd/csrc/conv2d.hip b/neuralrgbd_amd/csrc/conv2d.hip
--- a/neuralrgbd_amd/csrc/conv2d.hip
+++ b/neuralrgbd_amd/csrc/conv2d.hip
@@ -1,5 +1,7 @@
 #include <cstdint>
 #include <cstdlib>
+#include <type_traits>
+#include <utility>
 
 #include "conv_tile.hpp"
 
@@ -29,8 +31,30 @@
     int xs;
 };
 
-template <int COUT, int DIL, bool RES, int NTAP = 9, int EPI = 0>
+constexpr unsigned kLiveAll = 0xFFFFFFFFu;
+constexpr unsigned kLiveS2a = 0xFF000000u, kLiveS2b = 0xFFFF0000u, kLiveS2c = 0xFF00FF00u;
+constexpr unsigned kLiveS2Rgb = 0xFF3ECF0Eu;
+__host__ __device__ constexpr int live_steps(unsigned m) {
+    int n = 0;
+    for (int s = 0; s < 8; ++s) n += ((m >> (4 * s)) & 15u) != 0;
+    return n;
+}
+__host__ __device__ constexpr int live_step(unsigned m, int j) {
+    for (int s = 0; s < 8; ++s)
+        if ((m >> (4 * s)) & 15u) {
+            if (j == 0) return s;
+            --j;
+        }
+    return -1;
+}
+template <class F, int... I>
+__device__ __forceinline__ void static_for_impl(F&& f, std::integer_sequence<int, I...>) { (f(std::integral_constant<int, I>{}), ...); }
+template <int N, class F>
+__device__ __forceinline__ void static_for(F&& f) { static_for_impl(f, std::make_integer_sequence<int, N>{}); }
+
+template <int COUT, int DIL, bool RES, int NTAP = 9, int EPI = 0, bool LIVE = false>
 __global__ __launch_bounds__(256, COUT <= 32 ? 3 : 2) void conv2d_mfma_kernel(const Conv2dArgs a) {
+    static_assert(!LIVE || (NTAP == 4 && !RES && EPI == 0 && (COUT == 32 || COUT == 64)), "the live walk: the trunk's stride-2 layers");
     constexpr int HS = kT2 + 2 * DIL, HALO = HS * HS;
     constexpr int NPF = (HALO * (kCB / 4) + 255) / 256;
     constexpr int NF = COUT / 32;
@@ -92,6 +116,99 @@
         if constexpr (RES) prer[u] = *reinterpret_cast<const f32x4*>(a.res + pf_off[u]);
     }
 
+    if constexpr (LIVE) {
+        constexpr int BD = 3, NB = BD + 1;
+        const f32x4* wl = reinterpret_cast<const f32x4*>(wpk) + lane;
+        auto block = [&](int cblk, auto mask) __attribute__((always_inline)) {
+            {
+                const int c = cblk * kCB + c4 * 4;
+                float ss[8] = {1.f, 0.f, 1.f, 0.f, 1.f, 0.f, 1.f, 0.f};
+                if (a.x_ss) {
+#pragma unroll
+                    for (int e = 0; e < 8; ++e) ss[e] = a.x_ss[2 * c + e];
+                }
+#pragma unroll
+                for (int u = 0; u < NPF; ++u) {
+                    const int hv = (tid >> 2) + 64 * u;
+                    if (hv >= HALO) continue;
+                    f32x4 v = {0.f, 0.f, 0.f, 0.f};
+                    if ((pf_ok >> u) & 1u) {
+                        v = pre[u];
+                        if (a.x_ss) {
+                            v.x = __builtin_fmaf(v.x, ss[0], ss[1]); v.y = __builtin_fmaf(v.y, ss[2], ss[3]);
+                            v.z = __builtin_fmaf(v.z, ss[4], ss[5]); v.w = __builtin_fmaf(v.w, ss[6], ss[7]);
+                        }
+                        if (a.x_relu) { v.x = fmaxf(v.x, 0.f); v.y = fmaxf(v.y, 0.f); v.z = fmaxf(v.z, 0.f); v.w = fmaxf(v.w, 0.f); }
+                    }
+                    *reinterpret_cast<f32x4*>(lds + lds_slot(hv, c4)) = v;
+                }
+            }
+            __syncthreads();
+            f32x4 Bn[NB][NF], An[2][2];
+        const unsigned nb = (cblk + 1) * kCB;
+        const bool more = cblk + 1 < ncblk;
+        constexpr unsigned M = decltype(mask)::value;
+        constexpr int NL = live_steps(M), BDL = NL <= NB ? NL : BD;
+        static_assert(NL <= NB || NL >= NPF + 1, "the next block's words have no steps to go to");
+#pragma unroll
+        for (int b = 0; b < BDL; ++b)
+#pragma unroll
+            for (int f = 0; f < NF; ++f) Bn[b][f] = wl[(b * NF + f) * 64];
+        {
+            constexpr int s0 = live_step(M, 0), tap = s0 / G4, g = s0 % G4, voff = (tap >> 1) * HS + (tap & 1);
+            int h0 = hv0;
+            asm volatile("" : "+v"(h0));
+            An[0][0] = *reinterpret_cast<const f32x4*>(lds + lds_slot(h0 + voff, khalf * 2 + g));
+            An[0][1] = *reinterpret_cast<const f32x4*>(lds + lds_slot(h0 + 2 * HS + voff, khalf * 2 + g));
+        }
+        static_for<NL>([&](auto jc) __attribute__((always_inline)) {
+            constexpr int j = decltype(jc)::value, s = live_step(M, j), cur = j & 1, nxt = cur ^ 1;
+            if constexpr (j + 1 < NL) {
+                constexpr int s1 = live_step(M, j + 1), tap = s1 / G4, g = s1 % G4, voff = (tap >> 1) * HS + (tap & 1);
+                int h0 = hv0;
+                asm volatile("" : "+v"(h0));
+                An[nxt][0] = *reinterpret_cast<const f32x4*>(lds + lds_slot(h0 + voff, khalf * 2 + g));
+                An[nxt][1] = *reinterpret_cast<const f32x4*>(lds + lds_slot(h0 + 2 * HS + voff, khalf * 2 + g));
+            }
+            if constexpr (j + BDL < NL) {
+#pragma unroll
+                for (int f = 0; f < NF; ++f) Bn[(j + BDL) % NB][f] = wl[((j + BDL) * NF + f) * 64];
+            }
+            if constexpr (NL >= NPF + 1) {
+                if constexpr (j >= NL - NPF) {
+                    if (more) pre[j - (NL - NPF)] = *reinterpret_cast<const f32x4*>(a.x + pf_off[j - (NL - NPF)] + nb);
+                }
+            } else if constexpr (j == 0) {
+                if (more) {
+#pragma unroll
+                    for (int u = 0; u < NPF; ++u) pre[u] = *reinterpret_cast<const f32x4*>(a.x + pf_off[u] + nb);
+                }
+            }
+#pragma unroll
+            for (int e = 0; e < 4; ++e) {
+                if ((M >> (4 * s + e)) & 1u) {
+#pragma unroll
+                    for (int m = 0; m < 2; ++m)
+#pragma unroll
+                        for (int f = 0; f < NF; ++f)
+                            acc[m][f] = __builtin_amdgcn_mfma_f32_32x32x2f32(An[cur][m][e], Bn[j % NB][f][e], acc[m][f], 0, 0, 0);
+                }
+            }
+        });
+        wl += NL * NF * 64;
+            __syncthreads();
+        };
+        if constexpr (COUT == 32) {
+            block(0, std::integral_constant<unsigned, kLiveS2Rgb>{});
+        } else {
+            const int q = ncblk >> 2;
+            int cblk = 0;
+            for (; cblk < q; ++cblk) block(cblk, std::integral_constant<unsigned, kLiveS2a>{});
+            for (; cblk < 2 * q; ++cblk) block(cblk, std::integral_constant<unsigned, kLiveS2b>{});
+            for (; cblk < 3 * q; ++cblk) block(cblk, std::integral_constant<unsigned, kLiveS2c>{});
+            for (; cblk < ncblk; ++cblk) block(cblk, std::integral_constant<unsigned, kLiveAll>{});
+        }
+    } else {
     const int wstep = ncblk * (G4 * NF * 64);
     for (int cblk = 0; cblk < ncblk; ++cblk) {
         {
@@ -196,6 +313,8 @@
         __syncthreads();
     }
 
+    }
+
     float s1[NF], s2[NF], bs[NF];
 #pragma unroll
     for (int f = 0; f < NF; ++f) { s1[f] = 0.f; s2[f] = 0.f; bs[f] = a.bias ? a.bias[f * 32 + i] : 0.f; }
@@ -460,6 +579,12 @@
     const size_t lds = (size_t)HS * HS * kSV * sizeof(float);
     hipLaunchKernelGGL((conv2d_mfma_kernel<COUT, 1, false, NTAP, 0>), dim3(nwg), dim3(256), lds, st, a);
 }
+template <int COUT>
+static void launch_conv2d_live(const Conv2dArgs& a, int nwg, hipStream_t st) {
+    constexpr int HS = kT2 + 2;
+    const size_t lds = (size_t)HS * HS * kSV * sizeof(float);
+    hipLaunchKernelGGL((conv2d_mfma_kernel<COUT, 1, false, 4, 0, true>), dim3(nwg), dim3(256), lds, st, a);
+}
 
 __global__ __launch_bounds__(256) void space_to_depth2_kernel(const float* __restrict__ x, int nchw, float* __restrict__ y,
                                                               int N, int C, int H, int W, int Cp) {
@@ -569,6 +694,25 @@
         else if (Cout == 64) launch_conv2d_taps<64, 4>(a, nwg, st);
         else return NRGBD_E_SHAPE;
     }
+    NRGBD_CHECK_LAUNCH();
+    return NRGBD_OK;
+}
+
+extern "C" int nrgbd_conv2d_taps_live_f32(const float* x, const float* x_ss, int x_relu, const float* w_packed, float* y, float* stats,
+                                          int N, int H, int W, int Cin, int Cout, const unsigned* live, void* stream) {
+    using namespace nrgbd;
+    if (!live) return nrgbd_conv2d_taps_f32(x, x_ss, x_relu, w_packed, y, stats, N, H, W, Cin, Cout, 4, 1, stream);
+    if (!x || !w_packed || !y) return NRGBD_E_NULL;
+    if (N <= 0 || H <= 0 || W <= 0 || (Cout != 32 && Cout != 64) || (Cout == 32 ? Cin != kCB : (Cin <= 0 || Cin % (4 * kCB)))) return NRGBD_E_SHAPE;
+    if ((long)N * H * W * Cin >= (1L << 32)) return NRGBD_E_SHAPE;
+    Conv2dArgs a{x, x_ss, nullptr, nullptr, nullptr, w_packed, nullptr, y, stats, x_relu, 0, 0, N, H, W, Cin,
+                 0, Cout, 0, Cout, 0, 0, 0, nullptr, 1};
+    const unsigned group[4] = {kLiveS2a, kLiveS2b, kLiveS2c, kLiveAll};
+    for (int c = 0, q = Cin / (4 * kCB); c < Cin / kCB; ++c)
+        if (live[c] != (Cout == 32 ? kLiveS2Rgb : group[c / q])) return NRGBD_E_ARG;
+    const int nwg = ceil_div(W, kT2) * ceil_div(H, kT2) * N;
+    if (Cout == 32) launch_conv2d_live<32>(a, nwg, (hipStream_t)stream);
+    else launch_conv2d_live<64>(a, nwg, (hipStream_t)stream);
     NRGBD_CHECK_LAUNCH();
     return NRGBD_OK;
 }
diff --git a/neuralrgbd_amd/csrc/conv_few.hip b/neuralrgbd_amd/csrc/conv_few.hip
--- a/neuralrgbd_amd/csrc/conv_few.hip
+++ b/neuralrgbd_amd/csrc/conv_few.hip
@@ -1,3 +1,5 @@
+#include <type_traits>
+
 #include "common.hpp"
 
 namespace nrgbd {
@@ -14,6 +16,7 @@
     const float* bias;
     float* y;
     int N, H, W, Cin, ldx, ldy, ycoff, lrelu;
+    int last_words;
 };
 
 template <int CO>
@@ -39,17 +42,25 @@
         off[u] = in ? (unsigned)((((size_t)n * a.H + gy) * a.W + gx) * a.ldx + c4 * 4) : (unsigned)(c4 * 4);
         if (in) ok |= 1u << u;
     }
+    auto word_live = [&](int c) { return c4 < (c + 1 == nblk ? a.last_words : 4); };
     f32x4 pre[kFewNPF];
+    auto fetch = [&](int c) {
+        if (word_live(c)) {
 #pragma unroll
-    for (int u = 0; u < kFewNPF; ++u) pre[u] = *reinterpret_cast<const f32x4*>(a.x + off[u]);
-    auto publish = [&](int buf) {
-#pragma unroll
-        for (int u = 0; u < kFewNPF; ++u) {
-            const int hv = (tid >> 2) + 64 * u;
-            if (hv < kFewHalo)
-                *reinterpret_cast<f32x4*>(&tile[buf][hv * kFewPitch + c4 * 4]) = ((ok >> u) & 1u) ? pre[u] : f32x4{0.f, 0.f, 0.f, 0.f};
+            for (int u = 0; u < kFewNPF; ++u) pre[u] = *reinterpret_cast<const f32x4*>(a.x + off[u] + c * 16);
         }
     };
+    auto publish = [&](int c) {
+        if (word_live(c)) {
+#pragma unroll
+            for (int u = 0; u < kFewNPF; ++u) {
+                const int hv = (tid >> 2) + 64 * u;
+                if (hv < kFewHalo)
+                    *reinterpret_cast<f32x4*>(&tile[0][hv * kFewPitch + c4 * 4]) = ((ok >> u) & 1u) ? pre[u] : f32x4{0.f, 0.f, 0.f, 0.f};
+            }
+        }
+    };
+    fetch(0);
     publish(0);
     __syncthreads();
 
@@ -57,27 +68,22 @@
 #pragma unroll
     for (int co = 0; co < CO; ++co) acc[co] = a.bias ? a.bias[co] : 0.f;
 
-    for (int c = 0; c < nblk; ++c) {
-        constexpr int buf = 0;
-        if (c + 1 < nblk) {
-#pragma unroll
-            for (int u = 0; u < kFewNPF; ++u) pre[u] = *reinterpret_cast<const f32x4*>(a.x + off[u] + (c + 1) * 16);
-        }
-        const float* w = a.wp + (size_t)c * (9 * CO * 16);
+    auto block = [&](const float* w, auto nw) {
+        constexpr int NW = decltype(nw)::value;
 #pragma unroll 1
         for (int ky = 0; ky < 3; ++ky) {
-            const float* trow = &tile[buf][((py + ky) * kFewHS + px) * kFewPitch];
+            const float* trow = &tile[0][((py + ky) * kFewHS + px) * kFewPitch];
 #pragma unroll
             for (int kx = 0; kx < 3; ++kx) {
                 const float* tp = trow + kx * kFewPitch;
-                f32x4 v[4];
+                f32x4 v[NW];
 #pragma unroll
-                for (int q = 0; q < 4; ++q) v[q] = *reinterpret_cast<const f32x4*>(tp + 4 * q);
+                for (int q = 0; q < NW; ++q) v[q] = *reinterpret_cast<const f32x4*>(tp + 4 * q);
 #pragma unroll
                 for (int co = 0; co < CO; ++co) {
                     const float* wr = w + ((ky * 3 + kx) * CO + co) * 16;
 #pragma unroll
-                    for (int q = 0; q < 4; ++q) {
+                    for (int q = 0; q < NW; ++q) {
                         acc[co] = __builtin_fmaf(v[q].x, wr[4 * q + 0], acc[co]);
                         acc[co] = __builtin_fmaf(v[q].y, wr[4 * q + 1], acc[co]);
                         acc[co] = __builtin_fmaf(v[q].z, wr[4 * q + 2], acc[co]);
@@ -86,8 +92,14 @@
                 }
             }
         }
+    };
+    for (int c = 0; c < nblk; ++c) {
+        if (c + 1 < nblk) fetch(c + 1);
+        const float* w = a.wp + (size_t)c * (9 * CO * 16);
+        if (c + 1 == nblk && a.last_words == 1) block(w, std::integral_constant<int, 1>{});
+        else block(w, std::integral_constant<int, 4>{});
         __syncthreads();
-        if (c + 1 < nblk) publish(0);
+        if (c + 1 < nblk) publish(c + 1);
         __syncthreads();
     }
     const int gy = y0 + py, gx = x0 + px;
@@ -104,16 +116,17 @@
 
 }
 
-extern "C" int nrgbd_conv2d_few_f32(const float* x, int ldx, const float* w_packed, const float* bias, int out_lrelu, float* y, int ldy,
-                                    int ycoff, int N, int H, int W, int Cin, int Cout, void* stream) {
+extern "C" int nrgbd_conv2d_few_live_f32(const float* x, int ldx, const float* w_packed, const float* bias, int out_lrelu, float* y, int ldy,
+                                         int ycoff, int N, int H, int W, int Cin, int Cout, int last_words, void* stream) {
     using namespace nrgbd;
     if (!x || !w_packed || !y) return NRGBD_E_NULL;
+    if (last_words < 1 || last_words > 4) return NRGBD_E_ARG;
     if (N <= 0 || H <= 0 || W <= 0 || Cin <= 0 || (Cin & 15) || ldx < Cin || (ldx & 3) || Cout < 1 || Cout > 4 || ycoff < 0 ||
         ldy < ycoff + Cout)
         return NRGBD_E_SHAPE;
     if (reinterpret_cast<uintptr_t>(x) & 15) return NRGBD_E_ALIGN;
     if ((long)N * H * W * ldx >= (1L << 32)) return NRGBD_E_SHAPE;
-    ConvFewArgs a{x, w_packed, bias, y, N, H, W, Cin, ldx, ldy, ycoff, out_lrelu};
+    ConvFewArgs a{x, w_packed, bias, y, N, H, W, Cin, ldx, ldy, ycoff, out_lrelu, last_words == 1 ? 1 : 4};
     const int nwg = ceil_div(W, kFewT) * ceil_div(H, kFewT) * N;
     hipStream_t st = (hipStream_t)stream;
     switch (Cout) {
@@ -125,3 +138,8 @@
     NRGBD_CHECK_LAUNCH();
     return NRGBD_OK;
 }
+
+extern "C" int nrgbd_conv2d_few_f32(const float* x, int ldx, const float* w_packed, const float* bias, int out_lrelu, float* y, int ldy,
+                                    int ycoff, int N, int H, int W, int Cin, int Cout, void* stream) {
+    return nrgbd_conv2d_few_live_f32(x, ldx, w_packed, bias, out_lrelu, y, ldy, ycoff, N, H, W, Cin, Cout, 4, stream);
+}
diff --git a/neuralrgbd_amd/csrc/wino_pc.hip b/neuralrgbd_amd/csrc/wino_pc.hip
--- a/neuralrgbd_amd/csrc/wino_pc.hip
+++ b/neuralrgbd_amd/csrc/wino_pc.hip
@@ -10,7 +10,8 @@
     int a0, a1;
     unsigned ldy, lane_yoff;
 };
-template <bool HALF> using PcAcc = f32x4[16][HALF ? 1 : 2];
+constexpr int kPcShortK = 3;
+template <bool HALF> using PcAcc =f32x4[16][HALF ? 1 : 2];
 
 template <int DIL, int EPI, bool HALF>
 __device__ __forceinline__ PcLane pc_lane(const WinoPcArgs& a, int lane, int wv) {
@@ -39,9 +40,10 @@
     }
 }
 
-template <bool HALF, bool FIRST>
+template <bool HALF, bool FIRST, bool SHORT = false>
 __device__ __forceinline__ void pc_mfma_stage(PcAcc<HALF>& acc, f32x4 (&An)[4][2], f32x4 (&Bn)[kPcNB], const float* Vc, const float* Vn,
-                                              const f32x4* wcur, const f32x4* wnx, const PcLane& c) {
+                                              const f32x4* wcur, const f32x4* wnx, const PcLane& c, bool skip3 = false) {
+    static_assert(!SHORT || (!HALF && !FIRST && kPcShortK > kPcWPos), "a short stage: full form, never a tile's first, the weight request keeps its gap");
     const int a0 = c.a0, a1 = c.a1;
     const f32x4 zero4 = {0.f, 0.f, 0.f, 0.f};
     if constexpr (HALF) {
@@ -76,8 +78,10 @@
             }
 #pragma unroll
             for (int e = 0; e < 4; ++e) {
-                acc[xi][0] = __builtin_amdgcn_mfma_f32_16x16x4f32(An[cur][0][e], Bn[xi % kPcNB][e], FIRST && e == 0 ? zero4 : acc[xi][0], 0, 0, 0);
-                acc[xi][1] = __builtin_amdgcn_mfma_f32_16x16x4f32(An[cur][1][e], Bn[xi % kPcNB][e], FIRST && e == 0 ? zero4 : acc[xi][1], 0, 0, 0);
+                if (!(SHORT && e >= kPcShortK && skip3)) {
+                    acc[xi][0] = __builtin_amdgcn_mfma_f32_16x16x4f32(An[cur][0][e], Bn[xi % kPcNB][e], FIRST && e == 0 ? zero4 : acc[xi][0], 0, 0, 0);
+                    acc[xi][1] = __builtin_amdgcn_mfma_f32_16x16x4f32(An[cur][1][e], Bn[xi % kPcNB][e], FIRST && e == 0 ? zero4 : acc[xi][1], 0, 0, 0);
+                }
                 if (e == kPcWPos) Bn[(xi + kPcBD) % kPcNB] = xi + kPcBD < 16 ? wcur[(xi + kPcBD) * 256] : wnx[(xi + kPcBD - 16) * 256];
                 __builtin_amdgcn_sched_barrier(0);
             }
@@ -608,6 +612,8 @@
         __syncthreads();
         pc_prime_a<HALF>(An, Vb, c);
         int buf = 0;
+        bool short_last = false;
+        if constexpr (EPI == 1 && !HALF && ODD) short_last = a.k_live_last == kPcShortK;
         for (int it = 0; it < count; ++it) {
             const int tnext = first + (it + 1 < count ? it + 1 : it) * step;
             const PcTile tn = pc_decode<KD, DIL>(tnext, a);
@@ -619,7 +625,7 @@
                 const f32x4* wcur = wt + (size_t)s * (16 * 256);
                 const f32x4* wnx = s + 1 < NS ? wcur + 16 * 256 : wt_next;
                 if (s == 0) pc_mfma_stage<HALF, true>(acc, An, Bn, Vc, Vn, wcur, wnx, c);
-                else pc_mfma_stage<HALF, false>(acc, An, Bn, Vc, Vn, wcur, wnx, c);
+                else pc_mfma_stage<HALF, false, EPI == 1 && !HALF && ODD>(acc, An, Bn, Vc, Vn, wcur, wnx, c, short_last && s + 1 == NS);
                 __syncthreads();
                 buf = nbuf;
             }
@@ -838,10 +844,11 @@
     return NRGBD_OK;
 }
 
-extern "C" int nrgbd_conv_wino_rnet_ex_f32(const float* x, const float* w_wino, const float* bias, int out_lrelu, float* y, int N,
-                                           int H, int W, int Cin, int Cout, int ldy, int ycoff, int cout_valid, void* stream) {
+extern "C" int nrgbd_conv_wino_rnet_live_f32(const float* x, const float* w_wino, const float* bias, int out_lrelu, float* y, int N,
+                                             int H, int W, int Cin, int Cout, int ldy, int ycoff, int cout_valid, int k_live_last, void* stream) {
     using namespace nrgbd;
     if (!x || !w_wino || !y) return NRGBD_E_NULL;
+    if (k_live_last < 1 || k_live_last > 4) return NRGBD_E_ARG;
     const bool half = Cout == 32;
     if (N <= 0 || H <= 0 || W <= 0 || Cin < 32 || Cin % kCB || Cout <= 0 || (Cout % 64 && !half)) return NRGBD_E_SHAPE;
     if ((long)N * H * W * Cin >= (1L << 30)) return NRGBD_E_SHAPE;
@@ -852,6 +859,7 @@
     if (nt >= (1L << 30)) return NRGBD_E_SHAPE;
     WinoPcArgs a{x, nullptr, nullptr, nullptr, nullptr, w_wino, y, nullptr, 0, 0, N, H, W, Cin, Cout, (int)nt, half ? 2 * rows : rows,
                  bias, out_lrelu, ldy, ycoff, cout_valid};
+    a.k_live_last = k_live_last;
     int nwg = 0;
     const int rc = pc_workgroups(nt, &nwg);
     if (rc != NRGBD_OK) return rc;
@@ -866,6 +874,17 @@
     if (e != hipSuccess) return (int)e;
     NRGBD_CHECK_LAUNCH();
     return NRGBD_OK;
+}
+
+extern "C" int nrgbd_conv_wino_rnet_ex_f32(const float* x, const float* w_wino, const float* bias, int out_lrelu, float* y, int N,
+                                           int H, int W, int Cin, int Cout, int ldy, int ycoff, int cout_valid, void* stream) {
+    return nrgbd_conv_wino_rnet_live_f32(x, w_wino, bias, out_lrelu, y, N, H, W, Cin, Cout, ldy, ycoff, cout_valid, 4, stream);
+}
+
+extern "C" int nrgbd_conv_wino_last_k_steps(int width) {
+    if (width <= 0) return NRGBD_E_SHAPE;
+    const int r = width % nrgbd::kCB;
+    return r == 0 || r > 4 ? 4 : r;
 }
 
 extern "C" int nrgbd_conv_wino_rnet_deconv_pack(const float* w_wino, float* w_masked, int Cin, void* stream) {
diff --git a/neuralrgbd_amd/csrc/wino_pc.hpp b/neuralrgbd_amd/csrc/wino_pc.hpp
--- a/neuralrgbd_amd/csrc/wino_pc.hpp
+++ b/neuralrgbd_amd/csrc/wino_pc.hpp
@@ -35,6 +35,7 @@
     int out_lrelu;
     int ldy, ycoff, cout_valid;
     float x_unit;
+    int k_live_last;
 };
 
 struct PcTile { int n, y0, x0, py, px, cg, row; };
diff --git a/neuralrgbd_amd/nets.py b/neuralrgbd_amd/nets.py
--- a/neuralrgbd_amd/nets.py
+++ b/neuralrgbd_amd/nets.py
@@ -52,6 +52,7 @@
 _PACKERS = {
     "taps": lambda ops, w: ops.conv_pack_weights(w),
     "s2": lambda ops, w: ops.conv_s2_pack(w),
+    "s2live": lambda ops, w: ops.conv_s2_pack(w, live=True),
     "pc": lambda ops, w: ops.conv_wino_pack32(w) if w.shape[0] == 32 and w.dim() == 4 else ops.conv_wino_pack(w),
     "dw": lambda ops, w: ops.conv_wino_dw_pack(w),
     "dw4": lambda ops, w: ops.conv_wino_dw4_pack(w),
@@ -302,13 +303,22 @@
             s2 = (conv.kernel_size == (3, 3) and conv.stride == (2, 2) and conv.padding == (1, 1) and d == 1
                   and mat.shape[1] % 2 == 0 and mat.shape[2] % 2 == 0 and conv.out_channels in (32, 64))
             if s2:
-                z, st = ops.conv2d_taps(ops.space_to_depth2(mat), _packed(self, conv, "s2"), conv.out_channels, 4,
-                                        want_stats=_needs_stats(bn))
+                z, st = self._conv_s2(conv, ops.space_to_depth2(mat), _needs_stats(bn))
             else:
                 raise _no_kernel("feature CNN layer %d -> %d, kernel %s, stride %s, dilation %d on a %d x %d map" % (
                     conv.in_channels, conv.out_channels, tuple(conv.kernel_size), tuple(conv.stride), d, mat.shape[1], mat.shape[2]))
         count = z.shape[0] * z.shape[1] * z.shape[2]
         return _Act(z, _bn_scale_shift(bn, st, count, "cm" if wino else "rows"), relu), mat
+
+    s2_kernels = ("live", "dense")
+
+    def _conv_s2(self, conv, s2d, want_stats):
+        from . import ops
+        c = conv.in_channels
+        if self.s2_kernels[0] == "live" and ((c % 16 == 0 and conv.out_channels == 64) or (c == 3 and conv.out_channels == 32)):
+            wp, masks = _packed(self, conv, "s2live")
+            return ops.conv2d_taps(s2d, wp, conv.out_channels, 4, want_stats=want_stats, live=masks)
+        return ops.conv2d_taps(s2d, _packed(self, conv, "s2"), conv.out_channels, 4, want_stats=want_stats)
 
     def _pointwise_cl(self, conv, m, stride=1, want_stats=False):
         from . import ops
@@ -339,8 +349,7 @@
         if x.shape[2] % 4 or x.shape[3] % 4:
             raise _no_kernel("image %d x %d: the plane-sweep grid is the image / 4 (models/basic.py:254-263), both sides must be multiples of 4"
                              % (x.shape[2], x.shape[3]))
-        z, st = ops.conv2d_taps(ops.space_to_depth2(x.contiguous(), nchw=True), _packed(self, conv, "s2"), conv.out_channels, 4,
-                                want_stats=_needs_stats(bn))
+        z, st = self._conv_s2(conv, ops.space_to_depth2(x.contiguous(), nchw=True), _needs_stats(bn))
         a = _Act(z, _bn_scale_shift(bn, st, z.numel() // z.shape[-1]), True)
         for i in (2, 4):
             a, _ = self._conv_bn_cl(self.firstconv[i], a, relu=True)
@@ -615,6 +624,8 @@
         return ((D, 64), (D0, D0), (D1, D1)) if ok else None
 
     deconv_kernels = ("wino", "direct")
+    last_stage_kernels = ("short", "dense")
+    few_kernels = ("live", "dense")
     _FEATS = (64, 32, 3)
 
     def mfma_ok(self, dpv):
@@ -705,6 +716,7 @@
         val = {"t0": deconv("trans_conv0"), "t1": deconv("trans_conv1")}
         for name in ("conv0", "conv0_1", "conv1", "conv1_1", "conv2", "conv2_1", "conv2_2"):
             val[name + "_w"] = wino(name)
+            val[name + "_cin"] = int(emb[name][0].shape[1])
         cache["key"], cache["val"] = key, val
         return val
 
@@ -764,11 +776,14 @@
 
         def conv_w(x, name, out=None, lrelu=True):
             wt = pk[name + "_w"]
-            out = ops.conv_wino_rnet(x, wt[0], wt[2], bias=wt[1], lrelu=lrelu, out=out, cout_valid=wt[3])
+            real = pk[name + "_cin"]
+            klast = ops.conv_wino_last_k_steps(real) if self.last_stage_kernels[0] == "short" else 4
+            out = ops.conv_wino_rnet(x, wt[0], wt[2], bias=wt[1], lrelu=lrelu, out=out, cout_valid=wt[3], k_live_last=klast)
             if len(wt) > 4:
                 t = wt[4]
                 if t[0] == "few":
-                    ops.conv2d_few(x, t[1], bias=t[2], lrelu=lrelu, out=out, ycoff=t[4])
+                    words = min(4, -(-(real % 16) // 4)) if real % 16 and self.few_kernels[0] == "live" else 4
+                    ops.conv2d_few(x, t[1], bias=t[2], lrelu=lrelu, out=out, ycoff=t[4], last_words=words)
                 else:
                     ops.conv_wino_rnet(x, t[0], t[2], bias=t[1], lrelu=lrelu, out=out, ycoff=t[4], cout_valid=t[3])
             return out
diff --git a/neuralrgbd_amd/ops.py b/neuralrgbd_amd/ops.py
--- a/neuralrgbd_amd/ops.py
+++ b/neuralrgbd_amd/ops.py
@@ -758,9 +758,38 @@
     return y, stats, mat
 
 
-def conv_s2_pack(w, cp=None):
+def conv_s2_pack(w, cp=None, live=False):
     w = _need(w, "w")
-    return conv_pack_weights(conv_s2_weights(w, cp))
+    w2 = conv_s2_weights(w, cp)
+    if not live:
+        return conv_pack_weights(w2)
+    masks, keep = conv_s2_live(w2, w.shape[1])
+    lines = conv_pack_weights(w2).view(4, w2.shape[1] // 16, 2, -1).permute(1, 0, 2, 3).reshape(len(keep), -1)
+    return lines[torch.tensor(keep, device=lines.device).nonzero().flatten()].reshape(-1).contiguous(), masks
+
+
+def conv_s2_live(w2, c):
+    cout, cp = w2.shape[:2]
+    w2 = w2.detach().cpu()
+    if cp % 16 or tuple(w2.shape[2:]) != (2, 2) or 4 * c > cp:
+        raise ValueError("conv_s2_live: w2 [Cout, cp %% 16 == 0, 2, 2] with 4 c <= cp expected, got %s, c = %d" % (tuple(w2.shape), c))
+    masks, keep = [], []
+    for cb in range(cp // 16):
+        m = 0
+        for tap in range(4):
+            ty, tx = tap >> 1, tap & 1
+            for g in range(2):
+                for e in range(4):
+                    chans = (cb * 16 + 4 * g + e, cb * 16 + 8 + 4 * g + e)
+                    reach = [ch < 4 * c and (ty, (ch // c) >> 1) != (0, 0) and (tx, (ch // c) & 1) != (0, 0) for ch in chans]
+                    if any(reach):
+                        m |= 1 << (4 * (tap * 2 + g) + e)
+                    elif bool((w2[:, list(chans), ty, tx] != 0).any()):
+                        raise ValueError("conv_s2_live: non-zero weight of channel %d or %d at window tap (%d, %d), which no 3x3 stride-2 "
+                                         "kernel reaches" % (chans[0], chans[1], ty, tx))
+                keep.append(((m >> (4 * (tap * 2 + g))) & 15) != 0)
+        masks.append(m)
+    return tuple(masks), keep
 
 
 def conv_s2_weights(w, cp=None):
@@ -789,9 +818,13 @@
     return y
 
 
-def conv2d_taps(x, w_packed, cout, taps, x_ss=None, x_relu=False, want_stats=True, stride=1):
+def conv2d_taps(x, w_packed, cout, taps, x_ss=None, x_relu=False, want_stats=True, stride=1, live=None):
     x = _need(x, "x")
     N, H, W, Cin = x.shape
+    if live is not None:
+        steps = sum(bin(m & (15 << (4 * s))).count("1") > 0 for m in live for s in range(8))
+        if taps != 4 or stride != 1 or len(live) != Cin // 16 or w_packed.numel() != steps * cout * 8:
+            raise ValueError("conv2d_taps: live masks go with taps = 4, one per 16 input channels, and a stream of their %d lines" % steps)
     if stride != 1:
         if taps != 1 or H % stride or W % stride:
             raise ValueError("conv2d_taps: a stride needs taps = 1 and sides that are multiples of it")
@@ -799,9 +832,13 @@
     y = torch.empty((N, H, W, cout), dtype=torch.float32, device=x.device)
     stats = torch.empty((conv2d_workgroups(N, H, W), 2 * cout), dtype=torch.float32, device=x.device) if want_stats else None
     with torch.cuda.device(x.device):
-        rc = _lib.load().nrgbd_conv2d_taps_f32(_p(x), _p(x_ss), int(x_relu), _p(w_packed), _p(y), _p(stats), N, H, W, Cin,
-                                                int(cout), int(taps), int(stride), _stream(x))
-    _lib.check(rc, "nrgbd_conv2d_taps_f32")
+        if live is not None:
+            rc = _lib.load().nrgbd_conv2d_taps_live_f32(_p(x), _p(x_ss), int(x_relu), _p(w_packed), _p(y), _p(stats), N, H, W, Cin,
+                                                         int(cout), ctypes.cast((ctypes.c_uint * len(live))(*live), ctypes.c_void_p), _stream(x))
+        else:
+            rc = _lib.load().nrgbd_conv2d_taps_f32(_p(x), _p(x_ss), int(x_relu), _p(w_packed), _p(y), _p(stats), N, H, W, Cin,
+                                                    int(cout), int(taps), int(stride), _stream(x))
+    _lib.check(rc, "nrgbd_conv2d_taps_live_f32" if live is not None else "nrgbd_conv2d_taps_f32")
     return y, stats
 
 
@@ -908,7 +945,13 @@
     return ss
 
 
-def conv_wino_rnet(x, w_wino, cout, bias=None, lrelu=True, out=None, ycoff=0, cout_valid=None):
+def conv_wino_last_k_steps(width):
+    k = int(_lib.load().nrgbd_conv_wino_last_k_steps(int(width)))
+    _lib.check(min(k, 0), "nrgbd_conv_wino_last_k_steps")
+    return k
+
+
+def conv_wino_rnet(x, w_wino, cout, bias=None, lrelu=True, out=None, ycoff=0, cout_valid=None, k_live_last=4):
     x = _need(x, "x")
     N, H, W, Cin = x.shape
     valid = int(cout if cout_valid is None else cout_valid)
@@ -917,9 +960,9 @@
     elif tuple(out.shape[:3]) != (N, H, W) or not out.is_contiguous() or out.shape[3] < ycoff + valid:
         raise ValueError("conv_wino_rnet: out must be a contiguous [N,H,W,>= ycoff + cout_valid] tensor")
     with torch.cuda.device(x.device):
-        rc = _lib.load().nrgbd_conv_wino_rnet_ex_f32(_p(x), _p(w_wino), _p(bias), int(bool(lrelu)), _p(out), N, H, W, Cin, int(cout),
-                                                      int(out.shape[3]), int(ycoff), valid, _stream(x))
-    _lib.check(rc, "nrgbd_conv_wino_rnet_ex_f32")
+        rc = _lib.load().nrgbd_conv_wino_rnet_live_f32(_p(x), _p(w_wino), _p(bias), int(bool(lrelu)), _p(out), N, H, W, Cin, int(cout),
+                                                        int(out.shape[3]), int(ycoff), valid, int(k_live_last), _stream(x))
+    _lib.check(rc, "nrgbd_conv_wino_rnet_live_f32")
     return out
 
 
@@ -965,7 +1008,7 @@
     return out
 
 
-def conv2d_few(x, w_few, bias=None, lrelu=True, out=None, ycoff=0):
+def conv2d_few(x, w_few, bias=None, lrelu=True, out=None, ycoff=0, last_words=4):
     x = _need(x, "x")
     w_few = _need(w_few, "w_few")
     N, H, W, ldx = x.shape
@@ -977,9 +1020,9 @@
     elif tuple(out.shape[:3]) != (N, H, W) or not out.is_contiguous() or out.shape[3] < ycoff + cout:
         raise ValueError("conv2d_few: out must be a contiguous [N,H,W,>= ycoff + Cout] tensor")
     with torch.cuda.device(x.device):
-        rc = _lib.load().nrgbd_conv2d_few_f32(_p(x), int(ldx), _p(w_few), _p(bias), int(bool(lrelu)), _p(out), int(out.shape[3]), int(ycoff),
-                                               N, H, W, nblk * 16, cout, _stream(x))
-    _lib.check(rc, "nrgbd_conv2d_few_f32")
+        rc = _lib.load().nrgbd_conv2d_few_live_f32(_p(x), int(ldx), _p(w_few), _p(bias), int(bool(lrelu)), _p(out), int(out.shape[3]), int(ycoff),
+                                                    N, H, W, nblk * 16, cout, int(last_words), _stream(x))
+    _lib.check(rc, "nrgbd_conv2d_few_live_f32")
     return out
 
 
```

After: 32.38 frames/s, median of 6. About the same (+0.2%).
